# Rose-STL-Lab/spherical-dyffusion

Hardware: AMD Instinct MI355X
Metric: forecast-steps/sec (180x360, 63ch), 25-member ensemble DYffusion sampling, whole job (higher is better)
Workload: dtype f32 tensors; every GEMM-class kernel (1x1 convs, fused MLP, Legendre analysis/synthesis, dhconv) as 3-pass split-f16 MFMA with f32 accumulation; FFT / norms / pointwise in f32 (statistics f64); 1 GPU; 25-member ensemble x horizon-6 DYffusion sampling pass (6 forecaster + 10 interpolator SFNO forwards, dropout stream on, AR feedback), 180x360, 63 state + 2 forcing channels, embed 256, 8 blocks; horizon=6, relayed_members=0, parallelism=members of one initial condition sharded over GPUs, no data-path collective

## Files before the change

### include/sdy_amd.h

```cpp
#ifndef SDY_AMD_H
#define SDY_AMD_H

#include <stddef.h>
#include <stdint.h>

#ifdef __cplusplus
extern "C" {
#endif
#pragma GCC visibility push(default)

#define SDY_OK 0
#define SDY_ERR_ARG (-1)
#define SDY_ERR_UNSUPPORTED (-2)
#define SDY_ERR_ALIGN (-3)
#define SDY_ERR_WORKSPACE (-4)
#define SDY_ERR_NAME (-5)
#define SDY_ERR_SHAPE (-6)
#define SDY_ERR_STATE (-7)

#define SDY_GRID_EQUIANGULAR 0
#define SDY_GRID_LEGENDRE_GAUSS 1

int sdy_version(void);
const char* sdy_error_string(int code);
#define SDY_ABI_STRUCTS 25
int sdy_abi_check(const size_t* sizes, int n);
int sdy_abi_sizes(size_t* sizes, int n);

typedef struct sdy_sht_plan sdy_sht_plan;

int sdy_sht_tables_host(int nlat, int nlon, int lmax, int mmax, int grid, double* pct, double* w, double* theta);

int sdy_sht_plan_create(int nlat, int nlon, int lmax, int mmax, int grid, sdy_sht_plan** out);
int sdy_sht_plan_create_ex(int nlat, int nlon, int lmax, int mmax, int grid, int gemm_mode, sdy_sht_plan** out);
void sdy_sht_plan_destroy(sdy_sht_plan* plan);
int sdy_sht_plan_dims(const sdy_sht_plan* plan, int dims[6]);
int sdy_sht_plan_kernels(const sdy_sht_plan* plan, int out[2]);
size_t sdy_sht_workspace_floats(const sdy_sht_plan* plan, int B, int C);

int sdy_sht_forward(const sdy_sht_plan* plan, const float* x, float* out_c64, int B, int C, float* ws,
                    size_t ws_floats, void* stream);
int sdy_sht_inverse(const sdy_sht_plan* plan, const float* in_c64, float* y, int B, int C, float* ws,
                    size_t ws_floats, void* stream);

int sdy_rfft_lon(const sdy_sht_plan* plan, const float* x, const float* a, const float* d, float* xn_out,
                 float* Xf, int B, int C, void* stream);
int sdy_legendre_fwd(const sdy_sht_plan* plan, const float* Xf, float* Cs, int B, int C, void* stream);
int sdy_legendre_inv(const sdy_sht_plan* plan, const float* Cs, float* Yf, int B, int C, void* stream);
int sdy_irfft_lon(const sdy_sht_plan* plan, const float* Yf, const float* bias, float* y, int B, int C,
                  void* stream);
int sdy_irfft_lon_act(const sdy_sht_plan* plan, const float* Yf, const float* bias, float* zt, long zt_bstride, double* part,
                      int B, int C, void* stream);
int sdy_instnorm_from_partials(const double* part, int K, int B, int C, int HW, const float* gamma, const float* beta,
                               float eps, float* a, float* d, void* stream);
int sdy_gelu_stats(const float* y, long y_bstride, float* out, long out_bstride, int out_tiled, double* stats, int B, int C,
                   int HW, void* stream);
int sdy_affine_copy_stats(const float* x, long x_bstride, const float* a, const float* d, float* out, long out_bstride,
                          double* stats, int C, int HW, const unsigned char* rows, int n_rows, int src_row0, void* stream);

int sdy_dhconv_pack_weight(const float* w_host, int Ci, int Co, int L, float* w_packed_dev, void* stream);
int sdy_dhconv(const float* Cs_in, const float* w_packed, float* Cs_out, int L, int mtr, int B, int Ci, int Co,
               void* stream);
size_t sdy_dhconv_h3_pack_bytes(int Ci, int Co, int L);
int sdy_dhconv_h3_pack_weight(const float* w_host, int Ci, int Co, int L, void* packed_dev, float* scale);
int sdy_dhconv_h3(const float* Cs_in, const void* packed, float scale, float* Cs_out, int L, int mtr, int B, int Ci,
                  int Co, void* stream);

int sdy_dhconv_frag_supported(int Ci, int Co);
size_t sdy_dhconv_frag_pack_bytes(int L);
int sdy_dhconv_frag_pack(const float* w_host, int L, void* packed_dev, float* scale);
int sdy_dhconv_frag(const float* Cs_in, const void* packed, float scale, float* Cs_out, int L, int mtr, int B,
                    void* stream);

int sdy_instnorm_coeffs(const float* x, int B, int C, int HW, const float* gamma, const float* beta,
                        const float* scale_shift, long ss_stride, float eps, float* a, float* d, void* stream);

typedef struct sdy_conv_args {
  const float* x;  long x_bstride;
  const float* wt; int ldw;
  float* out;      long out_bstride;
  int B, Cin, Cout, HW;
  const float* pa; const float* pd;
  const float* bias;
  const float* add; long add_bstride;
  int add_mode;
  int act;
  float drop_p;
  const float* keep_mask;
  uint64_t seed; uint32_t call; uint32_t stream_id; uint32_t batch_offset;
  int rows_per_call;
  const float* batch_scale;
  int kernel_tag;
  const void* w_h3;
  float w_h3_scale;
  const void* w_frag;
  float w_frag_scale;
  double* stats;
  int out_tiled;
  const unsigned char* x_rows;
} sdy_conv_args;
int sdy_conv1x1(const sdy_conv_args* args, void* stream);

int sdy_conv256_h3_supported(int Cin, int Cout);
size_t sdy_conv256_h3_pack_bytes(void);
size_t sdy_conv256_h3_pack_bytes_cin(int Cin);
int sdy_conv256_h3_pack(const float* w_host, void* packed_dev, float* scale);
int sdy_conv256_h3_pack_cin(const float* w_host, int Cin, void* packed_dev, float* scale);
size_t sdy_h3_pack_bytes(int Cout, int Cin);
int sdy_h3_pack_weight(const float* w_host, int Cout, int Cin, void* packed_dev, float* scale);

typedef struct sdy_mlp_args {
  const float* x;  long x_bstride;
  const float* pa; const float* pd;
  const void* w; float w1_scale; float w2_scale;
  const float* b1; const float* b2;
  float* out;      long out_bstride;
  const float* add; long add_bstride;
  const float* add_a; const float* add_d;
  int B, E, hidden, HW;
  float drop_p;
  uint64_t seed; uint32_t call; uint32_t stream_fc1; uint32_t stream_fc2; uint32_t batch_offset;
  int rows_per_call;
  const float* batch_scale;
  double* stats;
  int x_tiled;
  const float* keep_hidden;
  const float* keep_out;
  const unsigned char* out_rows;
  int add_by_launch_row;
} sdy_mlp_args;
int sdy_instnorm_from_stats(double* stats, int B, int C, int HW, const float* gamma, const float* beta,
                            const float* scale_shift, long ss_bstride, float eps, float* a_out, float* d_out, void* stream);
int sdy_mlp_h3_supported(int E, int hidden);
size_t sdy_mlp_h3_pack_bytes(int E, int hidden);
int sdy_mlp_h3_pack(const float* w1_host, const float* w2_host, int E, int hidden, void* packed_dev, float* scale1,
                    float* scale2);
int sdy_mlp_h3(const sdy_mlp_args* args, void* stream);

typedef struct sdy_pair_args {
  const float* x;  long x_bstride;
  const void* w; float w1_scale; float w2_scale;
  const float* b1;
  float* out;      long out_bstride;
  const float* add; long add_bstride;
  int B, Cin, hidden, Cout, HW;
  double* stats;
} sdy_pair_args;
int sdy_pair_h3_supported(int Cin, int hidden, int Cout);
size_t sdy_pair_h3_pack_bytes(int Cin, int hidden, int Cout);
int sdy_pair_h3_pack(const float* w1_host, const float* w2_host, int Cin, int hidden, int Cout, void* packed_dev,
                     float* scale1, float* scale2);
int sdy_pair_h3(const sdy_pair_args* args, void* stream);

typedef struct sdy_sfno_config {
  int nlat, nlon;
  int in_chans;
  int out_chans;
  int embed_dim;
  int num_layers;
  int mlp_hidden;
  int lmax, mmax;
  int data_grid;
  int with_time_emb;
  int time_dim;
  float dropout_mlp;
  float drop_path_rate;
  int big_skip, pos_embed;
  int gemm_mode;
} sdy_sfno_config;

typedef struct sdy_sfno sdy_sfno;
int sdy_sfno_create(const sdy_sfno_config* cfg, sdy_sfno** out);
void sdy_sfno_destroy(sdy_sfno* net);
int sdy_sfno_set_param(sdy_sfno* net, const char* name, const float* host, size_t numel);
int sdy_sfno_ready(const sdy_sfno* net);
const char* sdy_sfno_missing(const sdy_sfno* net);
size_t sdy_sfno_workspace_floats(const sdy_sfno* net, int B);
int sdy_sfno_max_batch(const sdy_sfno* net);

typedef struct sdy_sfno_fwd_args {
  const float* in[3]; int in_chans[3];
  const float* time;
  float* out;
  int B;
  int enable_dropout;
  uint64_t seed; uint32_t call; uint32_t batch_offset;
  int rows_per_call;
  const float* const* keep_masks;
  const float* drop_path_keep;
  float* ws; size_t ws_floats;
  int reuse_encoder;
  int shared_inputs;
  const float* gen_src;
  int gen_chans;
  int gen_pos;
  const float* gen_coef;
  const float* gen_noise;
} sdy_sfno_fwd_args;
int sdy_sfno_forward(sdy_sfno* net, const sdy_sfno_fwd_args* args, void* stream);

int sdy_sfno_time_embed(sdy_sfno* net, const float* time, int B, float* t_repr, float* ss, void* stream);

int sdy_cold_update(const float* x_s, const float* x_ip_next, const float* x_ip_s, float* out, size_t n,
                    void* stream);
int sdy_concat_channels(const float* const* src, const int* chans, int nsrc, float* out, int B, int HW,
                        void* stream);

#define SDY_MAX_VARS 96
typedef struct sdy_var_table {
  int nvars;
  const float* data[SDY_MAX_VARS];
  float mean[SDY_MAX_VARS];
  float std[SDY_MAX_VARS];
} sdy_var_table;
int sdy_norm_pack(const sdy_var_table* vars, int t, int T1, int B, int HW, float* out, void* stream);

typedef struct sdy_step_finish_args {
  int B, HW, T1, t;
  const float* gen; int n_out;
  const float* prev_in; float* next_in; int n_in;
  int n_entries;
  int out_idx[SDY_MAX_VARS];
  int in_idx[SDY_MAX_VARS];
  float* gen_norm_tl[SDY_MAX_VARS];
  float* gen_tl[SDY_MAX_VARS];
  float mean[SDY_MAX_VARS], std[SDY_MAX_VARS];
  int presc_entry;
  const float* presc_target;
  const float* presc_mask;
  int mask_value, interpolate;
  const float* ar_init;
} sdy_step_finish_args;
int sdy_step_finish(const sdy_step_finish_args* args, void* stream);
int sdy_init_timeline(const sdy_var_table* vars, int T1, int B, int HW, float* const* tl_norm, float* const* tl_denorm,
                      void* stream);
int sdy_lp_rel_terms(const float* gen, const sdy_var_table* targets, int t, int T1, int B, int HW, double* terms,
                     void* stream);

int sdy_ensemble_metrics(const float* pred, const float* truth, const float* weights, int M, long member_stride,
                         int n_planes, int HW, double* out, void* stream);

int sdy_ensemble_series(const float* pred, int M, long member_stride, long sample_stride, const float* truth,
                        long truth_sample_stride, const float* weights, int n_sample, int T, int HW, double* out,
                        void* stream);

int sdy_ensemble_series_grad(const float* pred, int M, long member_stride, long sample_stride, const float* truth,
                             long truth_sample_stride, const float* weights, int n_sample, int T, int nlat, int nlon,
                             double* out, void* stream);

#define SDY_DERIVED_MAX_LEVELS 16
typedef struct {
  const float* q[SDY_DERIVED_MAX_LEVELS];
  const float* ps;
  const float* lhf;
  const float* prate;
  const float* adv;
  long s0, s1;
  int n0, n1, T, HW, K;
  float ak[SDY_DERIVED_MAX_LEVELS + 1], bk[SDY_DERIVED_MAX_LEVELS + 1];
// ... 338 lines not shown
```

### spherical-dyffusion_amd/_lib.py

```python
from __future__ import annotations

import ctypes as C
import os

_HERE = os.path.dirname(os.path.abspath(__file__))
LIB_PATH = os.environ.get("SDY_AMD_LIB") or os.path.join(_HERE, "libsdy_amd.so")

SDY_GRID = {"equiangular": 0, "legendre-gauss": 1}


class SdyError(RuntimeError):
    pass


class SdyConvArgs(C.Structure):
    _fields_ = [
        ("x", C.c_void_p), ("x_bstride", C.c_long),
        ("wt", C.c_void_p), ("ldw", C.c_int),
        ("out", C.c_void_p), ("out_bstride", C.c_long),
        ("B", C.c_int), ("Cin", C.c_int), ("Cout", C.c_int), ("HW", C.c_int),
        ("pa", C.c_void_p), ("pd", C.c_void_p),
        ("bias", C.c_void_p),
        ("add", C.c_void_p), ("add_bstride", C.c_long),
        ("add_mode", C.c_int),
        ("act", C.c_int),
        ("drop_p", C.c_float),
        ("keep_mask", C.c_void_p),
        ("seed", C.c_uint64), ("call", C.c_uint32), ("stream_id", C.c_uint32), ("batch_offset", C.c_uint32),
        ("rows_per_call", C.c_int),
        ("batch_scale", C.c_void_p),
        ("kernel_tag", C.c_int),
        ("w_h3", C.c_void_p),
        ("w_h3_scale", C.c_float),
        ("w_frag", C.c_void_p),
        ("w_frag_scale", C.c_float),
        ("stats", C.c_void_p),
        ("out_tiled", C.c_int),
        ("x_rows", C.c_void_p),
    ]


class SdyMlpArgs(C.Structure):
    _fields_ = [
        ("x", C.c_void_p), ("x_bstride", C.c_long),
        ("pa", C.c_void_p), ("pd", C.c_void_p),
        ("w", C.c_void_p), ("w1_scale", C.c_float), ("w2_scale", C.c_float),
        ("b1", C.c_void_p), ("b2", C.c_void_p),
        ("out", C.c_void_p), ("out_bstride", C.c_long),
        ("add", C.c_void_p), ("add_bstride", C.c_long),
        ("add_a", C.c_void_p), ("add_d", C.c_void_p),
        ("B", C.c_int), ("E", C.c_int), ("hidden", C.c_int), ("HW", C.c_int),
        ("drop_p", C.c_float),
        ("seed", C.c_uint64), ("call", C.c_uint32), ("stream_fc1", C.c_uint32), ("stream_fc2", C.c_uint32),
        ("batch_offset", C.c_uint32),
        ("rows_per_call", C.c_int),
        ("batch_scale", C.c_void_p),
        ("stats", C.c_void_p),
        ("x_tiled", C.c_int),
        ("keep_hidden", C.c_void_p), ("keep_out", C.c_void_p),
        ("out_rows", C.c_void_p),
        ("add_by_launch_row", C.c_int),
    ]


class SdyPairArgs(C.Structure):
    _fields_ = [
        ("x", C.c_void_p), ("x_bstride", C.c_long),
        ("w", C.c_void_p), ("w1_scale", C.c_float), ("w2_scale", C.c_float),
        ("b1", C.c_void_p),
        ("out", C.c_void_p), ("out_bstride", C.c_long),
        ("add", C.c_void_p), ("add_bstride", C.c_long),
        ("B", C.c_int), ("Cin", C.c_int), ("hidden", C.c_int), ("Cout", C.c_int), ("HW", C.c_int),
        ("stats", C.c_void_p),
    ]


SDY_MAX_VARS = 96


class SdyVarTable(C.Structure):
    _fields_ = [("nvars", C.c_int), ("data", C.c_void_p * SDY_MAX_VARS), ("mean", C.c_float * SDY_MAX_VARS),
                ("std", C.c_float * SDY_MAX_VARS)]


class SdyStepFinishArgs(C.Structure):
    _fields_ = [
        ("B", C.c_int), ("HW", C.c_int), ("T1", C.c_int), ("t", C.c_int),
        ("gen", C.c_void_p), ("n_out", C.c_int),
        ("prev_in", C.c_void_p), ("next_in", C.c_void_p), ("n_in", C.c_int),
        ("n_entries", C.c_int),
        ("out_idx", C.c_int * SDY_MAX_VARS), ("in_idx", C.c_int * SDY_MAX_VARS),
        ("gen_norm_tl", C.c_void_p * SDY_MAX_VARS), ("gen_tl", C.c_void_p * SDY_MAX_VARS),
        ("mean", C.c_float * SDY_MAX_VARS), ("std", C.c_float * SDY_MAX_VARS),
        ("presc_entry", C.c_int),
        ("presc_target", C.c_void_p), ("presc_mask", C.c_void_p),
        ("mask_value", C.c_int), ("interpolate", C.c_int),
        ("ar_init", C.c_void_p),
    ]


class SdySfnoConfig(C.Structure):
    _fields_ = [
        ("nlat", C.c_int), ("nlon", C.c_int),
        ("in_chans", C.c_int), ("out_chans", C.c_int),
        ("embed_dim", C.c_int), ("num_layers", C.c_int), ("mlp_hidden", C.c_int),
        ("lmax", C.c_int), ("mmax", C.c_int),
        ("data_grid", C.c_int),
        ("with_time_emb", C.c_int), ("time_dim", C.c_int),
        ("dropout_mlp", C.c_float), ("drop_path_rate", C.c_float),
        ("big_skip", C.c_int), ("pos_embed", C.c_int),
        ("gemm_mode", C.c_int),
    ]


class SdySfnoFwdArgs(C.Structure):
    _fields_ = [
        ("in_", C.c_void_p * 3), ("in_chans", C.c_int * 3),
        ("time", C.c_void_p),
        ("out", C.c_void_p),
        ("B", C.c_int),
# ... 238 lines not shown
        ("pool_times", C.c_int),
        ("n_events", C.c_int),
        ("n_maps", C.c_int),
        ("below", C.c_ubyte * SDY_MAX_VARS), ("is_map", C.c_ubyte * SDY_MAX_VARS),
        ("map_first", C.c_int * SDY_MAX_VARS),
        ("scalars", C.c_void_p), ("maps", C.c_void_p),
        ("acc", C.c_void_p),
    ]


SDY_FSS_MAX_RADII = 4


class SdyFssArgs(C.Structure):
    _anonymous_ = ("win",)
    _fields_ = [
        ("win", SdyWindow), ("H", C.c_int), ("W", C.c_int),
        ("t0", C.c_int),
        ("t_start", C.c_int), ("n_slots", C.c_int),
        ("pool_times", C.c_int),
        ("n_events", C.c_int),
        ("n_maps", C.c_int),
        ("below", C.c_ubyte * SDY_MAX_VARS), ("is_map", C.c_ubyte * SDY_MAX_VARS),
        ("map_first", C.c_int * SDY_MAX_VARS),
        ("scalars", C.c_void_p), ("maps", C.c_void_p),
        ("n_radii", C.c_int), ("radii", C.c_int * SDY_FSS_MAX_RADII),
        ("acc", C.c_void_p),
        ("ws", C.c_void_p), ("ws_bytes", C.c_size_t),
    ]


SDY_GRAM_MAX_MEMBERS = 64


class SdyMemberGramArgs(C.Structure):
    _anonymous_ = ("win",)
    _fields_ = [
        ("win", SdyWindow), ("HW", C.c_int),
        ("weights", C.c_void_p),
        ("climatology", C.c_void_p * SDY_MAX_VARS),
        ("out", C.c_void_p),
        ("ws", C.c_void_p), ("ws_bytes", C.c_size_t),
    ]


SDY_RANK_HIST_MAX_MEMBERS = 64


class SdyRankHistArgs(C.Structure):
    _anonymous_ = ("win",)
    _fields_ = [
        ("win", SdyWindow), ("H", C.c_int), ("W", C.c_int),
        ("t0", C.c_int),
        ("t_start", C.c_int), ("n_slots", C.c_int),
        ("pool_times", C.c_int),
        ("counts", C.c_void_p), ("ties", C.c_void_p),
    ]


ABI_STRUCTS = (SdyConvArgs, SdyMlpArgs, SdyPairArgs, SdySfnoConfig, SdySfnoFwdArgs, SdyVarTable, SdyStepFinishArgs,
               SdyDerivedArgs, SdyCorrectorArgs, SdyDryAirArgs, SdyHistArgs, SdyCoarsenArgs, SdyVideoArgs, SdyZonalArgs,
               SdyMemberSumArgs, SdyMemberStatsArgs, SdySpectrumArgs, SdyVariabilityArgs, SdyVariabilityMapsArgs,
               SdyVariabilityStatsArgs, SdyRegionSeriesArgs, SdyEventArgs, SdyFssArgs, SdyMemberGramArgs,
               SdyRankHistArgs)

SIGNATURES = {
    "sdy_version": (C.c_int, []),
    "sdy_error_string": (C.c_char_p, [C.c_int]),
    "sdy_abi_check": (C.c_int, [C.POINTER(C.c_size_t), C.c_int]),
    "sdy_abi_sizes": (C.c_int, [C.POINTER(C.c_size_t), C.c_int]),
    "sdy_sht_tables_host": (C.c_int, [C.c_int, C.c_int, C.c_int, C.c_int, C.c_int, C.c_void_p, C.c_void_p, C.c_void_p]),
    "sdy_sht_plan_create": (C.c_int, [C.c_int, C.c_int, C.c_int, C.c_int, C.c_int, C.POINTER(C.c_void_p)]),
    "sdy_sht_plan_create_ex": (C.c_int, [C.c_int, C.c_int, C.c_int, C.c_int, C.c_int, C.c_int, C.POINTER(C.c_void_p)]),
    "sdy_sht_plan_destroy": (None, [C.c_void_p]),
    "sdy_sht_plan_dims": (C.c_int, [C.c_void_p, C.POINTER(C.c_int * 6)]),
    "sdy_sht_plan_kernels": (C.c_int, [C.c_void_p, C.POINTER(C.c_int * 2)]),
    "sdy_sht_workspace_floats": (C.c_size_t, [C.c_void_p, C.c_int, C.c_int]),
    "sdy_sht_forward": (C.c_int, [C.c_void_p, C.c_void_p, C.c_void_p, C.c_int, C.c_int, C.c_void_p, C.c_size_t, C.c_void_p]),
    "sdy_sht_inverse": (C.c_int, [C.c_void_p, C.c_void_p, C.c_void_p, C.c_int, C.c_int, C.c_void_p, C.c_size_t, C.c_void_p]),
    "sdy_rfft_lon": (C.c_int, [C.c_void_p, C.c_void_p, C.c_void_p, C.c_void_p, C.c_void_p, C.c_void_p, C.c_int, C.c_int, C.c_void_p]),
    "sdy_legendre_fwd": (C.c_int, [C.c_void_p, C.c_void_p, C.c_void_p, C.c_int, C.c_int, C.c_void_p]),
    "sdy_legendre_inv": (C.c_int, [C.c_void_p, C.c_void_p, C.c_void_p, C.c_int, C.c_int, C.c_void_p]),
    "sdy_irfft_lon": (C.c_int, [C.c_void_p, C.c_void_p, C.c_void_p, C.c_void_p, C.c_int, C.c_int, C.c_void_p]),
    "sdy_irfft_lon_act": (C.c_int, [C.c_void_p, C.c_void_p, C.c_void_p, C.c_void_p, C.c_long, C.c_void_p, C.c_int, C.c_int,
                                    C.c_void_p]),
    "sdy_instnorm_from_partials": (C.c_int, [C.c_void_p, C.c_int, C.c_int, C.c_int, C.c_int, C.c_void_p, C.c_void_p, C.c_float,
                                             C.c_void_p, C.c_void_p, C.c_void_p]),
    "sdy_gelu_stats": (C.c_int, [C.c_void_p, C.c_long, C.c_void_p, C.c_long, C.c_int, C.c_void_p, C.c_int, C.c_int, C.c_int,
                                 C.c_void_p]),
    "sdy_affine_copy_stats": (C.c_int, [C.c_void_p, C.c_long, C.c_void_p, C.c_void_p, C.c_void_p, C.c_long, C.c_void_p, C.c_int,
                                        C.c_int, C.c_void_p, C.c_int, C.c_int, C.c_void_p]),
    "sdy_dhconv_pack_weight": (C.c_int, [C.c_void_p, C.c_int, C.c_int, C.c_int, C.c_void_p, C.c_void_p]),
    "sdy_dhconv": (C.c_int, [C.c_void_p, C.c_void_p, C.c_void_p, C.c_int, C.c_int, C.c_int, C.c_int, C.c_int, C.c_void_p]),
    "sdy_dhconv_h3_pack_bytes": (C.c_size_t, [C.c_int, C.c_int, C.c_int]),
    "sdy_dhconv_h3_pack_weight": (C.c_int, [C.c_void_p, C.c_int, C.c_int, C.c_int, C.c_void_p, C.POINTER(C.c_float)]),
    "sdy_dhconv_h3": (C.c_int, [C.c_void_p, C.c_void_p, C.c_float, C.c_void_p, C.c_int, C.c_int, C.c_int, C.c_int, C.c_int,
                                C.c_void_p]),
    "sdy_dhconv_frag_supported": (C.c_int, [C.c_int, C.c_int]),
    "sdy_dhconv_frag_pack_bytes": (C.c_size_t, [C.c_int]),
    "sdy_dhconv_frag_pack": (C.c_int, [C.c_void_p, C.c_int, C.c_void_p, C.POINTER(C.c_float)]),
    "sdy_dhconv_frag": (C.c_int, [C.c_void_p, C.c_void_p, C.c_float, C.c_void_p, C.c_int, C.c_int, C.c_int, C.c_void_p]),
    "sdy_instnorm_coeffs": (C.c_int, [C.c_void_p, C.c_int, C.c_int, C.c_int, C.c_void_p, C.c_void_p, C.c_void_p, C.c_long,
                                      C.c_float, C.c_void_p, C.c_void_p, C.c_void_p]),
    "sdy_conv1x1": (C.c_int, [C.POINTER(SdyConvArgs), C.c_void_p]),
    "sdy_ensemble_metrics": (C.c_int, [C.c_void_p, C.c_void_p, C.c_void_p, C.c_int, C.c_long, C.c_int, C.c_int, C.c_void_p,
                                       C.c_void_p]),
    "sdy_instnorm_from_stats": (C.c_int, [C.c_void_p, C.c_int, C.c_int, C.c_int, C.c_void_p, C.c_void_p, C.c_void_p,
                                          C.c_long, C.c_float, C.c_void_p, C.c_void_p, C.c_void_p]),
    "sdy_mlp_h3_supported": (C.c_int, [C.c_int, C.c_int]),
    "sdy_mlp_h3_pack_bytes": (C.c_size_t, [C.c_int, C.c_int]),
    "sdy_mlp_h3_pack": (C.c_int, [C.c_void_p, C.c_void_p, C.c_int, C.c_int, C.c_void_p, C.POINTER(C.c_float),
                                  C.POINTER(C.c_float)]),
    "sdy_mlp_h3": (C.c_int, [C.POINTER(SdyMlpArgs), C.c_void_p]),
    "sdy_pair_h3_supported": (C.c_int, [C.c_int, C.c_int, C.c_int]),
    "sdy_pair_h3_pack_bytes": (C.c_size_t, [C.c_int, C.c_int, C.c_int]),
    "sdy_pair_h3_pack": (C.c_int, [C.c_void_p, C.c_void_p, C.c_int, C.c_int, C.c_int, C.c_void_p, C.POINTER(C.c_float),
                                   C.POINTER(C.c_float)]),
    "sdy_pair_h3": (C.c_int, [C.POINTER(SdyPairArgs), C.c_void_p]),
    "sdy_conv256_h3_supported": (C.c_int, [C.c_int, C.c_int]),
    "sdy_conv256_h3_pack_bytes": (C.c_size_t, []),
    "sdy_conv256_h3_pack_bytes_cin": (C.c_size_t, [C.c_int]),
    "sdy_conv256_h3_pack": (C.c_int, [C.c_void_p, C.c_void_p, C.POINTER(C.c_float)]),
    "sdy_conv256_h3_pack_cin": (C.c_int, [C.c_void_p, C.c_int, C.c_void_p, C.POINTER(C.c_float)]),
    "sdy_h3_pack_bytes": (C.c_size_t, [C.c_int, C.c_int]),
    "sdy_h3_pack_weight": (C.c_int, [C.c_void_p, C.c_int, C.c_int, C.c_void_p, C.POINTER(C.c_float)]),
    "sdy_sfno_create": (C.c_int, [C.POINTER(SdySfnoConfig), C.POINTER(C.c_void_p)]),
    "sdy_sfno_destroy": (None, [C.c_void_p]),
    "sdy_sfno_set_param": (C.c_int, [C.c_void_p, C.c_char_p, C.c_void_p, C.c_size_t]),
    "sdy_sfno_ready": (C.c_int, [C.c_void_p]),
    "sdy_sfno_missing": (C.c_char_p, [C.c_void_p]),
    "sdy_sfno_workspace_floats": (C.c_size_t, [C.c_void_p, C.c_int]),
    "sdy_sfno_max_batch": (C.c_int, [C.c_void_p]),
    "sdy_sfno_forward": (C.c_int, [C.c_void_p, C.POINTER(SdySfnoFwdArgs), C.c_void_p]),
    "sdy_sfno_time_embed": (C.c_int, [C.c_void_p, C.c_void_p, C.c_int, C.c_void_p, C.c_void_p, C.c_void_p]),
    "sdy_norm_pack": (C.c_int, [C.POINTER(SdyVarTable), C.c_int, C.c_int, C.c_int, C.c_int, C.c_void_p, C.c_void_p]),
    "sdy_step_finish": (C.c_int, [C.POINTER(SdyStepFinishArgs), C.c_void_p]),
    "sdy_init_timeline": (C.c_int, [C.POINTER(SdyVarTable), C.c_int, C.c_int, C.c_int, C.POINTER(C.c_void_p),
                                    C.POINTER(C.c_void_p), C.c_void_p]),
    "sdy_lp_rel_terms": (C.c_int, [C.c_void_p, C.POINTER(SdyVarTable), C.c_int, C.c_int, C.c_int, C.c_int, C.c_void_p,
                                   C.c_void_p]),
    "sdy_cold_update": (C.c_int, [C.c_void_p, C.c_void_p, C.c_void_p, C.c_void_p, C.c_size_t, C.c_void_p]),
    "sdy_concat_channels": (C.c_int, [C.POINTER(C.c_void_p), C.POINTER(C.c_int), C.c_int, C.c_void_p, C.c_int, C.c_int,
                                      C.c_void_p]),
    "sdy_time_mean_accumulate": (C.c_int, [C.c_void_p, C.c_int, C.c_long, C.c_int, C.c_long, C.c_int, C.c_int, C.c_int,
                                          C.c_float, C.c_void_p, C.c_void_p]),
    "sdy_status_flags": (C.c_int, [C.POINTER(C.c_uint), C.c_int, C.c_void_p]),
    "sdy_status_flags_async": (C.c_int, [C.c_void_p, C.c_int, C.c_void_p]),
    "sdy_range_headroom_enable": (C.c_int, [C.c_int]),
    "sdy_range_headroom": (C.c_int, [C.POINTER(C.c_float), C.c_int, C.c_void_p]),
    "sdy_dropout_stream_rounds": (C.c_int, []),
    "sdy_dropout_stream_words": (C.c_int, [C.c_uint32, C.c_uint32, C.c_uint32, C.c_uint32, C.c_uint32, C.c_uint32,
                                           C.POINTER(C.c_uint32)]),
    "sdy_cond_noise_fill": (C.c_int, [C.c_uint64, C.c_uint32, C.c_uint32, C.c_int, C.c_int, C.c_int, C.c_int, C.c_void_p,
                                      C.c_void_p]),
    "sdy_ensemble_series": (C.c_int, [C.c_void_p, C.c_int, C.c_long, C.c_long, C.c_void_p, C.c_long, C.c_void_p, C.c_int,
                                     C.c_int, C.c_int, C.c_void_p, C.c_void_p]),
    "sdy_ensemble_series_grad": (C.c_int, [C.c_void_p, C.c_int, C.c_long, C.c_long, C.c_void_p, C.c_long, C.c_void_p,
                                          C.c_int, C.c_int, C.c_int, C.c_int, C.c_void_p, C.c_void_p]),
    "sdy_derived_water": (C.c_int, [C.POINTER(SdyDerivedArgs), C.c_void_p]),
    "sdy_corrector": (C.c_int, [C.POINTER(SdyCorrectorArgs), C.c_void_p]),
    "sdy_corrector_host": (C.c_int, [C.POINTER(SdyCorrectorArgs)]),
    "sdy_corrector_workspace_bytes": (C.c_size_t, [C.c_int, C.c_int]),
    "sdy_dry_air_series": (C.c_int, [C.POINTER(SdyDryAirArgs), C.c_void_p]),
    "sdy_dry_air_series_host": (C.c_int, [C.POINTER(SdyDryAirArgs)]),
    "sdy_dry_air_workspace_bytes": (C.c_size_t, [C.c_int, C.c_int, C.c_int]),
    "sdy_hist_add": (C.c_int, [C.POINTER(SdyHistArgs), C.c_void_p]),
# ... 115 lines not shown
```

### spherical-dyffusion_amd/csrc/capi.hip

```cpp
#include <cmath>
#include <cstdio>
#include <cstdlib>
#include <cstring>
#include <mutex>
#include <string>
#include <vector>

#include "common.h"
#include "fft.h"
#include "pointwise.h"

static inline int round_up(int v, int m) { return (v + m - 1) / m * m; }
static inline size_t round_up_sz(size_t v, size_t m) { return (v + m - 1) / m * m; }

template <class F>
static float h3_pack_host(std::vector<_Float16>& buf, int nb, int rows, int K, int rows_pad, int Kpad, F value) {
  float mx = 0.f;
  for (int b = 0; b < nb; ++b)
    for (int r = 0; r < rows; ++r)
      for (int k = 0; k < K; ++k) mx = std::fmax(mx, std::fabs(value(b, r, k)));
  const float s = sdy_h3_scale(mx);
  const size_t plane = (size_t)nb * rows_pad * Kpad;
  buf.assign(2 * plane, (_Float16)0.0f);
  for (int b = 0; b < nb; ++b)
    for (int r = 0; r < rows; ++r) {
      const size_t base = ((size_t)b * rows_pad + r) * Kpad;
      for (int k = 0; k < K; ++k) sdy_h3_split(value(b, r, k) * s, buf[base + k], buf[plane + base + k]);
    }
  return s;
}


extern "C" int sdy_version(void) { return 102; }

extern "C" int sdy_abi_sizes(size_t* sizes, int n) {
  const size_t mine[SDY_ABI_STRUCTS] = {
      sizeof(sdy_conv_args),      sizeof(sdy_mlp_args),      sizeof(sdy_pair_args),        sizeof(sdy_sfno_config),
      sizeof(sdy_sfno_fwd_args),  sizeof(sdy_var_table),     sizeof(sdy_step_finish_args), sizeof(sdy_derived_args),
      sizeof(sdy_corrector_args), sizeof(sdy_dry_air_args),  sizeof(sdy_hist_args),        sizeof(sdy_coarsen_args),
      sizeof(sdy_video_args),     sizeof(sdy_zonal_args),    sizeof(sdy_member_sum_args),  sizeof(sdy_member_stats_args),
      sizeof(sdy_spectrum_args),  sizeof(sdy_variability_args), sizeof(sdy_variability_maps_args),
      sizeof(sdy_variability_stats_args), sizeof(sdy_region_series_args), sizeof(sdy_event_args),
      sizeof(sdy_fss_args),       sizeof(sdy_member_gram_args), sizeof(sdy_rank_hist_args)};
  if (!sizes || n != SDY_ABI_STRUCTS) return SDY_ERR_ARG;
  for (int i = 0; i < n; ++i) sizes[i] = mine[i];
  return SDY_OK;
}

extern "C" int sdy_abi_check(const size_t* sizes, int n) {
  size_t mine[SDY_ABI_STRUCTS];
  if (!sizes || sdy_abi_sizes(mine, n) != SDY_OK) return SDY_ERR_ARG;
  for (int i = 0; i < n; ++i)
    if (sizes[i] != mine[i]) return SDY_ERR_ARG;
  return SDY_OK;
}

extern "C" const char* sdy_error_string(int code) {
  switch (code) {
    case SDY_OK: return "ok";
    case SDY_ERR_ARG: return "bad argument (null pointer or non-positive extent)";
    case SDY_ERR_UNSUPPORTED: return "unsupported size/configuration";
    case SDY_ERR_ALIGN: return "extent along a contiguous dimension is not a multiple of 4, or a pointer read as float4 is not 16-byte aligned";
    case SDY_ERR_WORKSPACE: return "workspace too small";
    case SDY_ERR_NAME: return "unknown parameter name";
    case SDY_ERR_SHAPE: return "parameter has the wrong number of elements";
    case SDY_ERR_STATE: return "object not fully initialised";
    default: return code > 0 ? hipGetErrorString((hipError_t)code) : "unknown error";
  }
}

struct sdy_sht_plan {
  int nlat, nlon, lmax, mmax, mtr, grid;
  int Lpad4, Kpad4;
  float* d_wqT = nullptr;
  float* d_pct = nullptr;
  float* d_tw = nullptr;
  float* d_pw = nullptr;
  SdyFftDesc fft;
  int gemm_mode = 0;
  void* d_wq_h3 = nullptr;
  void* d_pct_h3 = nullptr;
  float s_wq = 1.f, s_pct = 1.f;
  int h3_rows_fwd = 0, h3_k_fwd = 0, h3_rows_inv = 0, h3_k_inv = 0;
  void* d_wq_frag = nullptr;
  void* d_pct_frag = nullptr;
  float s_wq_frag = 1.f, s_pct_frag = 1.f;
  void* d_wq_par = nullptr;
  void* d_pct_par = nullptr;
  float s_wq_par = 1.f, s_pct_par = 1.f;
  int* d_kdead = nullptr;
  int* d_mcut = nullptr;
  enum Leg { LEG_PAR, LEG_H3, LEG_GEMM_H3, LEG_GEMM_F32 } leg = LEG_GEMM_F32;
  bool fused360 = false;
};

namespace {
struct SdySwitches {
  bool gemm_f32, no_fft360, no_leg_par, no_leg_frag, no_dh_frag, no_fused_mlp, no_drop_skip, no_skip_fold;
};
const SdySwitches& sw() {
  static const SdySwitches v = [] {
    auto on = [](const char* n) { return std::getenv(n) != nullptr; };
    const char* g = std::getenv("SDY_GEMM_MODE");
    return SdySwitches{g && std::string(g) == "f32", on("SDY_NO_FFT360"), on("SDY_NO_LEG_PAR"), on("SDY_NO_LEG_FRAG"),
                       on("SDY_NO_DH_FRAG"), on("SDY_NO_FUSED_MLP"), on("SDY_NO_DROP_SKIP"), on("SDY_NO_SKIP_FOLD")};
  }();
  return v;
}
}
static int env_gemm_mode() { return sw().gemm_f32 ? 0 : 1; }

template <class D, class T>
static hipError_t upload(D** dst, const std::vector<T>& v) {
  hipError_t e = hipMalloc((void**)dst, v.size() * sizeof(T));
  return e == hipSuccess ? hipMemcpy(*dst, v.data(), v.size() * sizeof(T), hipMemcpyHostToDevice) : e;
}
struct LegTables { const float *wqT, *pf; int nlat, lmax, Lpad4, Kpad4; };
static float leg_wq_at(void* c, int m, int l, int k) {
  const LegTables* x = static_cast<const LegTables*>(c);
  return x->wqT[((size_t)m * x->nlat + k) * x->Lpad4 + l];
}
static float leg_pct_at(void* c, int m, int k, int l) {
  const LegTables* x = static_cast<const LegTables*>(c);
  return x->pf[((size_t)m * x->lmax + l) * x->Kpad4 + k];
}

extern "C" int sdy_sht_plan_create(int nlat, int nlon, int lmax, int mmax, int grid, sdy_sht_plan** out) {
  return sdy_sht_plan_create_ex(nlat, nlon, lmax, mmax, grid, env_gemm_mode(), out);
}

extern "C" int sdy_sht_plan_create_ex(int nlat, int nlon, int lmax, int mmax, int grid, int gemm_mode,
                                      sdy_sht_plan** out) {
  if (gemm_mode != 0 && gemm_mode != 1) return SDY_ERR_ARG;
  if (!out || nlat < 2 || nlon < 4 || lmax < 1 || mmax < 1) return SDY_ERR_ARG;
  if (nlon % 4) return SDY_ERR_ALIGN;
  if (mmax > nlon / 2 + 1) return SDY_ERR_ARG;
  if (grid != SDY_GRID_EQUIANGULAR && grid != SDY_GRID_LEGENDRE_GAUSS) return SDY_ERR_ARG;
  sdy_sht_plan* p = new sdy_sht_plan();
  p->nlat = nlat; p->nlon = nlon; p->lmax = lmax; p->mmax = mmax; p->grid = grid;
  p->mtr = mmax < lmax ? mmax : lmax;
  p->Lpad4 = round_up(lmax, 4);
  p->Kpad4 = round_up(nlat, 4);
  const int n = nlon / 2;
  p->fft.n = n;
  p->fft.S = (n + 1) | 1;
  p->fft.guard_f16 = gemm_mode == 1 ? 1 : 0;
  int r = sdy_factor_radices(n, p->fft.radices, &p->fft.nstages);
  if (r != SDY_OK) { delete p; return r; }
  if ((size_t)(4 * 16 * p->fft.S + 4 * n + 2) * sizeof(float) > 64 * 1024) { delete p; return SDY_ERR_UNSUPPORTED; }

  std::vector<double> pct((size_t)mmax * lmax * nlat), w(nlat);
  r = sdy_sht_tables_host(nlat, nlon, lmax, mmax, grid, pct.data(), w.data(), nullptr);
  if (r != SDY_OK) { delete p; return r; }
  const int mtr = p->mtr;
  std::vector<float> wqT((size_t)mtr * nlat * p->Lpad4, 0.0f), pf((size_t)mtr * lmax * p->Kpad4, 0.0f);
  for (int m = 0; m < mtr; ++m)
    for (int l = 0; l < lmax; ++l)
      for (int k = 0; k < nlat; ++k) {
        const double v = pct[((size_t)m * lmax + l) * nlat + k];
        wqT[((size_t)m * nlat + k) * p->Lpad4 + l] = (float)(v * w[k]);
        pf[((size_t)m * lmax + l) * p->Kpad4 + k] = (float)v;
      }
  std::vector<float> tw(2 * (size_t)n), pw(2 * (size_t)(n + 1));
  for (int j = 0; j < n; ++j) {
    const double a = -2.0 * M_PI * j / n;
    tw[2 * j] = (float)std::cos(a);
    tw[2 * j + 1] = (float)std::sin(a);
  }
  for (int m = 0; m <= n; ++m) {
    const double a = -2.0 * M_PI * m / nlon;
    pw[2 * m] = (float)std::cos(a);
    pw[2 * m + 1] = (float)std::sin(a);
  }
  hipError_t e = upload(&p->d_wqT, wqT);
  if (e == hipSuccess) e = upload(&p->d_pct, pf);
  if (e == hipSuccess) e = upload(&p->d_tw, tw);
  if (e == hipSuccess) e = upload(&p->d_pw, pw);
  if (e != hipSuccess) { sdy_sht_plan_destroy(p); return (int)e; }
  p->gemm_mode = gemm_mode;
  if (gemm_mode == 1) {
    std::vector<_Float16> buf;
    p->h3_rows_fwd = lmax > 128 ? round_up(lmax, 256) : 128; p->h3_k_fwd = round_up(nlat, 64);
    p->s_wq = h3_pack_host(buf, mtr, lmax, nlat, p->h3_rows_fwd, p->h3_k_fwd, [&](int m, int l, int k) {
      return wqT[((size_t)m * nlat + k) * p->Lpad4 + l];
    });
    if ((e = upload(&p->d_wq_h3, buf)) != hipSuccess) { sdy_sht_plan_destroy(p); return (int)e; }
    p->h3_rows_inv = nlat > 128 ? round_up(nlat, 256) : 128; p->h3_k_inv = round_up(lmax, 64);
    p->s_pct = h3_pack_host(buf, mtr, nlat, lmax, p->h3_rows_inv, p->h3_k_inv, [&](int m, int k, int l) {
// ... 120 lines not shown
  g.B = Xf; g.ldb = N; g.sB = (long)p->nlat * N;
  g.C = Cs; g.ldc = p->mtr * N; g.sC = N;
  g.M = p->Lpad4; g.M_store = p->lmax; g.N = N; g.K = p->nlat; g.nbatch = p->mtr;
  g.tri_mode = SDY_TRI_LEG_FWD; g.tile = SDY_TILE_64x128;
  if (p->leg == sdy_sht_plan::LEG_PAR)
    return sdy_leg_par_launch(p->d_wq_par, p->s_wq_par, p->mtr, Xf, tiled ? 64 : N, (long)p->nlat * N, Cs,
                              cs_tiled ? 64L : (long)p->mtr * N, cs_tiled ? (long)(N / 64) * p->lmax * 64 : (long)N,
                              p->lmax, p->nlat, N, 1, polar ? p->d_kdead : nullptr, (hipStream_t)stream,
                              tiled ? 64L * p->nlat : 0L, cs_tiled ? 64L * p->lmax : 0L);
  if (tiled || cs_tiled) return SDY_ERR_UNSUPPORTED;
  if (p->leg == sdy_sht_plan::LEG_H3)
    return sdy_leg_h3_launch(p->d_wq_frag, p->s_wq_frag, p->mtr, Xf, N, (long)p->nlat * N, Cs, (long)p->mtr * N, N, p->lmax,
                             p->nlat, N, SDY_TRI_LEG_FWD, (hipStream_t)stream);
  if (p->leg == sdy_sht_plan::LEG_GEMM_H3)
    return sdy_gemm_h3_launch(g, p->d_wq_h3, p->h3_rows_fwd, p->h3_k_fwd, (long)p->h3_rows_fwd * p->h3_k_fwd,
                              (long)p->mtr * p->h3_rows_fwd * p->h3_k_fwd, p->s_wq, 0, (hipStream_t)stream);
  return sdy_gemm_launch(g, (hipStream_t)stream);
}
extern "C" int sdy_legendre_fwd(const sdy_sht_plan* p, const float* Xf, float* Cs, int B, int C, void* stream) {
  if (!p || !Xf || !Cs || B <= 0 || C <= 0) return SDY_ERR_ARG;
  if (C & 1) return SDY_ERR_ALIGN;
  SDY_TRY(sdy_spec_zero_upper_launch(Cs, p->lmax, p->mtr, 2 * B * C, (hipStream_t)stream));
  return legendre_fwd_impl(p, Xf, Cs, B, C, false, stream, false, false);
}

struct sdy_vsht_plan {
  const sdy_sht_plan* base = nullptr;
  float* d_dT = nullptr;
  float* d_mT = nullptr;
};

extern "C" void sdy_vsht_plan_destroy(sdy_vsht_plan* v) {
  if (!v) return;
  if (v->d_dT) (void)hipFree(v->d_dT);
  if (v->d_mT) (void)hipFree(v->d_mT);
  delete v;
}

extern "C" int sdy_vsht_plan_create(const sdy_sht_plan* p, sdy_vsht_plan** out) {
  if (!p || !out) return SDY_ERR_ARG;
  const int nlat = p->nlat, lmax = p->lmax, mtr = p->mtr;
  std::vector<double> dtab((size_t)mtr * lmax * nlat), mtab((size_t)mtr * lmax * nlat), w(nlat);
  SDY_TRY(sdy_vsht_tables_host(nlat, p->nlon, lmax, mtr, p->grid, dtab.data(), mtab.data()));
  SDY_TRY(sdy_sht_tables_host(nlat, p->nlon, lmax, mtr, p->grid, nullptr, w.data(), nullptr));
  std::vector<float> dT((size_t)mtr * nlat * p->Lpad4, 0.0f), mT((size_t)mtr * nlat * p->Lpad4, 0.0f);
  for (int m = 0; m < mtr; ++m)
    for (int l = 0; l < lmax; ++l)
      for (int k = 0; k < nlat; ++k) {
        const size_t from = ((size_t)m * lmax + l) * nlat + k, to = ((size_t)m * nlat + k) * p->Lpad4 + l;
        dT[to] = (float)(dtab[from] * w[k]);
        mT[to] = (float)(mtab[from] * w[k]);
      }
  sdy_vsht_plan* v = new sdy_vsht_plan();
  v->base = p;
  hipError_t e = upload(&v->d_dT, dT);
  if (e == hipSuccess) e = upload(&v->d_mT, mT);
  if (e != hipSuccess) { sdy_vsht_plan_destroy(v); return (int)e; }
  *out = v;
  return SDY_OK;
}

extern "C" int sdy_vector_legendre_fwd(const sdy_vsht_plan* v, const float* Xf, float* Cs_d, float* Cs_m, int B, int C,
                                       void* stream) {
  if (!v || !v->base || !Xf || !Cs_d || !Cs_m || B <= 0 || C <= 0) return SDY_ERR_ARG;
  if (C & 1) return SDY_ERR_ALIGN;
  const sdy_sht_plan* p = v->base;
  const int N = 2 * B * C;
  const float* tables[2] = {v->d_dT, v->d_mT};
  float* outs[2] = {Cs_d, Cs_m};
  for (int i = 0; i < 2; ++i) {
    SDY_TRY(sdy_spec_zero_upper_launch(outs[i], p->lmax, p->mtr, N, (hipStream_t)stream));
    GemmParams g{};
    g.A = tables[i]; g.lda = p->Lpad4; g.sA = (long)p->nlat * p->Lpad4;
    g.B = Xf; g.ldb = N; g.sB = (long)p->nlat * N;
    g.C = outs[i]; g.ldc = p->mtr * N; g.sC = N;
    g.M = p->Lpad4; g.M_store = p->lmax; g.N = N; g.K = p->nlat; g.nbatch = p->mtr;
    g.tri_mode = SDY_TRI_LEG_FWD; g.tile = SDY_TILE_64x128;
    SDY_TRY(sdy_gemm_launch(g, (hipStream_t)stream));
  }
  return SDY_OK;
}

static int legendre_inv_impl(const sdy_sht_plan* p, const float* Cs, float* Yf, int B, int C, bool polar, void* stream,
                             bool tiled, bool cs_tiled) {
  if (!p || !Cs || !Yf || B <= 0 || C <= 0) return SDY_ERR_ARG;
  if (C & 1) return SDY_ERR_ALIGN;
  const int N = 2 * B * C;
  GemmParams g{};
  g.A = p->d_pct; g.lda = p->Kpad4; g.sA = (long)p->lmax * p->Kpad4;
  g.B = Cs; g.ldb = p->mtr * N; g.sB = N;
  g.C = Yf; g.ldc = N; g.sC = (long)p->nlat * N;
  g.M = p->Kpad4; g.M_store = p->nlat; g.N = N; g.K = p->lmax; g.nbatch = p->mtr;
  g.tri_mode = SDY_TRI_LEG_INV; g.tile = SDY_TILE_64x128;
  if (p->leg == sdy_sht_plan::LEG_PAR)
    return sdy_leg_par_launch(p->d_pct_par, p->s_pct_par, p->mtr, Cs, cs_tiled ? 64L : (long)p->mtr * N,
                              cs_tiled ? (long)(N / 64) * p->lmax * 64 : (long)N, Yf, tiled ? 64 : N,
                              (long)p->nlat * N, p->nlat, p->lmax, N, 0, polar ? p->d_kdead : nullptr, (hipStream_t)stream,
                              cs_tiled ? 64L * p->lmax : 0L, tiled ? 64L * p->nlat : 0L);
  if (tiled || cs_tiled) return SDY_ERR_UNSUPPORTED;
  if (p->leg == sdy_sht_plan::LEG_H3)
    return sdy_leg_h3_launch(p->d_pct_frag, p->s_pct_frag, p->mtr, Cs, (long)p->mtr * N, N, Yf, N, (long)p->nlat * N, p->nlat,
                             p->lmax, N, SDY_TRI_LEG_INV, (hipStream_t)stream);
  if (p->leg == sdy_sht_plan::LEG_GEMM_H3)
    return sdy_gemm_h3_launch(g, p->d_pct_h3, p->h3_rows_inv, p->h3_k_inv, (long)p->h3_rows_inv * p->h3_k_inv,
                              (long)p->mtr * p->h3_rows_inv * p->h3_k_inv, p->s_pct, 0, (hipStream_t)stream);
  return sdy_gemm_launch(g, (hipStream_t)stream);
}
extern "C" int sdy_legendre_inv(const sdy_sht_plan* p, const float* Cs, float* Yf, int B, int C, void* stream) {
  return legendre_inv_impl(p, Cs, Yf, B, C, false, stream, false, false);
}

extern "C" int sdy_sht_forward(const sdy_sht_plan* p, const float* x, float* out_c64, int B, int C, float* ws,
                               size_t ws_floats, void* stream) {
  if (!p || !x || !out_c64 || !ws) return SDY_ERR_ARG;
  if (ws_floats < sdy_sht_workspace_floats(p, B, C)) return SDY_ERR_WORKSPACE;
  float* Xf = ws;
  float* Cs = ws + round_up_sz(xf_floats(p, B, C), 64);
  SDY_TRY(sdy_rfft_lon(p, x, nullptr, nullptr, nullptr, Xf, B, C, stream));
  SDY_TRY(legendre_fwd_impl(p, Xf, Cs, B, C, false, stream, false, false));
  return sdy_spec_to_torch_launch(Cs, out_c64, B, C, p->lmax, p->mtr, p->mmax, (hipStream_t)stream);
}

extern "C" int sdy_sht_inverse(const sdy_sht_plan* p, const float* in_c64, float* y, int B, int C, float* ws,
                               size_t ws_floats, void* stream) {
  if (!p || !in_c64 || !y || !ws) return SDY_ERR_ARG;
  if (ws_floats < sdy_sht_workspace_floats(p, B, C)) return SDY_ERR_WORKSPACE;
  float* Yf = ws;
  float* Cs = ws + round_up_sz(xf_floats(p, B, C), 64);
  SDY_TRY(sdy_torch_to_spec_launch(in_c64, Cs, B, C, p->lmax, p->mtr, p->mmax, (hipStream_t)stream));
  SDY_TRY(sdy_legendre_inv(p, Cs, Yf, B, C, stream));
  return sdy_irfft_lon(p, Yf, nullptr, y, B, C, stream);
}

extern "C" int sdy_dhconv_pack_weight(const float* w_host, int Ci, int Co, int L, float* w_packed_dev, void* stream) {
  if (!w_host || !w_packed_dev || Ci <= 0 || Co <= 0 || L <= 0) return SDY_ERR_ARG;
  std::vector<float> packed((size_t)L * 2 * Ci * Co);
  for (int i = 0; i < Ci; ++i)
    for (int o = 0; o < Co; ++o)
      for (int l = 0; l < L; ++l) {
        const float* s = w_host + (((size_t)i * Co + o) * L + l) * 2;
        packed[(((size_t)l * 2 + 0) * Ci + i) * Co + o] = s[0];
        packed[(((size_t)l * 2 + 1) * Ci + i) * Co + o] = s[1];
      }
  (void)stream;
  SDY_HIP_TRY(hipMemcpy(w_packed_dev, packed.data(), packed.size() * sizeof(float), hipMemcpyHostToDevice));
  return SDY_OK;
}

extern "C" int sdy_dhconv(const float* Cs_in, const float* w_packed, float* Cs_out, int L, int mtr, int B, int Ci,
                          int Co, void* stream) {
  if (!Cs_in || !w_packed || !Cs_out || L <= 0 || mtr <= 0 || B <= 0 || Ci <= 0 || Co <= 0) return SDY_ERR_ARG;
  if ((Ci & 3) || (Co & 3)) return SDY_ERR_ALIGN;
  GemmParams g{};
  g.A = Cs_in; g.a_kcontig = 1; g.lda = 2 * Ci; g.sA = (long)mtr * B * 2 * Ci;
  g.B = w_packed; g.b_cplx = 1; g.cplx_Ei = Ci; g.cplx_Eo = Co; g.ldb = 2 * Co; g.sB = (long)2 * Ci * Co;
  g.C = Cs_out; g.ldc = 2 * Co; g.sC = (long)mtr * B * 2 * Co;
  g.M = mtr * B; g.M_store = mtr * B; g.N = 2 * Co; g.K = 2 * Ci; g.nbatch = L;
  g.tri_mode = SDY_TRI_DHCONV; g.tri_B = B; g.tile = SDY_TILE_64x128;
  return sdy_gemm_launch(g, (hipStream_t)stream);
}

static inline int dh_npad(int Co) { return round_up(2 * Co, 128); }
static inline int dh_kpad(int Ci) { return round_up(2 * Ci, 64); }

extern "C" size_t sdy_dhconv_h3_pack_bytes(int Ci, int Co, int L) {
  if (Ci <= 0 || Co <= 0 || L <= 0) return 0;
  return (size_t)2 * L * dh_npad(Co) * dh_kpad(Ci) * sizeof(_Float16);
}

static int dhconv_h3_pack(const float* w, int Ci, int Co, int L, void* packed_dev, float* scale, int ilv) {
  if (!w || !packed_dev || !scale || Ci <= 0 || Co <= 0 || L <= 0) return SDY_ERR_ARG;
  if (ilv && ((Ci & 15) || (Co & 15))) return SDY_ERR_UNSUPPORTED;
  std::vector<_Float16> buf;
  *scale = h3_pack_host(buf, L, 2 * Co, 2 * Ci, dh_npad(Co), dh_kpad(Ci), [&](int l, int op, int ip) {
    const int ro = ilv ? (op >> 4) & 1 : op >= Co, o = ilv ? (op >> 5) * 16 + (op & 15) : op - ro * Co;
    const int ri = ilv ? (ip >> 4) & 1 : ip >= Ci, i = ilv ? (ip >> 5) * 16 + (ip & 15) : ip - ri * Ci;
    const float* e = w + (((size_t)i * Co + o) * L + l) * 2;
    if (ri == ro) return e[0];
    return ri ? -e[1] : e[1];
  });
  SDY_HIP_TRY(hipMemcpy(packed_dev, buf.data(), buf.size() * sizeof(_Float16), hipMemcpyHostToDevice));
  return SDY_OK;
}
extern "C" int sdy_dhconv_h3_pack_weight(const float* w, int Ci, int Co, int L, void* packed_dev, float* scale) {
  return dhconv_h3_pack(w, Ci, Co, L, packed_dev, scale, 0);
}

extern "C" int sdy_dhconv_h3(const float* Cs_in, const void* packed, float scale, float* Cs_out, int L, int mtr, int B,
                             int Ci, int Co, void* stream) {
  if (!Cs_in || !packed || !Cs_out || L <= 0 || mtr <= 0 || B <= 0 || Ci <= 0 || Co <= 0) return SDY_ERR_ARG;
  if ((Ci & 3) || (Co & 3)) return SDY_ERR_ALIGN;
  GemmParams g{};
  g.A = Cs_in; g.lda = 2 * Ci; g.sA = (long)mtr * B * 2 * Ci;
  g.C = Cs_out; g.ldc = 2 * Co; g.sC = (long)mtr * B * 2 * Co;
  g.M = mtr * B; g.M_store = mtr * B; g.N = 2 * Co; g.K = 2 * Ci; g.nbatch = L;
  g.tri_mode = SDY_TRI_DHCONV; g.tri_B = B;
  const int Np = dh_npad(Co), Kp = dh_kpad(Ci);
  return sdy_gemm_h3_launch(g, packed, Np, Kp, (long)Np * Kp, (long)L * Np * Kp, scale, 1, (hipStream_t)stream);
}

extern "C" int sdy_instnorm_coeffs(const float* x, int B, int C, int HW, const float* gamma, const float* beta,
                                   const float* scale_shift, long ss_stride, float eps, float* a, float* d,
                                   void* stream) {
  return sdy_instnorm_coeffs_launch(x, B, C, HW, gamma, beta, scale_shift, ss_stride, eps, a, d, (hipStream_t)stream);
}

static inline bool tiled_stride_ok(long bs, int C, int HW) { return bs >= (long)((HW + 63) / 64) * C * 64; }

extern "C" int sdy_instnorm_from_partials(const double* part, int K, int B, int C, int HW, const float* gamma,
                                          const float* beta, float eps, float* a, float* d, void* stream) {
  if (!part || !gamma || !beta || !a || !d || K <= 0 || B <= 0 || C <= 0 || HW <= 0) return SDY_ERR_ARG;
  if ((HW & 3) || !fft_aligned16(part)) return SDY_ERR_ALIGN;
  return sdy_instnorm_from_partials_launch(part, K, B, C, HW, gamma, beta, eps, a, d, (hipStream_t)stream);
}

extern "C" int sdy_gelu_stats(const float* y, long y_bstride, float* out, long out_bstride, int out_tiled, double* stats,
                              int B, int C, int HW, void* stream) {
  if (!y || !out || B <= 0 || C <= 0 || HW <= 0 || y_bstride < 0 || out_bstride < 0) return SDY_ERR_ARG;
  if ((HW & 3) || (y_bstride & 3) || (out_bstride & 3) || !fft_aligned16(y) || !fft_aligned16(out) || !fft_aligned16(stats))
    return SDY_ERR_ALIGN;
  if (out_tiled && (!tiled_stride_ok(out_bstride, C, HW) || out == y)) return SDY_ERR_ARG;
  return sdy_gelu_stats_launch(y, y_bstride, out, out_bstride, out_tiled ? 1 : 0, stats, B, C, HW, (hipStream_t)stream);
}

extern "C" int sdy_affine_copy_stats(const float* x, long x_bstride, const float* a, const float* d, float* out,
                                     long out_bstride, double* stats, int C, int HW, const unsigned char* rows, int n_rows,
                                     int src_row0, void* stream) {
  if (!x || !out || !rows || (a == nullptr) != (d == nullptr) || C <= 0 || HW <= 0 || n_rows <= 0 || n_rows > SDY_MAP_MAX ||
      x_bstride < 0 || out_bstride < 0)
    return SDY_ERR_ARG;
  if ((HW & 3) || (x_bstride & 3) || (out_bstride & 3) || !fft_aligned16(x) || !fft_aligned16(out) || !fft_aligned16(stats))
    return SDY_ERR_ALIGN;
  return sdy_affine_copy_stats_launch(x, x_bstride, a, d, out, out_bstride, stats, C, HW, rows, n_rows, (hipStream_t)stream,
                                      src_row0 >= 0 ? src_row0 : -1);
}

extern "C" int sdy_irfft_lon_act(const sdy_sht_plan* p, const float* Yf, const float* bias, float* zt, long zt_bstride,
                                 double* part, int B, int C, void* stream) {
  if (!p || !Yf || !zt || !part || B <= 0 || C <= 0 || zt_bstride < 0) return SDY_ERR_ARG;
  if (C % 4 != 0 || (zt_bstride & 3) || !fft_aligned16(Yf) || !fft_aligned16(zt) || !fft_aligned16(part)) return SDY_ERR_ALIGN;
  if (!(p->fft.fft360 && p->fft.n == 180) || C % 16 != 0) return SDY_ERR_UNSUPPORTED;
  if (!tiled_stride_ok(zt_bstride, C, p->nlat * p->nlon)) return SDY_ERR_ARG;
  return sdy_fft360_launch_inv(p->fft, Yf, bias, nullptr, B, C, p->nlat, p->mtr, 0, nullptr, (hipStream_t)stream, zt, zt_bstride,
                               part);
}

static inline int h3_mpad(int Cout) { return Cout > 128 ? round_up(Cout, 256) : 128; }
static inline int h3_kpad(int Cin) { return round_up(Cin, 64); }

extern "C" size_t sdy_h3_pack_bytes(int Cout, int Cin) {
  if (Cout <= 0 || Cin <= 0) return 0;
  return (size_t)2 * h3_mpad(Cout) * h3_kpad(Cin) * sizeof(_Float16);
}

extern "C" int sdy_h3_pack_weight(const float* w, int Cout, int Cin, void* packed_dev, float* scale) {
  if (!w || !packed_dev || !scale || Cout <= 0 || Cin <= 0) return SDY_ERR_ARG;
  std::vector<_Float16> buf;
  *scale = h3_pack_host(buf, 1, Cout, Cin, h3_mpad(Cout), h3_kpad(Cin),
                        [&](int, int o, int i) { return w[(size_t)o * Cin + i]; });
  SDY_HIP_TRY(hipMemcpy(packed_dev, buf.data(), buf.size() * sizeof(_Float16), hipMemcpyHostToDevice));
  return SDY_OK;
}

extern "C" int sdy_conv1x1(const sdy_conv_args* a, void* stream) {
  if (!a || !a->x || (!a->wt && !a->w_h3 && !a->w_frag) || !a->out) return SDY_ERR_ARG;
  if (a->B <= 0 || a->Cin <= 0 || a->Cout <= 0 || a->HW <= 0) return SDY_ERR_ARG;
  if (!a->w_h3 && a->ldw < a->Cout) return SDY_ERR_ARG;
  if ((a->pa == nullptr) != (a->pd == nullptr)) return SDY_ERR_ARG;
  if (a->add_mode != 0 && !a->add) return SDY_ERR_ARG;
  if ((!a->w_h3 && (a->ldw & 3)) || (a->HW & 3) || (a->x_bstride & 3) || (a->out_bstride & 3)) return SDY_ERR_ALIGN;
  if (a->drop_p < 0.0f || a->drop_p >= 1.0f) return SDY_ERR_ARG;
  if (a->w_frag && sdy_conv256_h3_supported(a->Cin, a->Cout) && a->drop_p == 0.0f && !a->keep_mask && !a->batch_scale)
    return sdy_conv256_h3_launch(a, (hipStream_t)stream);
  if (a->stats || a->out_tiled || a->x_rows) return SDY_ERR_UNSUPPORTED;
  GemmParams g{};
  g.A = a->wt; g.lda = a->ldw; g.sA = 0;
  g.B = a->x; g.ldb = a->HW; g.sB = a->x_bstride;
  g.C = a->out; g.ldc = a->HW; g.sC = a->out_bstride;
  g.M = round_up(a->Cout, 4); g.M_store = a->Cout; g.N = a->HW; g.K = a->Cin; g.nbatch = a->B;
  g.tile = a->Cout > 64 ? SDY_TILE_128x128 : SDY_TILE_64x128;
  g.tag = (a->kernel_tag >= 1 && a->kernel_tag <= 3) ? a->kernel_tag : 0;
  g.pa = a->pa; g.pd = a->pd; g.p_bstride = a->Cin;
  g.bias = a->bias;
  g.add = a->add_mode ? a->add : nullptr; g.sAdd = a->add_bstride; g.ldadd = a->HW; g.add_mode = a->add_mode;
  g.act = a->act;
  if (a->drop_p > 0.0f) {
    g.drop_thr = sdy_drop_threshold16(a->drop_p);
    if (g.drop_thr == 0u) g.drop_thr = 1u;
    g.drop_scale = 1.0f / (1.0f - a->drop_p);
    g.keep_mask = a->keep_mask;
  }
  g.seed_lo = (uint32_t)(a->seed & 0xFFFFFFFFu); g.seed_hi = (uint32_t)(a->seed >> 32);
  g.stream_id = a->stream_id; g.call = a->call; g.batch_offset = a->batch_offset;
  if (a->rows_per_call < 0 || (a->rows_per_call > 0 && a->B % a->rows_per_call)) return SDY_ERR_ARG;
  g.rows_per_call = a->rows_per_call > 0 ? a->rows_per_call : a->B;
  g.batch_scale = a->batch_scale;
  if (a->w_h3) {
    const int Mp = h3_mpad(a->Cout), Kp = h3_kpad(a->Cin);
    return sdy_gemm_h3_launch(g, a->w_h3, Mp, Kp, 0, (long)Mp * Kp, a->w_h3_scale, 0, (hipStream_t)stream);
  }
  return sdy_gemm_launch(g, (hipStream_t)stream);
}

extern "C" int sdy_cold_update(const float* x_s, const float* x_ip_next, const float* x_ip_s, float* out, size_t n,
                               void* stream) {
  return sdy_cold_update_launch(x_s, x_ip_next, x_ip_s, out, n, (hipStream_t)stream);
}

extern "C" int sdy_concat_channels(const float* const* src, const int* chans, int nsrc, float* out, int B, int HW,
                                   void* stream) {
  if (!src || !chans || nsrc < 1 || nsrc > 4) return SDY_ERR_ARG;
  long total = 0;
  for (int i = 0; i < nsrc; ++i) total += chans[i];
  return sdy_concat_launch(src, chans, nsrc, out, total * HW, B, HW, (hipStream_t)stream);
}

extern "C" int sdy_cond_noise_fill(uint64_t seed, uint32_t call, uint32_t batch_offset, int rows_per_call, int B, int C, int HW,
                                   float* out, void* stream) {
  return sdy_cond_noise_launch(seed, call, batch_offset, rows_per_call, B, C, HW, out, (hipStream_t)stream);
}

namespace {

struct DevBuf {
  float* p = nullptr;
  size_t n = 0;
  bool set = false;
  void* h3 = nullptr;
  float h3_scale = 1.0f;
  void* frag = nullptr;
  float frag_scale = 1.0f;
};

struct BlockW {
  DevBuf n0w, n0b, n1w, n1b;
  DevBuf tw, tb;
  DevBuf fw;
  DevBuf fb;
  DevBuf skw, skb;
  DevBuf w1, b1, w2, b2;
  std::vector<float> w1_host, w2_host;
  void* mlp = nullptr;
  float mlp_s1 = 1.0f, mlp_s2 = 1.0f;
  std::vector<float> fw_host, skw_host, fb_host, skb_host;
  DevBuf fbs;
};

}

static int spec_ilv(const sdy_sfno_config& c) { return (c.gemm_mode == 1 && c.embed_dim % 16 == 0) ? 1 : 0; }

static bool skip_foldable(const sdy_sfno_config& c, int i) {
  const bool first = i == 0, last = i == c.num_layers - 1;
  return c.gemm_mode == 1 && c.data_grid != SDY_GRID_LEGENDRE_GAUSS && first != last;
}

enum DhKind { DH_FOLDED, DH_FRAG, DH_GEMM_H3, DH_GEMM_F32 };
static DhKind dhconv_kind(const sdy_sfno_config& c, int i) {
  if (c.gemm_mode != 1) return DH_GEMM_F32;
  if (!sdy_dhconv_frag_supported(c.embed_dim, c.embed_dim) || sw().no_dh_frag) return DH_GEMM_H3;
  return skip_foldable(c, i) && !sw().no_skip_fold ? DH_FOLDED : DH_FRAG;
}

namespace {
struct XfSide {
  const sdy_sht_plan* plan;
  bool polar;
  bool tiled;
  int ilv;
  const int* mcut;
};

struct BlockPath {
  XfSide in, out;
  bool scale_residual;
  bool fused_mlp;
  bool lazy_norm;
  bool cs_tiled;
  DhKind dh;
  enum Skip { SKIP_CONV, SKIP_GELU, SKIP_IN_FFT } skip;
  bool stats1;
  bool z_tiled;
  bool drop_skip;
};
}

struct sdy_sfno {
  sdy_sfno_config cfg;
  int HW, catC, decC, ldo;
  sdy_sht_plan* plan_data = nullptr;
  sdy_sht_plan* plan_lg = nullptr;
  DevBuf pos, e0w, e0b, e2w, d0w, d0b, d2w;
  struct Pair { std::vector<float> w1_host, w2_host; void* w = nullptr; float s1 = 1.0f, s2 = 1.0f; } enc, dec;
  DevBuf t1w, t1b, t3w, t3b, freq, wbt, bb;
  std::vector<BlockW> blk;
  std::vector<BlockPath> path;
  SdyTimeMlp tm;
  std::string missing;
  const float* enc_ws = nullptr;
  int enc_B = 0;
  bool enc_has_stats = false;
};

static int dev_alloc(DevBuf& b, size_t n) {
  if (b.p && b.n == n) return SDY_OK;
  if (b.p) (void)hipFree(b.p);
  b.p = nullptr;
  SDY_HIP_TRY(hipMalloc((void**)&b.p, n * sizeof(float)));
  b.n = n;
  return SDY_OK;
}
static int dev_upload(DevBuf& b, const float* host, size_t n) {
  SDY_TRY(dev_alloc(b, n));
  SDY_HIP_TRY(hipMemcpy(b.p, host, n * sizeof(float), hipMemcpyHostToDevice));
  b.set = true;
  return SDY_OK;
}
static int dev_upload_T(DevBuf& b, const float* host, int out, int in, int ld) {
  std::vector<float> t((size_t)in * ld, 0.0f);
  for (int o = 0; o < out; ++o)
    for (int i = 0; i < in; ++i) t[(size_t)i * ld + o] = host[(size_t)o * in + i];
  return dev_upload(b, t.data(), t.size());
}
static void dev_free(DevBuf& b) {
  if (b.p) (void)hipFree(b.p);
  if (b.h3) (void)hipFree(b.h3);
  if (b.frag) (void)hipFree(b.frag);
  b.p = nullptr;
  b.h3 = nullptr;
  b.frag = nullptr;
  b.set = false;
}
static int dev_upload_conv(DevBuf& b, const float* host, int out, int in, int ld, bool want_h3) {
  SDY_TRY(dev_upload_T(b, host, out, in, ld));
  if (want_h3) {
    if (b.h3) (void)hipFree(b.h3);
    b.h3 = nullptr;
    SDY_HIP_TRY(hipMalloc(&b.h3, sdy_h3_pack_bytes(out, in)));
    SDY_TRY(sdy_h3_pack_weight(host, out, in, b.h3, &b.h3_scale));
    if (sdy_conv256_h3_supported(in, out)) {
      if (b.frag) (void)hipFree(b.frag);
      b.frag = nullptr;
      SDY_HIP_TRY(hipMalloc(&b.frag, sdy_conv256_h3_pack_bytes_cin(in)));
      SDY_TRY(sdy_conv256_h3_pack_cin(host, in, b.frag, &b.frag_scale));
    }
  }
  return SDY_OK;
}

extern "C" int sdy_sfno_create(const sdy_sfno_config* c, sdy_sfno** out) {
  if (!c || !out) return SDY_ERR_ARG;
  if (c->nlat < 2 || c->nlon < 4 || c->in_chans < 1 || c->out_chans < 1 || c->embed_dim < 4 || c->num_layers < 1 ||
      c->num_layers > 32 || c->mlp_hidden < 4)
    return SDY_ERR_ARG;
  if ((c->embed_dim & 3) || (c->mlp_hidden & 3) || ((c->nlat * c->nlon) & 3)) return SDY_ERR_ALIGN;
  if (c->with_time_emb && (c->time_dim < 4 || (c->embed_dim & 1))) return SDY_ERR_ARG;
  if (c->dropout_mlp < 0.f || c->dropout_mlp >= 1.f || c->drop_path_rate < 0.f || c->drop_path_rate >= 1.f)
    return SDY_ERR_ARG;
  sdy_sfno* n = new sdy_sfno();
  n->cfg = *c;
  n->HW = c->nlat * c->nlon;
  n->catC = c->embed_dim + c->in_chans;
  n->decC = c->embed_dim + (c->big_skip ? c->in_chans : 0);
  n->ldo = round_up(c->out_chans, 4);
  n->blk.resize(c->num_layers);
// ... 143 lines not shown
          float* d = sum.data() + ((size_t)ii * E + oo) * c.lmax * 2;
          for (int l = 0; l < c.lmax; ++l) d[2 * l] += ws;
        }
      if (!w.fw.frag) SDY_HIP_TRY(hipMalloc(&w.fw.frag, sdy_dhconv_frag_pack_bytes(c.lmax)));
      return sdy_dh_h3_pack(sum.data(), c.lmax, w.fw.frag, &w.fw.frag_scale, spec_ilv(c));
    };
    const DhKind dh = dhconv_kind(c, i);
    const bool fold = dh == DH_FOLDED;
    if (rest == "filter.filter.weight") {
      EXPECT_NUMEL((size_t)E * E * c.lmax * 2);
      if (fold) {
        w.fw_host.assign(host, host + numel);
        SDY_TRY(pack_folded());
      } else if (dh == DH_FRAG) {
        if (!w.fw.frag) SDY_HIP_TRY(hipMalloc(&w.fw.frag, sdy_dhconv_frag_pack_bytes(c.lmax)));
        SDY_TRY(sdy_dh_h3_pack(host, c.lmax, w.fw.frag, &w.fw.frag_scale, spec_ilv(c)));
      } else if (dh == DH_GEMM_H3) {
        if (w.fw.h3) (void)hipFree(w.fw.h3);
        w.fw.h3 = nullptr;
        SDY_HIP_TRY(hipMalloc(&w.fw.h3, sdy_dhconv_h3_pack_bytes(E, E, c.lmax)));
        SDY_TRY(dhconv_h3_pack(host, E, E, c.lmax, w.fw.h3, &w.fw.h3_scale, spec_ilv(c)));
      } else {
        SDY_TRY(dev_alloc(w.fw, numel));
        SDY_TRY(sdy_dhconv_pack_weight(host, E, E, c.lmax, w.fw.p, nullptr));
      }
      w.fw.set = true;
      return SDY_OK;
    }
    auto fold_bias = [&]() -> int {
      if (!fold || w.fb_host.empty() || w.skb_host.empty()) return SDY_OK;
      std::vector<float> sum(E);
      for (int k = 0; k < E; ++k) sum[k] = w.fb_host[k] + w.skb_host[k];
      return dev_upload(w.fbs, sum.data(), E);
    };
    if (rest == "filter.filter.bias") {
      EXPECT_NUMEL(E);
      w.fb_host.assign(host, host + numel);
      SDY_TRY(fold_bias());
      return dev_upload(w.fb, host, numel);
    }
    if (rest == "inner_skip.weight") {
      EXPECT_NUMEL((size_t)E * E);
      if (fold) {
        w.skw_host.assign(host, host + numel);
        SDY_TRY(pack_folded());
      }
      return dev_upload_conv(w.skw, host, E, E, E, h3);
    }
    if (rest == "inner_skip.bias") {
      EXPECT_NUMEL(E);
      w.skb_host.assign(host, host + numel);
      SDY_TRY(fold_bias());
      return dev_upload(w.skb, host, numel);
    }
    auto pack_mlp = [&]() -> int {
      if (!h3 || !sdy_mlp_h3_supported(E, H) || w.w1_host.empty() || w.w2_host.empty()) return SDY_OK;
      if (!w.mlp) SDY_HIP_TRY(hipMalloc(&w.mlp, sdy_mlp_h3_pack_bytes(E, H)));
      return sdy_mlp_h3_pack(w.w1_host.data(), w.w2_host.data(), E, H, w.mlp, &w.mlp_s1, &w.mlp_s2);
    };
    if (rest == "mlp.fwd.0.weight") {
      EXPECT_NUMEL((size_t)H * E);
      SDY_TRY(dev_upload_conv(w.w1, host, H, E, H, h3));
      if (h3 && sdy_mlp_h3_supported(E, H)) { w.w1_host.assign(host, host + numel); SDY_TRY(pack_mlp()); }
      return SDY_OK;
    }
    if (rest == "mlp.fwd.0.bias") { EXPECT_NUMEL(H); return dev_upload(w.b1, host, numel); }
    if (rest == "mlp.fwd.2.weight" || rest == "mlp.fwd.3.weight") {
      EXPECT_NUMEL((size_t)E * H);
      SDY_TRY(dev_upload_conv(w.w2, host, E, H, E, h3));
      if (h3 && sdy_mlp_h3_supported(E, H)) { w.w2_host.assign(host, host + numel); SDY_TRY(pack_mlp()); }
      return SDY_OK;
    }
    if (rest == "mlp.fwd.2.bias" || rest == "mlp.fwd.3.bias") { EXPECT_NUMEL(E); return dev_upload(w.b2, host, numel); }
  }
  return SDY_ERR_NAME;
}

static BlockPath resolve_path(const sdy_sfno* n, int i) {
  const sdy_sfno_config& c = n->cfg;
  const BlockW& w = n->blk[i];
  const int E = c.embed_dim, ilv = spec_ilv(c);
  auto side = [&](const sdy_sht_plan* p) {
    const bool polar = plan_polar_ok(p, E), tiled = plan_tiled_ok(p, E, ilv);
    return XfSide{p, polar, tiled, tiled ? 2 : ilv, polar ? p->d_mcut : nullptr};
  };
  BlockPath b;
  b.in = side(i == 0 ? n->plan_data : n->plan_lg);
  b.out = side(i == c.num_layers - 1 ? n->plan_data : n->plan_lg);
  b.scale_residual = b.in.plan != b.out.plan;
  b.fused_mlp = w.mlp && !sw().no_fused_mlp;
  b.lazy_norm = b.fused_mlp && !b.scale_residual;
  b.dh = dhconv_kind(c, i);
  const bool dh_frag = b.dh == DH_FOLDED || b.dh == DH_FRAG;
  b.cs_tiled = b.in.tiled && b.out.tiled && dh_frag && b.in.plan->lmax == b.out.plan->lmax && b.in.plan->mtr == b.out.plan->mtr;
  b.stats1 = c.gemm_mode == 1 && w.skw.frag && sdy_conv256_h3_supported(E, E);
  b.z_tiled = b.stats1 && b.fused_mlp;
  b.skip = b.dh != DH_FOLDED ? BlockPath::SKIP_CONV : (b.out.tiled && b.z_tiled) ? BlockPath::SKIP_IN_FFT : BlockPath::SKIP_GELU;
  b.drop_skip = b.fused_mlp && b.z_tiled && b.cs_tiled && !sw().no_drop_skip;
  return b;
}

extern "C" int sdy_sfno_ready(const sdy_sfno* n_c) {
  sdy_sfno* n = const_cast<sdy_sfno*>(n_c);
  if (!n) return SDY_ERR_ARG;
  if (!n->path.empty()) return SDY_OK;
  const sdy_sfno_config& c = n->cfg;
  n->missing.clear();
  auto need = [&](const DevBuf& b, const std::string& nm) {
    if (!b.set && n->missing.empty()) n->missing = nm;
  };
  if (c.pos_embed) need(n->pos, "pos_embed");
  need(n->e0w, "encoder.0.weight"); need(n->e0b, "encoder.0.bias"); need(n->e2w, "encoder.2.weight");
  need(n->d0w, "decoder.0.weight"); need(n->d0b, "decoder.0.bias"); need(n->d2w, "decoder.2.weight");
  if (c.with_time_emb) {
    need(n->t1w, "time_emb_mlp.1.weight"); need(n->t1b, "time_emb_mlp.1.bias");
    need(n->t3w, "time_emb_mlp.3.weight"); need(n->t3b, "time_emb_mlp.3.bias");
  }
  for (int i = 0; i < c.num_layers; ++i) {
    const BlockW& w = n->blk[i];
    const std::string p = "blocks." + std::to_string(i) + ".";
    need(w.n0w, p + "norm0.weight"); need(w.n0b, p + "norm0.bias");
    need(w.n1w, p + "norm1.weight"); need(w.n1b, p + "norm1.bias");
    if (c.with_time_emb) { need(w.tw, p + "time_mlp.1.weight"); need(w.tb, p + "time_mlp.1.bias"); }
    need(w.fw, p + "filter.filter.weight"); need(w.fb, p + "filter.filter.bias");
    need(w.skw, p + "inner_skip.weight"); need(w.skb, p + "inner_skip.bias");
    need(w.w1, p + "mlp.fwd.0.weight"); need(w.b1, p + "mlp.fwd.0.bias");
    need(w.w2, p + "mlp.fwd.{2|3}.weight"); need(w.b2, p + "mlp.fwd.{2|3}.bias");
  }
  if (!n->missing.empty()) return SDY_ERR_STATE;
  if (c.with_time_emb) {
    n->tm.E = c.embed_dim; n->tm.T = c.time_dim;
    n->tm.freq = n->freq.p; n->tm.w1t = n->t1w.p; n->tm.b1 = n->t1b.p; n->tm.w2t = n->t3w.p; n->tm.b2 = n->t3b.p;
    n->tm.wbt = n->wbt.p; n->tm.bb = n->bb.p;
  } else {
    n->tm.E = 0;
  }
  std::vector<BlockPath> path;
  for (int i = 0; i < c.num_layers; ++i) {
    const BlockW& w = n->blk[i];
    const BlockPath b = resolve_path(n, i);
    const void* packed = b.dh == DH_GEMM_F32 ? (const void*)w.fw.p : b.dh == DH_GEMM_H3 ? w.fw.h3 : w.fw.frag;
    if (!packed) return SDY_ERR_STATE;
    if (b.dh == DH_FOLDED && !(b.scale_residual && w.fbs.set)) return SDY_ERR_STATE;
    path.push_back(b);
  }
  n->path = std::move(path);
  return SDY_OK;
}

extern "C" const char* sdy_sfno_missing(const sdy_sfno* n) { return n ? n->missing.c_str() : ""; }

namespace {
struct WsLayout {
  size_t cat, xa, xb, xe, xn, y, zt, hid, xf, cs, cs2, ca, cd, ca1, cd1, st0, st1, ste, ss, dp, trep, sp, total;
};
WsLayout ws_layout(const sdy_sfno* n, int B) {
  const sdy_sfno_config& c = n->cfg;
  const size_t HW = n->HW, E = c.embed_dim;
  WsLayout w;
  size_t off = 0;
  auto take = [&](size_t floats) { size_t o = off; off += round_up_sz(floats, 64); return o; };
  w.cat = take((size_t)B * n->catC * HW);
  const size_t img = (size_t)B * E * HW;
  w.xa = take(img); w.xb = take(img);
  w.xe = take(img);
  w.xn = take(img); w.y = take(img);
  w.zt = take((size_t)B * ((HW + 63) / 64) * E * 64);
  w.hid = take((size_t)B * c.mlp_hidden * HW);
  w.xf = take(xf_floats(n->plan_data, B, (int)E));
  w.cs = take(cs_floats(n->plan_data, B, (int)E)); w.cs2 = take(cs_floats(n->plan_data, B, (int)E));
  w.ca = take((size_t)B * E); w.cd = take((size_t)B * E); w.ca1 = take((size_t)B * E); w.cd1 = take((size_t)B * E);
  w.st1 = take((size_t)B * E * 4);
  w.st0 = take((size_t)B * E * 4);
  w.ste = take((size_t)B * E * 4);
  w.ss = take((size_t)B * c.num_layers * 2 * E);
  w.dp = take((size_t)B * c.num_layers);
  w.trep = take((size_t)2 * B * (c.with_time_emb ? c.time_dim : 1));
  w.sp = take((size_t)B * E * c.nlat * 4);
  w.total = off;
  return w;
}
}

extern "C" size_t sdy_sfno_workspace_floats(const sdy_sfno* n, int B) {
  if (!n || B <= 0) return 0;
  return ws_layout(n, B).total;
}

extern "C" int sdy_sfno_max_batch(const sdy_sfno* n) {
  if (!n) return 0;
  const sdy_sfno_config& c = n->cfg;
  const int mtr = c.mmax < c.lmax ? c.mmax : c.lmax;
  bool all_tiled = sdy_sfno_ready(n) == SDY_OK;
  for (const BlockPath& p : n->path) all_tiled = all_tiled && p.cs_tiled;
  long b;
  if (all_tiled) {
    b = ((1L << 32) - 1) / ((long)mtr * 8 * c.lmax * 64);
  } else {
    const long per_row = 192L * mtr * 2 * c.embed_dim * 4 + 2L * c.embed_dim * 4;
    b = ((1L << 32) - 1) / per_row;
  }
  if (b > SDY_MAP_MAX) b = SDY_MAP_MAX;
  return b < 1 ? 1 : (int)b;
}

extern "C" int sdy_sfno_time_embed(sdy_sfno* n, const float* time, int B, float* t_repr, float* ss, void* stream) {
  if (!n || !time || B <= 0) return SDY_ERR_ARG;
  SDY_TRY(sdy_sfno_ready(n));
  if (!n->cfg.with_time_emb) return SDY_ERR_UNSUPPORTED;
  if (!ss) return SDY_ERR_ARG;
  float* scratch = nullptr;
  SDY_HIP_TRY(hipMallocAsync(reinterpret_cast<void**>(&scratch), (size_t)2 * B * n->cfg.time_dim * sizeof(float), (hipStream_t)stream));
  const int rc = sdy_time_mlp_launch(n->tm, time, B, t_repr, ss, nullptr, nullptr, 0, 0, 0, 0, 0, (hipStream_t)stream, scratch);
  SDY_HIP_TRY(hipFreeAsync(scratch, (hipStream_t)stream));
  return rc;
}

namespace {
enum SdyStage {
  ST_CONCAT, ST_TIME_MLP, ST_ENC0, ST_ENC2, ST_NORM_COEFFS, ST_FFT_FWD, ST_LEG_FWD, ST_LEG_INV, ST_FFT_INV, ST_DHCONV,
  ST_SKIP_CONV, ST_MLP_FUSED, ST_MLP_FUSED_DROP, ST_FC1, ST_FC2, ST_DEC0, ST_DEC2, ST_ENC_PAIR, ST_DEC_PAIR, ST_DROP_COPY,
  ST_SKIP_GELU, ST_COUNT
};
const char* const kStageNames[ST_COUNT] = {
  "concat", "time_mlp", "encoder.0 conv", "encoder.2 conv", "instnorm coefficients", "rfft (lon)", "legendre analysis",
  "legendre synthesis", "irfft (lon)", "dhconv", "inner-skip conv", "mlp fused", "mlp fused (dropout)", "mlp fc1", "mlp fc2",
  "decoder.0 conv", "decoder.2 conv", "encoder (fused pair)", "decoder (fused pair)", "drop-path copy",
  "inner skip folded (gelu)"};
struct SdyProfiler {
  bool on = false;
  struct Rec { int stage; int rows; hipEvent_t e0, e1; bool closed; };
  std::vector<Rec> recs;
  std::vector<hipEvent_t> pool;
  std::mutex mu;
  int get_event(hipEvent_t* e) {
    if (!pool.empty()) { *e = pool.back(); pool.pop_back(); return SDY_OK; }
    SDY_HIP_TRY(hipEventCreate(e));
    return SDY_OK;
  }
  int begin(int stage, int rows, hipStream_t s, int* idx) {
    std::lock_guard<std::mutex> g(mu);
    Rec r{stage, rows, nullptr, nullptr, false};
    SDY_TRY(get_event(&r.e0));
    int rc = get_event(&r.e1);
    if (rc == SDY_OK) {
      hipError_t e = hipEventRecord(r.e0, s);
      if (e != hipSuccess) rc = (int)e;
    }
    if (rc != SDY_OK) {
      pool.push_back(r.e0);
      if (r.e1) pool.push_back(r.e1);
// ... 158 lines not shown
      SDY_STAGE_N(ST_ENC_PAIR, Be, sdy_pair_h3(&pa, stream));
    } else {
      sdy_conv_args cv = conv_args(n->e0w, B);
      cv.x = cat_in; cv.x_bstride = cat_bs; cv.ldw = E; cv.out = xa; cv.out_bstride = xbs;
      cv.Cin = c.in_chans; cv.Cout = E; cv.bias = n->e0b.p; cv.act = 1;
      SDY_STAGE(ST_ENC0, sdy_conv1x1(&cv, stream));
      cv = conv_args(n->e2w, B);
      cv.x = xa; cv.x_bstride = xbs; cv.ldw = E; cv.out = xe; cv.out_bstride = xbs; cv.Cin = E; cv.Cout = E;
      if (c.pos_embed) { cv.add = n->pos.p; cv.add_bstride = 0; cv.add_mode = 2; }
      if (cv.w_frag && sdy_conv256_h3_supported(E, E)) {
        SDY_HIP_TRY(hipMemsetAsync(ste, 0, (size_t)B * E * 2 * sizeof(double), stream));
        cv.stats = ste; have_ste = true;
      }
      SDY_STAGE(ST_ENC2, sdy_conv1x1(&cv, stream));
    }
    n->enc_ws = enc_once ? nullptr : ws; n->enc_B = B; n->enc_has_stats = have_ste;
    if (have_ste) {
      for (int b0 = 0; b0 < B; b0 += Be)
        SDY_HIP_TRY(hipMemcpyAsync(st0 + (size_t)b0 * E * 2, ste, (size_t)Be * E * 2 * sizeof(double), hipMemcpyDeviceToDevice,
                                   stream));
      cur_stats = st0;
    }
    return SDY_OK;
  }

  int block(int i) {
    const bool last = i == c.num_layers - 1;
    Blk k{i, n->path[i], n->blk[i], last ? cat : nxt, last ? cat_bs : xbs};
    k.z = k.P.z_tiled ? zt : y;
    k.z_bs = k.P.z_tiled ? zt_bs : xbs;
    k.st_out = (k.P.fused_mlp && !last) ? st0 : nullptr;
    SDY_TRY(norm0(k));
    drop_rows(k);
    SDY_TRY(spectral(k));
    if (k.Bp > 0) {
      SDY_TRY(inner_skip(k));
      SDY_TRY(mlp(k));
    }
    if (k.nD > 0) SDY_TRY(drop_copy(k));
    cur_stats = k.st_out;
    cur = k.dst;
    nxt = (k.dst == xa) ? xb : xa;
    return SDY_OK;
  }

  int norm0(const Blk& k) {
    const float* ssk = c.with_time_emb ? ss + (size_t)k.i * 2 * E : nullptr;
    const long ss_bs = (long)c.num_layers * 2 * E;
    if (cur_stats)
      SDY_STAGE(ST_NORM_COEFFS, sdy_instnorm_from_stats(cur_stats, B, E, HW, k.w.n0w.p, k.w.n0b.p, ssk, ss_bs, 1e-6f, ca, cd, stream));
    else
      SDY_STAGE(ST_NORM_COEFFS, sdy_instnorm_coeffs_launch(cur, B, E, HW, k.w.n0w.p, k.w.n0b.p, ssk, ss_bs, 1e-6f, ca, cd, stream));
    return SDY_OK;
  }

  void drop_rows(Blk& k) const {
    k.Bp = B;
    k.nD = 0;
    if (drop && !a->drop_path_keep && B <= SDY_MAP_MAX && n->tm.dp_rate[k.i] > 0.f && k.P.drop_skip) {
      unsigned char drp[SDY_MAP_MAX];
      k.Bp = 0;
      for (int b = 0; b < B; ++b) {
        const int bq = b / rpc;
        const philox4 wd = philox4x32((uint32_t)(b - bq * rpc) + a->batch_offset, 0xFFFFFFFFu, 0x1000u + (uint32_t)k.i,
                                      a->call + (uint32_t)bq, (uint32_t)(a->seed & 0xFFFFFFFFu), (uint32_t)(a->seed >> 32));
        if (wd.x >= n->tm.dp_thr[k.i]) k.perm[k.Bp++] = (unsigned char)b;
        else drp[k.nD++] = (unsigned char)b;
      }
      for (int j = 0; j < k.nD; ++j) k.perm[k.Bp + j] = drp[j];
    }
    k.rows = k.nD > 0 ? k.perm : nullptr;
    k.Bf = k.P.scale_residual ? B : k.Bp;
  }

  int spectral(const Blk& k) {
    const BlockPath& P = k.P;
    const sdy_sht_plan *pin = P.in.plan, *pout = P.out.plan;
    if (k.Bf > 0) {
      float* xn_out = (P.scale_residual || P.lazy_norm) ? nullptr : xn;
      SDY_STAGE_N(ST_FFT_FWD, k.Bf, sdy_fft_launch_fwd(pin->fft, cur, ca, cd, xn_out, Xf, k.Bf, E, pin->nlat, pin->mtr, P.in.ilv,
                                                       P.in.mcut, stream, k.rows, (k.i == 0 && enc_once) ? Be : 0));
      SDY_STAGE_N(ST_LEG_FWD, k.Bf, legendre_fwd_impl(pin, Xf, Cs, k.Bf, E, P.in.polar, stream, P.in.tiled, P.cs_tiled));
      if (P.scale_residual) {
        SDY_STAGE(ST_LEG_INV, legendre_inv_impl(pout, Cs, Xf, B, E, P.out.polar, stream, P.out.tiled, P.cs_tiled));
        SDY_STAGE(ST_FFT_INV, sdy_fft_launch_inv(pout->fft, Xf, nullptr, xn, B, E, pout->nlat, pout->mtr, P.out.ilv, P.out.mcut,
                                                 stream));
      }
    }
    if (k.Bp == 0) return SDY_OK;
    if (P.dh == DH_FOLDED || P.dh == DH_FRAG)
      SDY_STAGE_N(ST_DHCONV, k.Bp, sdy_dh_h3_launch(Cs, k.w.fw.frag, k.w.fw.frag_scale, Cs2, c.lmax, pin->mtr, k.Bp, ilv, stream,
                                                    P.cs_tiled ? 1 : 0, k.Bf));
    else if (P.dh == DH_GEMM_H3)
      SDY_STAGE(ST_DHCONV, sdy_dhconv_h3(Cs, k.w.fw.h3, k.w.fw.h3_scale, Cs2, c.lmax, pin->mtr, B, E, E, stream));
    else
      SDY_STAGE(ST_DHCONV, sdy_dhconv(Cs, k.w.fw.p, Cs2, c.lmax, pin->mtr, B, E, E, stream));
    SDY_STAGE_N(ST_LEG_INV, k.Bp, legendre_inv_impl(pout, Cs2, Xf, k.Bp, E, P.out.polar, stream, P.out.tiled, P.cs_tiled));
    const float* bias = P.dh == DH_FOLDED ? k.w.fbs.p : k.w.fb.p;
    if (P.skip == BlockPath::SKIP_IN_FFT)
      SDY_STAGE_N(ST_FFT_INV, k.Bp, sdy_fft360_launch_inv(pout->fft, Xf, bias, nullptr, k.Bp, E, pout->nlat, pout->mtr, P.out.ilv,
                                                          P.out.mcut, stream, zt, zt_bs, sp));
    else
      SDY_STAGE_N(ST_FFT_INV, k.Bp, sdy_fft_launch_inv(pout->fft, Xf, bias, y, k.Bp, E, pout->nlat, pout->mtr, P.out.ilv,
                                                       P.out.mcut, stream));
    return SDY_OK;
  }

  int inner_skip(const Blk& k) {
    const BlockPath& P = k.P;
    const BlockW& bw = k.w;
    if (P.skip == BlockPath::SKIP_IN_FFT) {
      SDY_STAGE_N(ST_NORM_COEFFS, k.Bp, sdy_instnorm_from_partials_launch(sp, P.out.plan->nlat, k.Bp, E, HW, bw.n1w.p, bw.n1b.p,
                                                                          1e-6f, ca1, cd1, stream));
      return SDY_OK;
    }
    if (P.skip == BlockPath::SKIP_GELU) {
      SDY_STAGE_N(ST_SKIP_GELU, k.Bp, sdy_gelu_stats_launch(y, xbs, k.z, k.z_bs, P.z_tiled ? 1 : 0, st1, k.Bp, E, HW, stream));
    } else {
      sdy_conv_args cv = conv_args(bw.skw, k.Bp);
      cv.x_rows = P.lazy_norm ? k.rows : nullptr;
      cv.x = P.lazy_norm ? cur : xn; cv.x_bstride = xbs;
      if (P.lazy_norm) { cv.pa = ca; cv.pd = cd; }
      cv.ldw = E; cv.out = k.z; cv.out_bstride = k.z_bs; cv.out_tiled = P.z_tiled ? 1 : 0;
      cv.Cin = E; cv.Cout = E; cv.bias = bw.skb.p; cv.add = y; cv.add_bstride = xbs; cv.add_mode = 1; cv.act = 1; cv.kernel_tag = 3;
      if (P.stats1) cv.stats = st1;
      SDY_STAGE_N(ST_SKIP_CONV, k.Bp, sdy_conv1x1(&cv, stream));
    }
    if (P.skip == BlockPath::SKIP_GELU || P.stats1)
      SDY_STAGE_N(ST_NORM_COEFFS, k.Bp, sdy_instnorm_from_stats(st1, k.Bp, E, HW, bw.n1w.p, bw.n1b.p, nullptr, 0, 1e-6f, ca1, cd1,
                                                                stream));
    else
      SDY_STAGE(ST_NORM_COEFFS, sdy_instnorm_coeffs_launch(y, B, E, HW, bw.n1w.p, bw.n1b.p, nullptr, 0, 1e-6f, ca1, cd1, stream));
    return SDY_OK;
  }

  int mlp(const Blk& k) {
    const BlockW& bw = k.w;
    const int i = k.i, Hd = c.mlp_hidden;
    const float* dps = (drop && n->tm.dp_rate[i] > 0.f) ? dp + (size_t)i * B : nullptr;
    const float* keep1 = (pm > 0.f && a->keep_masks) ? a->keep_masks[2 * i] : nullptr;
    const float* keep2 = (pm > 0.f && a->keep_masks) ? a->keep_masks[2 * i + 1] : nullptr;
    if (k.P.fused_mlp) {
      sdy_mlp_args ma;
      std::memset(&ma, 0, sizeof(ma));
      ma.x = k.z; ma.x_bstride = k.z_bs; ma.x_tiled = k.P.z_tiled ? 1 : 0; ma.pa = ca1; ma.pd = cd1;
      ma.w = bw.mlp; ma.w1_scale = bw.mlp_s1; ma.w2_scale = bw.mlp_s2; ma.b1 = bw.b1.p; ma.b2 = bw.b2.p;
      ma.out = k.dst; ma.out_bstride = k.dst_bs;
      if (k.P.lazy_norm) { ma.add = cur; ma.add_bstride = xbs; ma.add_a = ca; ma.add_d = cd; }
      else { ma.add = xn; ma.add_bstride = xbs; ma.add_by_launch_row = k.rows ? 1 : 0; }
      ma.B = k.Bp; ma.out_rows = k.rows; ma.E = E; ma.hidden = Hd; ma.HW = HW;
      ma.drop_p = pm; ma.seed = a->seed; ma.call = a->call; ma.stream_fc1 = 2u * i; ma.stream_fc2 = 2u * i + 1u;
      ma.batch_offset = a->batch_offset; ma.rows_per_call = rpc;
      ma.batch_scale = dps; ma.keep_hidden = keep1; ma.keep_out = keep2; ma.stats = k.st_out;
      SDY_STAGE_N(pm > 0.f ? ST_MLP_FUSED_DROP : ST_MLP_FUSED, k.Bp, sdy_mlp_h3(&ma, stream));
      return SDY_OK;
    }
    sdy_conv_args cv = conv_args(bw.w1, B);
    cv.x = y; cv.x_bstride = xbs; cv.ldw = Hd; cv.out = hid; cv.out_bstride = (long)Hd * HW;
    cv.Cin = E; cv.Cout = Hd; cv.pa = ca1; cv.pd = cd1; cv.bias = bw.b1.p; cv.act = 1; cv.kernel_tag = 1;
    cv.drop_p = pm; cv.stream_id = 2u * i; cv.keep_mask = keep1;
    SDY_STAGE(ST_FC1, sdy_conv1x1(&cv, stream));
    cv = conv_args(bw.w2, B);
    cv.x = hid; cv.x_bstride = (long)Hd * HW; cv.ldw = E; cv.out = k.dst; cv.out_bstride = k.dst_bs;
    cv.Cin = Hd; cv.Cout = E; cv.bias = bw.b2.p; cv.kernel_tag = 2;
    cv.drop_p = pm; cv.stream_id = 2u * i + 1u; cv.keep_mask = keep2; cv.batch_scale = dps;
    cv.add = xn; cv.add_bstride = xbs; cv.add_mode = 2;
    SDY_STAGE(ST_FC2, sdy_conv1x1(&cv, stream));
    return SDY_OK;
  }

  int drop_copy(const Blk& k) {
    if (k.P.lazy_norm)
      SDY_STAGE_N(ST_DROP_COPY, k.nD, sdy_affine_copy_stats_launch(cur, xbs, ca, cd, k.dst, k.dst_bs, k.st_out, E, HW,
                                                                   k.perm + k.Bp, k.nD, stream));
    else
      SDY_STAGE_N(ST_DROP_COPY, k.nD, sdy_affine_copy_stats_launch(xn, xbs, nullptr, nullptr, k.dst, k.dst_bs, k.st_out, E, HW,
                                                                   k.perm + k.Bp, k.nD, stream, k.Bp));
    return SDY_OK;
  }

  int decoder() {
    if (n->dec.w) {
      sdy_pair_args pa{};
      pa.x = cat; pa.x_bstride = cat_bs; pa.w = n->dec.w; pa.w1_scale = n->dec.s1; pa.w2_scale = n->dec.s2;
      pa.b1 = n->d0b.p; pa.out = a->out; pa.out_bstride = (long)c.out_chans * HW;
      pa.B = B; pa.Cin = n->decC; pa.hidden = E; pa.Cout = c.out_chans; pa.HW = HW;
      SDY_STAGE(ST_DEC_PAIR, sdy_pair_h3(&pa, stream));
      return SDY_OK;
    }
    sdy_conv_args cv = conv_args(n->d0w, B);
    cv.x = cat; cv.x_bstride = cat_bs; cv.ldw = E;
    cv.out = xa; cv.out_bstride = xbs; cv.Cin = n->decC; cv.Cout = E; cv.bias = n->d0b.p; cv.act = 1;
    SDY_STAGE(ST_DEC0, sdy_conv1x1(&cv, stream));
    cv = conv_args(n->d2w, B);
    cv.x = xa; cv.x_bstride = xbs; cv.ldw = n->ldo; cv.out = a->out; cv.out_bstride = (long)c.out_chans * HW;
    cv.Cin = E; cv.Cout = c.out_chans;
    SDY_STAGE(ST_DEC2, sdy_conv1x1(&cv, stream));
    return SDY_OK;
  }
};
}

extern "C" int sdy_sfno_forward(sdy_sfno* n, const sdy_sfno_fwd_args* a, void* stream) {
  if (!n || !a || !a->out || !a->ws || a->B <= 0) return SDY_ERR_ARG;
  SDY_TRY(sdy_sfno_ready(n));
  SfnoCall f(n, a, (hipStream_t)stream);
  SDY_TRY(f.check());
// ... 7 lines not shown
```

### spherical-dyffusion_amd/csrc/common.h

```cpp
#pragma once
#include <hip/hip_runtime.h>
#include <stdint.h>
#include <atomic>
#include <cmath>
#include <type_traits>

#include "../../include/sdy_amd.h"

#define SDY_HIP_TRY(expr)                       \
  do {                                          \
    hipError_t _e = (expr);                     \
    if (_e != hipSuccess) return (int)_e;       \
  } while (0)

#define SDY_TRY(expr)             \
  do {                            \
    int _r = (expr);              \
    if (_r != SDY_OK) return _r;  \
  } while (0)

static inline int sdy_launch_status() {
  hipError_t e = hipGetLastError();
  return e == hipSuccess ? SDY_OK : (int)e;
}
// ... 229 lines not shown
    uint32_t hi0 = (uint32_t)(p0 >> 32), lo0 = (uint32_t)p0;
    uint32_t hi1 = (uint32_t)(p1 >> 32), lo1 = (uint32_t)p1;
    uint32_t n0 = hi1 ^ c1 ^ k0, n2 = hi0 ^ c3 ^ k1;
    c0 = n0; c1 = lo1; c2 = n2; c3 = lo0;
    k0 += W0; k1 += W1;
  }
  return philox4{c0, c1, c2, c3};
}
static inline uint32_t sdy_drop_threshold16(float p) {
  double t = (double)p * 65536.0;
  if (t >= 65535.0) return 0xFFFFu;
  if (t <= 0.0) return 0u;
  return (uint32_t)t;
}
__host__ __device__ __forceinline__ bool sdy_keep16(uint32_t word, int half, uint32_t thr16) {
  return half ? (word >= (thr16 << 16)) : ((uint16_t)word >= (uint16_t)thr16);
}
static inline uint32_t sdy_drop_threshold(float p) {
  double t = (double)p * 4294967296.0;
  if (t >= 4294967295.0) return 0xFFFFFFFFu;
  if (t <= 0.0) return 0u;
  return (uint32_t)t;
}

#define SDY_NOISE_STREAM 0x2000u
__device__ __forceinline__ float sdy_u01_open0(uint32_t w) { return (float)((w >> 8) + 1u) * 5.9604644775390625e-08f; }
__device__ __forceinline__ f32x4 sdy_cond_noise4(uint32_t q, uint32_t traj, uint32_t C, uint32_t c, uint32_t call,
                                                 uint32_t seed_lo, uint32_t seed_hi) {
  const philox4 w = philox4x32(q, traj * C + c, SDY_NOISE_STREAM, call, seed_lo, seed_hi);
  const float r0 = sqrtf(-2.0f * logf(sdy_u01_open0(w.x)));
  const float r1 = sqrtf(-2.0f * logf(sdy_u01_open0(w.z)));
  float s0, c0, s1, c1;
  sincospif(2.0f * sdy_u01_open0(w.y), &s0, &c0);
  sincospif(2.0f * sdy_u01_open0(w.w), &s1, &c1);
  f32x4 e;
  e.x = r0 * c0; e.y = r0 * s0; e.z = r1 * c1; e.w = r1 * s1;
  return e;
}

enum { SDY_TRI_NONE = 0, SDY_TRI_LEG_FWD = 1, SDY_TRI_LEG_INV = 2, SDY_TRI_DHCONV = 3 };
enum { SDY_TILE_128x128 = 0, SDY_TILE_64x128 = 1 };

struct GemmParams {
  const float* A; const float* B; float* C;
  int M, N, K;
  int M_store;
  int lda, ldb, ldc;
  long sA, sB, sC;
  int nbatch;
  int a_kcontig;
  int b_cplx;
  int cplx_Ei, cplx_Eo;
  int tri_mode, tri_B;
  int tile;
  int tag;
  const float* pa; const float* pd; long p_bstride;
  const float* bias;
  const float* add; long sAdd; int ldadd; int add_mode;
  int act;
  uint32_t drop_thr; float drop_scale; const float* keep_mask;
  uint32_t seed_lo, seed_hi, stream_id, call, batch_offset;
  int rows_per_call;
  const float* batch_scale;
};
int sdy_gemm_launch(const GemmParams& p, hipStream_t stream);
int sdy_gemm_h3_launch(const GemmParams& p, const void* packed, int rows_pad, int Kpad, long bstride, long plane_halfs,
                       float w_scale, int rows_mode, hipStream_t stream);

int sdy_conv256_h3_launch(const sdy_conv_args* a, hipStream_t stream);
extern "C" int sdy_conv256_h3_pack_cin(const float* w_host, int Cin, void* dev, float* scale);
extern "C" size_t sdy_conv256_h3_pack_bytes_cin(int Cin);
int sdy_dh_h3_pack(const float* w_host, int L, void* packed_dev, float* scale, int ilv);
int sdy_dh_h3_launch(const float* Cs_in, const void* packed, float scale, float* Cs_out, int L, int mtr, int B, int ilv,
                      hipStream_t stream, int tiled = 0, int B_in = 0);

typedef float (*sdy_leg_value_fn)(void* ctx, int z, int row, int k);
int sdy_leg_h3_supported(int rows, int K);
size_t sdy_leg_h3_table_bytes(int nz);
int sdy_leg_h3_pack(int nz, int rows, int K, sdy_leg_value_fn value, void* ctx, void* dev, float* scale);
int sdy_leg_par_supported(int nlat, int lmax);
size_t sdy_leg_par_table_bytes(int nz);
int sdy_leg_par_pack(int nz, int nlat, int lmax, int fwd, sdy_leg_value_fn value, void* ctx, void* dev, float* scale);
int sdy_leg_par_launch(const void* table, float scale, int nz, const float* X, long ldx, long sX, float* C, long ldc,
                       long sC, int rows_out, int K, int N, int fwd, const int* kdead, hipStream_t stream, long tsx = 0, long tsc = 0);
int sdy_leg_h3_launch(const void* table, float scale, int nz, const float* X, long ldx, long sX, float* C, long ldc, long sC,
                      int M_store, int K, int N, int tri, hipStream_t stream);

int sdy_factor_radices(int n, int* radices, int* nstages);
```

### spherical-dyffusion_amd/csrc/conv_h3.hip

```cpp
#include <cmath>
#include <cstdlib>
#include <type_traits>
#include <vector>

#include "common.h"

namespace {

constexpr int CE = 256;
constexpr int CTN = 64;
constexpr int CKMAX = 384;
constexpr int CRING = 4;
constexpr float CSX = SDY_ACT_SX;
constexpr int CSTAT_BYTES = CE * 2 * 8;
#ifndef SDY_CONV_STAMP_T0
#define SDY_CONV_STAMP_T0 2
#endif

template <int KBLK, int NW>
struct ConvCfg {
  static_assert(NW == 4 || NW == 8, "4 or 8 waves");
  static constexpr int NT = 64 * NW;
  static constexpr int MT = 8 / NW;
  static constexpr int RS = 4 * NW;
  static constexpr int OC = (8 * KBLK + RS - 1) / RS;
  static constexpr int RPT = 64 / NW;
  static constexpr int PPI = (8 * OC + RPT - 1) / RPT;
  static constexpr int KROW = KBLK <= 4 ? 256 : 384;
  static constexpr int KSW = KROW / 16;
  static constexpr int GPK = 4 * MT;
  static constexpr int GPW = MT * KSW;
  static constexpr int WGS = NW == 4 ? 2 : 1;
  static constexpr int TILE_BYTES = 2 * CTN * KROW * 2;
  static constexpr int LDS_BYTES = TILE_BYTES + CSTAT_BYTES + CE * 4 + SDY_GELU_TAB_BYTES;
};
#ifndef SDY_CONV_GELU_TAB
#define SDY_CONV_GELU_TAB 1
#endif

struct ConvParams {
  const float* x; long x_bs;
  const float* pa; const float* pd;
  const sdy_f16x8* w;
  const float* bias;
  const float* add; long add_bs; int add_mode;
  int act;
  float* out; long out_bs;
  int out_tiled;
  double* stats;
  int HW, B;
  int Cin;
  float out_scale;
  unsigned* flags;
  unsigned* head;
  const float* gelu_tab;
  SdyImgMap xmap;
  unsigned long long* stamps;
};

__device__ __forceinline__ int cv_swz(int px) { return (px & 15) ^ (((px >> 4) & 1) * 3); }
template <int KROW>
__device__ __forceinline__ int cv_off(int px, int c) { return px * KROW + (((c & ~15) | ((c ^ cv_swz(px)) & 15)) << 3); }

template <int KBLK, int NW>
__global__ __launch_bounds__(64 * NW, NW == 4 ? 2 : 1) void conv_h3_kernel(const ConvParams p) {
  using G = ConvCfg<KBLK, NW>;
  constexpr int CMT = G::MT, CRS = G::RS, COC = G::OC, CRPT = G::RPT, KROW = G::KROW, CGPK = G::GPK, CGPW = G::GPW;
  __shared__ __attribute__((aligned(16))) unsigned char smem[G::LDS_BYTES];
  _Float16* Xs_hi = reinterpret_cast<_Float16*>(smem);
  _Float16* Xs_lo = Xs_hi + CTN * KROW;
  float* Os = reinterpret_cast<float*>(smem);

  const int tid = threadIdx.x, lane = tid & 63, wave = tid >> 6;
  int h = lane >> 5, l31 = lane & 31;
  int q0 = tid & 15, o0 = tid >> 4;
  const int tpi = (p.HW + CTN - 1) / CTN;
  const int ntiles = tpi * p.B;
  const int t_per = (ntiles + (int)gridDim.x - 1) / (int)gridDim.x;
  const int t_begin = (int)blockIdx.x * t_per;
  const int t_end = (t_begin + t_per < ntiles) ? t_begin + t_per : ntiles;

  sdy_f16x8 r_hi[CRING], r_lo[CRING];
  constexpr int CGROUP_BYTES = SDY_GROUP * (int)sizeof(sdy_f16x8);
  const char* const wbase = reinterpret_cast<const char*>(p.w) + (size_t)__builtin_amdgcn_readfirstlane(wave) * CGPW * CGROUP_BYTES;
  unsigned woff = (unsigned)lane * 16u;
#pragma unroll
  for (int s = 0; s < CRING; ++s) {
    r_hi[s] = sdy_ring_ld(wbase, woff, 0);
    r_lo[s] = sdy_ring_ld(wbase, woff, CGROUP_BYTES / 2);
    woff += CGROUP_BYTES;
  }
  constexpr int NWIN = KBLK * CMT;
  if (NWIN == 1) woff -= CRING * CGROUP_BYTES;

  double* Ss = reinterpret_cast<double*>(smem + G::TILE_BYTES);
  float* Bs = reinterpret_cast<float*>(smem + G::TILE_BYTES + CSTAT_BYTES);
  if (tid < CE) {
    Bs[tid] = p.bias ? p.bias[tid] / p.out_scale : 0.0f;
    Ss[2 * tid] = 0.0; Ss[2 * tid + 1] = 0.0;
  }
  float* Gt = reinterpret_cast<float*>(smem + G::TILE_BYTES + CSTAT_BYTES + CE * 4);
  const unsigned gt_base = (unsigned)(uintptr_t)Gt;
  const bool tab_gelu = SDY_CONV_GELU_TAB && p.act == 1;
  if (tab_gelu) gelu_tab_to_lds(Gt, p.gelu_tab, tid, G::NT, 1.0f / SDY_GELU_SX);
  const float os_scale = tab_gelu ? p.out_scale * SDY_GELU_WS : p.out_scale;

  f32x4 xr[COC][8], addv[CRPT];
  auto img = [&](const float* base, long bs, int t) { return base + (long)(t / tpi) * bs; };
  auto ximg = [&](int t) { return p.x + (long)sdy_img(p.xmap, t / tpi) * p.x_bs; };
  auto lane_col = [&](int t) {
    const int nn = (t % tpi) * CTN + 4 * q0;
    return nn < p.HW ? nn : 0;
  };
  const float* addsrc = p.add ? p.add : p.out;
  const long addsrc_bs = p.add ? p.add_bs : p.out_bs;
  if (t_begin < t_end) {
    const float* xz = ximg(t_begin);
    const unsigned xo = (unsigned)(8 * o0 * p.HW + lane_col(t_begin)) * 4u;
#pragma unroll
    for (int oc = 0; oc < COC; ++oc)
#pragma unroll
      for (int e = 0; e < 8; ++e) {
        const int ch = 8 * (o0 + CRS * oc) + e;
        xr[oc][e] = f32x4{0.f, 0.f, 0.f, 0.f};
        if (ch < p.Cin) xr[oc][e] = sdy_ld16s(xz + (long)(8 * CRS * oc + e) * p.HW, xo);
      }
  }

// ... 21 lines not shown
        if (p.pa) {
          const f32x4 a0 = *reinterpret_cast<const f32x4*>(p.pa + (long)zx * CE + c0);
          const f32x4 a1 = *reinterpret_cast<const f32x4*>(p.pa + (long)zx * CE + c0 + 4);
          const f32x4 d0 = *reinterpret_cast<const f32x4*>(p.pd + (long)zx * CE + c0);
          const f32x4 d1 = *reinterpret_cast<const f32x4*>(p.pd + (long)zx * CE + c0 + 4);
#pragma unroll
          for (int e = 0; e < 4; ++e) {
            av[e] = a0[e] * CSX; av[e + 4] = a1[e] * CSX;
            dv[e] = d0[e] * CSX; dv[e + 4] = d1[e] * CSX;
          }
        } else {
#pragma unroll
          for (int e = 0; e < 8; ++e) { av[e] = CSX; dv[e] = 0.f; }
        }
#pragma unroll
        for (int pp = 0; pp < 4; ++pp) {
          sdy_f16x8 vh, vl;
          float v[8];
#pragma unroll
          for (int e = 0; e < 8; ++e) v[e] = (ok && c0 + e < p.Cin) ? fmaf(xr[oc][e][pp], av[e], dv[e]) : 0.0f;
          sdy_split8(v, vh, vl, amax);
          const int off = cv_off<KROW>(4 * q0 + pp, o0 + CRS * oc);
          *reinterpret_cast<sdy_f16x8*>(Xs_hi + off) = vh;
          *reinterpret_cast<sdy_f16x8*>(Xs_lo + off) = vl;
        }
      }
      sdy_flag_range(p.flags, amax, p.head);
    }
    __syncthreads();
    stamp(1);
    const int col = n0 + 4 * q0;
    const bool c_ok = full || col < p.HW;
    const unsigned ro = (unsigned)(o0 * p.HW + (c_ok ? col : 0)) * 4u;
    const unsigned ro_out = p.out_tiled ? (unsigned)(o0 * CTN + 4 * q0) * 4u : ro;
    const int out_rs = p.out_tiled ? CTN : p.HW;
    const int tnext = (tile + 1 < t_end) ? tile + 1 : tile;
    const float* xz_next = ximg(tnext);
    const unsigned xo_next = (unsigned)(8 * o0 * p.HW + lane_col(tnext)) * 4u;
    stamp(2);
    f32x16 acc[CMT][2];
#pragma unroll
    for (int mi = 0; mi < CMT; ++mi)
#pragma unroll
      for (int r4 = 0; r4 < 4; ++r4) {
        const f32x4 b4 = *reinterpret_cast<const f32x4*>(Bs + 32 * (CMT * wave + mi) + 8 * r4 + 4 * h);
#pragma unroll
        for (int j = 0; j < 2; ++j)
#pragma unroll
          for (int r = 0; r < 4; ++r) acc[mi][j][4 * r4 + r] = b4[r];
      }
#pragma unroll
    for (int kb = 0; kb < KBLK; ++kb) {
#pragma unroll
      for (int i = 0; i < 4; ++i) {
        const int ks = 4 * kb + i;
        sdy_f16x8 bh[2], bl[2];
#pragma unroll
        for (int j = 0; j < 2; ++j) {
          const int off = cv_off<KROW>(32 * j + l31, 2 * ks + h);
          bh[j] = *reinterpret_cast<const sdy_f16x8*>(Xs_hi + off);
          bl[j] = *reinterpret_cast<const sdy_f16x8*>(Xs_lo + off);
        }
#pragma unroll
        for (int mi = 0; mi < CMT; ++mi) {
          const int g = kb * CGPK + CMT * i + mi;
          const int s = g % CRING;
#pragma unroll
          for (int j = 0; j < 2; ++j) SDY_CROSS_TERM(acc[mi][j] = __builtin_amdgcn_mfma_f32_32x32x16_f16(r_lo[s], bh[j], acc[mi][j], 0, 0, 0));
#pragma unroll
          for (int j = 0; j < 2; ++j) SDY_CROSS_TERM(acc[mi][j] = __builtin_amdgcn_mfma_f32_32x32x16_f16(r_hi[s], bl[j], acc[mi][j], 0, 0, 0));
#pragma unroll
          for (int j = 0; j < 2; ++j) acc[mi][j] = __builtin_amdgcn_mfma_f32_32x32x16_f16(r_hi[s], bh[j], acc[mi][j], 0, 0, 0);
          r_hi[s] = sdy_ring_ld(wbase, woff, 0);
          r_lo[s] = sdy_ring_ld(wbase, woff, CGROUP_BYTES / 2);
          woff += CGROUP_BYTES;
          if ((g + CRING + 1) % (NWIN * CRING) == 0) woff -= NWIN * CRING * CGROUP_BYTES;
          __builtin_amdgcn_sched_barrier(0);
        }
      }
    }

    stamp(3);
    {
      const float* az = img(addsrc, addsrc_bs, tile);
#pragma unroll
      for (int i = 0; i < CRPT; ++i) addv[i] = p.add ? sdy_ld16s(az + (long)(CRS * i) * p.HW, ro) : f32x4{0.f, 0.f, 0.f, 0.f};
    }
    __syncthreads();
    stamp(4);
#pragma unroll
    for (int mi = 0; mi < CMT; ++mi)
#pragma unroll
      for (int j = 0; j < 2; ++j)
#pragma unroll
        for (int r = 0; r < 16; ++r) {
          const int row = 32 * (CMT * wave + mi) + (r & 3) + 8 * (r >> 2) + 4 * h;
          Os[row * CTN + 32 * j + l31] = acc[mi][j][r] * os_scale;
        }
    __syncthreads();
    stamp(5);
    {
      float* oz = p.out + (long)z * p.out_bs + (p.out_tiled ? (long)(tile - z * tpi) * (CE * CTN) : 0L);
#pragma unroll
      for (int i = 0; i < CRPT; ++i) {
        f32x4 v = *reinterpret_cast<const f32x4*>(Os + (o0 + CRS * i) * CTN + 4 * q0);
        if (tab_gelu) {
          if (p.add_mode == 1) v = addv[i] * SDY_GELU_WS + v;
          v = f32x4{gelu_tab16(v.x, gt_base), gelu_tab16(v.y, gt_base), gelu_tab16(v.z, gt_base), gelu_tab16(v.w, gt_base)};
        } else {
        if (p.add_mode == 1) v += addv[i];
        if (p.act == 1) {
          const sdy_gf2 g0 = gelu_erf2(sdy_gf2{v.x, v.y}), g1 = gelu_erf2(sdy_gf2{v.z, v.w});
          v = f32x4{g0.x, g0.y, g1.x, g1.y};
        }
        }
        if (p.add_mode == 2) v += addv[i];
        if (c_ok) sdy_st16s(oz + (long)(CRS * i) * out_rs, ro_out, v);
#pragma unroll
        for (int k = 0; k < G::PPI; ++k) {
          const int piece = G::PPI * i + k, oc = piece >> 3, e = piece & 7;
          if (oc < COC) {
            const int ch = 8 * (o0 + CRS * oc) + e;
            if (ch < p.Cin) xr[oc][e] = sdy_ld16s(xz_next + (long)(8 * CRS * oc + e) * p.HW, xo_next);
          }
        }
        if (p.stats) {
          const float s1 = row16_sum(c_ok ? (v.x + v.y) + (v.z + v.w) : 0.0f);
          const float s2 = row16_sum(c_ok ? (v.x * v.x + v.y * v.y) + (v.z * v.z + v.w * v.w) : 0.0f);
          if (q0 == 0) {
            double* st = Ss + 2 * (o0 + CRS * i);
            __hip_atomic_fetch_add(st, (double)s1, __ATOMIC_RELAXED, __HIP_MEMORY_SCOPE_WORKGROUP);
            __hip_atomic_fetch_add(st + 1, (double)s2, __ATOMIC_RELAXED, __HIP_MEMORY_SCOPE_WORKGROUP);
          }
        }
      }
    }
    stamp(6);
    {
      const int nt = tile + 1;
      if (p.stats && (nt >= t_end || nt / tpi != z)) {
        __syncthreads();
        if (tid < CE) {
          double* st = p.stats + ((long)z * CE + tid) * 2;
          __hip_atomic_fetch_add(st, Ss[2 * tid], __ATOMIC_RELAXED, __HIP_MEMORY_SCOPE_AGENT);
          __hip_atomic_fetch_add(st + 1, Ss[2 * tid + 1], __ATOMIC_RELAXED, __HIP_MEMORY_SCOPE_AGENT);
          Ss[2 * tid] = 0.0; Ss[2 * tid + 1] = 0.0;
        }
      }
    }
    stamp(7);
    __syncthreads();
  }
}

}

#if SDY_STAMPS_ON
static unsigned long long* g_cstamps = nullptr;
SDY_DEBUG_EXPORT int sdy_conv256_h3_debug_stamps(unsigned long long* host64) {
  if (!g_cstamps || !host64) return SDY_ERR_STATE;
  SDY_HIP_TRY(hipDeviceSynchronize());
  SDY_HIP_TRY(hipMemcpy(host64, g_cstamps, 64 * sizeof(unsigned long long), hipMemcpyDeviceToHost));
  return SDY_OK;
}
#endif

extern "C" int sdy_conv256_h3_supported(int Cin, int Cout) { return (Cin >= 1 && Cin <= CKMAX && Cout == CE) ? 1 : 0; }

static void conv_layout(int Cin, int* nw, int* ksw, int* mt) {
  const int kblk = (Cin + 63) / 64;
  *nw = kblk <= 4 ? 4 : 8;
  *ksw = kblk <= 4 ? 16 : 24;
  *mt = 8 / *nw;
}

extern "C" size_t sdy_conv256_h3_pack_bytes_cin(int Cin) {
  int nw, ksw, mt;
  conv_layout(Cin < 1 ? 1 : Cin, &nw, &ksw, &mt);
  return (size_t)nw * mt * ksw * SDY_GROUP * sizeof(sdy_f16x8);
}
extern "C" size_t sdy_conv256_h3_pack_bytes(void) { return sdy_conv256_h3_pack_bytes_cin(CE); }

extern "C" int sdy_conv256_h3_pack_cin(const float* w_host, int Cin, void* dev, float* scale) {
  if (!w_host || !dev || !scale || Cin < 1 || Cin > CKMAX) return SDY_ERR_ARG;
  const float s = sdy_h3_scale(sdy_h3_absmax(w_host, (size_t)CE * Cin));
  int nw, ksw, mt;
  conv_layout(Cin, &nw, &ksw, &mt);
  const size_t gh = (size_t)SDY_GROUP * 8;
  std::vector<_Float16> buf((size_t)nw * mt * ksw * gh);
  _Float16* d = buf.data();
  for (int w = 0; w < nw; ++w)
    for (int ks = 0; ks < ksw; ++ks)
      for (int mi = 0; mi < mt; ++mi, d += gh)
        sdy_h3_put_group(d, s, [&](int r, int k) {
          const int kk = 16 * ks + k;
          return kk < Cin ? w_host[(size_t)(32 * (mt * w + mi) + r) * Cin + kk] : 0.0f;
        });
  SDY_HIP_TRY(hipMemcpy(dev, buf.data(), buf.size() * sizeof(_Float16), hipMemcpyHostToDevice));
  *scale = s;
  return SDY_OK;
}
extern "C" int sdy_conv256_h3_pack(const float* w_host, void* dev, float* scale) {
  return sdy_conv256_h3_pack_cin(w_host, CE, dev, scale);
}

template <int KBLK, int NW>
static void conv_launch(const ConvParams& p, long ntiles, int n_cu, hipStream_t stream) {
  using G = ConvCfg<KBLK, NW>;
  const long want = (long)n_cu * G::WGS;
  dim3 grid((unsigned)(ntiles < want ? ntiles : want));
  hipLaunchKernelGGL((conv_h3_kernel<KBLK, NW>), grid, dim3(G::NT), 0, stream, p);
}

int sdy_conv256_h3_launch(const sdy_conv_args* a, hipStream_t stream) {
  if (!a || !a->x || !a->w_frag || !a->out || a->B <= 0 || a->HW <= 0) return SDY_ERR_ARG;
  if (!sdy_conv256_h3_supported(a->Cin, a->Cout)) return SDY_ERR_UNSUPPORTED;
  if (a->drop_p > 0.f || a->keep_mask || a->batch_scale) return SDY_ERR_UNSUPPORTED;
  if (a->pa && a->Cin != CE) return SDY_ERR_UNSUPPORTED;
  if ((a->HW & 3) || (a->x_bstride & 3) || (a->out_bstride & 3) || (a->add_mode && (a->add_bstride & 3))) return SDY_ERR_ALIGN;
  if ((long)a->HW * CKMAX * 4 >= (1L << 32)) return SDY_ERR_UNSUPPORTED;
  ConvParams p;
  p.x = a->x; p.x_bs = a->x_bstride; p.pa = a->pa; p.pd = a->pd;
  p.w = reinterpret_cast<const sdy_f16x8*>(a->w_frag);
  p.bias = a->bias;
  p.add = a->add_mode ? a->add : nullptr; p.add_bs = a->add_bstride; p.add_mode = a->add_mode;
  p.act = a->act;
  p.out = a->out; p.out_bs = a->out_bstride; p.out_tiled = a->out_tiled;
  if (a->out_tiled && a->add_mode && a->add == a->out) return SDY_ERR_ARG;
  p.stats = a->stats;
  SDY_TRY(sdy_flags_ptr(&p.flags));
  SDY_TRY(sdy_headroom_ptr(SDY_RANGE_CONV, &p.head));
  SDY_TRY(sdy_gelu_table_ptr(&p.gelu_tab));
  p.HW = a->HW; p.B = a->B; p.Cin = a->Cin;
  SDY_TRY(sdy_img_map_fill(p.xmap, a->x_rows, a->B));
  p.out_scale = 1.0f / (a->w_frag_scale * CSX);
  p.stamps = nullptr;
#if SDY_STAMPS_ON
  if (std::getenv("SDY_CONV_STAMPS")) {
    if (!g_cstamps) SDY_HIP_TRY(hipMalloc(&g_cstamps, 64 * sizeof(unsigned long long)));
    p.stamps = g_cstamps;
  }
#endif
  int n_cu = 0;
  SDY_TRY(sdy_cu_count(&n_cu));
  const long ntiles = (long)((a->HW + CTN - 1) / CTN) * a->B;
  switch ((a->Cin + 63) / 64) {
    case 1: conv_launch<1, 4>(p, ntiles, n_cu, stream); break;
    case 2: conv_launch<2, 4>(p, ntiles, n_cu, stream); break;
    case 3: conv_launch<3, 4>(p, ntiles, n_cu, stream); break;
    case 4: conv_launch<4, 4>(p, ntiles, n_cu, stream); break;
    case 5: conv_launch<5, 8>(p, ntiles, n_cu, stream); break;
    default: conv_launch<6, 8>(p, ntiles, n_cu, stream); break;
  }
  return sdy_launch_status();
}
```

### spherical-dyffusion_amd/csrc/fft.h

```cpp
#pragma once
#include <hip/hip_runtime.h>

struct SdyFftDesc {
  int n;
  int S;
  int nstages;
  int radices[10];
  const float* tw;
  const float* pw;
  int guard_f16;
  int fft360;
};


int sdy_fft_launch_fwd(const SdyFftDesc& f, const float* x, const float* a, const float* d, float* xn_out, float* Xf,
                       int B, int C, int K, int mtr, int ilv, const int* mcut, hipStream_t stream,
                       const unsigned char* x_rows = nullptr, int x_mod = 0);
int sdy_fft_launch_inv(const SdyFftDesc& f, const float* Yf, const float* bias, float* y, int B, int C, int K, int mtr,
                       int ilv, const int* mcut, hipStream_t stream);

int sdy_fft360_launch_fwd(const SdyFftDesc& f, const float* x, const float* a, const float* d, float* xn_out, float* Xf,
                          int B, int C, int K, int mtr, int ilv, const int* mcut, hipStream_t stream,
                          const unsigned char* x_rows = nullptr, int x_mod = 0);
int sdy_fft360_launch_inv(const SdyFftDesc& f, const float* Yf, const float* bias, float* y, int B, int C, int K,
                          int mtr, int ilv, const int* mcut, hipStream_t stream, float* zt = nullptr, long zt_bs = 0,
                          double* part = nullptr);
```

### spherical-dyffusion_amd/csrc/fft.hip

```cpp
#include "common.h"
#include "fft.h"

namespace {

constexpr int CB = 16;
constexpr int NT = 256;

struct cpx {
  float r, i;
};
__device__ __forceinline__ cpx cmul(cpx a, cpx b) { return cpx{a.r * b.r - a.i * b.i, a.r * b.i + a.i * b.r}; }
__device__ __forceinline__ cpx cadd(cpx a, cpx b) { return cpx{a.r + b.r, a.i + b.i}; }
__device__ __forceinline__ cpx csub(cpx a, cpx b) { return cpx{a.r - b.r, a.i - b.i}; }
__device__ __forceinline__ cpx cmul_si(cpx a, float s) { return cpx{-s * a.i, s * a.r}; }

template <int R>
__device__ __forceinline__ void dft(cpx* v, float s);
template <>
__device__ __forceinline__ void dft<2>(cpx* v, float) {
  cpx a = v[0], b = v[1];
  v[0] = cadd(a, b);
  v[1] = csub(a, b);
}
template <>
// ... 299 lines not shown

  if constexpr (NH != 0) gload(k_begin);
  for (int k = k_begin; k < k_end; ++k) {
    if constexpr (NH != 0) {
#pragma unroll
      for (int it = 0; it < MIT; ++it) {
        const int m = mg + it * (NT / 4);
        if (m <= n) stage_m(m, rr[it], ri[it]);
      }
    } else {
      for (int m = mg; m <= n; m += NT / 4) {
        f32x4 vr = {0.f, 0.f, 0.f, 0.f}, vi = {0.f, 0.f, 0.f, 0.f};
        if (cq < C && m < mtr) {
          const long o = (((long)m * K + k) * B + b) * (2L * C) + (ilv ? c0 + cq : cq);
          vr = *reinterpret_cast<const f32x4*>(Yf + o);
          vi = *reinterpret_cast<const f32x4*>(Yf + o + (ilv ? CB : C));
        }
        stage_m(m, vr, vi);
      }
    }
    __syncthreads();
    if constexpr (NH != 0) {
      if (k + 1 < k_end) gload(k + 1);
    }

    const int np = n / 2 + 1;
    for (int id = threadIdx.x; id < CB * np; id += NT) {
      const int r = id / np, m = id - r * np;
      float* re = L.a_re + r * S;
      float* im = L.a_im + r * S;
      cpx A = cpx{re[m], im[m]};
      cpx Bc = cpx{re[n - m], -im[n - m]};
      if (m == 0) {
        A.i = 0.f;
        Bc.i = 0.f;
      }
      const cpx Sm = cadd(A, Bc);
      const cpx D = cmul(cpx{L.pw_re[m], -L.pw_im[m]}, csub(A, Bc));
      re[m] = Sm.r - D.i;
      im[m] = Sm.i + D.r;
      if (m > 0) {
        re[n - m] = Sm.r + D.i;
        im[n - m] = -(Sm.i - D.r);
      }
    }
    __syncthreads();

    float *zr, *zi;
    if constexpr (NH != 0)
      fft_rows_ct<NH>(L, S, +1.0f, &zr, &zi);
    else
      fft_rows(f, L, S, +1.0f, &zr, &zi);

    const int q4 = N / 4;
    for (int idx = threadIdx.x; idx < CB * q4; idx += NT) {
      const int r = idx / q4, q = idx - r * q4;
      const int c = c0 + r;
      if (c < C) {
        const float bv = bias ? bias[c] : 0.0f;
        f32x4 v;
        v.x = zr[r * S + 2 * q] + bv;
        v.y = zi[r * S + 2 * q] + bv;
        v.z = zr[r * S + 2 * q + 1] + bv;
        v.w = zi[r * S + 2 * q + 1] + bv;
        *reinterpret_cast<f32x4*>(y + (((long)b * C + c) * K + k) * N + 4 * q) = v;
      }
    }
    __syncthreads();
  }
}

size_t fft_smem_bytes(const SdyFftDesc& f) { return ((size_t)4 * CB * f.S + 2 * f.n + 2 * (f.n + 1)) * sizeof(float); }

}

int sdy_fft_launch_fwd(const SdyFftDesc& f, const float* x, const float* a, const float* d, float* xn_out, float* Xf,
                       int B, int C, int K, int mtr, int ilv, const int* mcut, hipStream_t stream,
                       const unsigned char* x_rows, int x_mod) {
  if (ilv && C % CB != 0) return SDY_ERR_UNSUPPORTED;
  if (f.n == 180 && f.fft360) {
    const int rc = sdy_fft360_launch_fwd(f, x, a, d, xn_out, Xf, B, C, K, mtr, ilv, mcut, stream, x_rows, x_mod);
    if (rc != SDY_ERR_UNSUPPORTED) return rc;
  }
  if (mcut || ilv == 2 || x_rows || x_mod) return SDY_ERR_UNSUPPORTED;
  const size_t smem = fft_smem_bytes(f);
  if (smem > 64 * 1024) return SDY_ERR_UNSUPPORTED;
  constexpr int KPW = 4;
  dim3 grid((C + CB - 1) / CB, (K + KPW - 1) / KPW, B);
  unsigned* flags = nullptr;
  if (f.guard_f16) SDY_TRY(sdy_flags_ptr(&flags));
  if (f.n == 180) {
    hipLaunchKernelGGL((rfft_fwd_kernel<180, KPW>), grid, dim3(NT), smem, stream, f, x, a, d, xn_out, Xf, B, C, K, mtr, ilv, flags);
  } else if (f.n == 32) {
    hipLaunchKernelGGL((rfft_fwd_kernel<32, KPW>), grid, dim3(NT), smem, stream, f, x, a, d, xn_out, Xf, B, C, K, mtr, ilv, flags);
  } else {
    grid.y = K;
    hipLaunchKernelGGL((rfft_fwd_kernel<0, 1>), grid, dim3(NT), smem, stream, f, x, a, d, xn_out, Xf, B, C, K, mtr, ilv, flags);
  }
  return sdy_launch_status();
}

int sdy_fft_launch_inv(const SdyFftDesc& f, const float* Yf, const float* bias, float* y, int B, int C, int K, int mtr,
                       int ilv, const int* mcut, hipStream_t stream) {
  if (ilv && C % CB != 0) return SDY_ERR_UNSUPPORTED;
  if (f.n == 180 && f.fft360) {
    const int rc = sdy_fft360_launch_inv(f, Yf, bias, y, B, C, K, mtr, ilv, mcut, stream);
    if (rc != SDY_ERR_UNSUPPORTED) return rc;
  }
  if (mcut || ilv == 2) return SDY_ERR_UNSUPPORTED;
  const size_t smem = fft_smem_bytes(f);
  if (smem > 64 * 1024) return SDY_ERR_UNSUPPORTED;
  constexpr int KPW = 4;
  dim3 grid((C + CB - 1) / CB, (K + KPW - 1) / KPW, B);
  if (f.n == 180) {
    hipLaunchKernelGGL((irfft_kernel<180, KPW>), grid, dim3(NT), smem, stream, f, Yf, bias, y, B, C, K, mtr, ilv);
  } else if (f.n == 32) {
    hipLaunchKernelGGL((irfft_kernel<32, KPW>), grid, dim3(NT), smem, stream, f, Yf, bias, y, B, C, K, mtr, ilv);
  } else {
    grid.y = K;
    hipLaunchKernelGGL((irfft_kernel<0, 1>), grid, dim3(NT), smem, stream, f, Yf, bias, y, B, C, K, mtr, ilv);
  }
  return sdy_launch_status();
}
```

### spherical-dyffusion_amd/csrc/fft360.hip

```cpp
#include "common.h"
#include "fft.h"

namespace {

typedef float c2 __attribute__((ext_vector_type(2)));

constexpr int NH = 180;
constexpr int NLON = 360;
constexpr int ROWS = 16;
constexpr int NT = 256;
constexpr int P = 200;
constexpr int Q4 = NLON / 4;
constexpr int MIT = 3;
#ifndef SDY_FFT_MINB_F
#define SDY_FFT_MINB_F 4
#endif
#ifndef SDY_FFT_MINB_I
#define SDY_FFT_MINB_I 4
#endif
#ifndef SDY_FFT_KPW
#define SDY_FFT_KPW 1
#endif
constexpr int MINB_F = SDY_FFT_MINB_F, MINB_I = SDY_FFT_MINB_I;

// ... 179 lines not shown
  const bool tail = L.lane < TAIL;

  const int c4 = threadIdx.x & 3, mg = threadIdx.x >> 2;
  const float scale = 6.28318530717958647692f / (float)NLON;
  c2 W[MIT];
#pragma unroll
  for (int it = 0; it < MIT; ++it) {
    const c2 w = reinterpret_cast<const c2*>(f.pw)[min(mg + 64 * it, NH)];
    W[it] = c2{w.y, -w.x} * (0.5f * scale);
  }
  const c2* za = Z + c4 * P + mg;
  const c2* zn01 = Z + c4 * P + (NH - 64 - mg);
  const c2* zn2 = Z + c4 * P + max(NH - 128 - mg, 0);
  const long mstride = (long)K * B * 2 * C;
  const int re_off = (ilv ? 2 * c0 : c0) + 4 * c4, im_off = ilv ? 16 : C;
  const long tile_base = (long)((b * (C / ROWS) + id.x) >> 1) * K * 64 + (id.x & 1) * 32 + 4 * c4;

  float amax = 0.0f;
  f32x4 regs[8];
  auto gload = [&](int k) {
#pragma unroll
    for (int r = 0; r < 4; ++r) {
      const float* src = xw + r * rstride + (long)k * NLON;
      regs[2 * r] = *reinterpret_cast<const f32x4*>(src);
      if (tail) regs[2 * r + 1] = *reinterpret_cast<const f32x4*>(src + 256);
    }
  };
  gload(k_begin);
  __syncthreads();

  for (int k = k_begin; k < k_end; ++k) {
#pragma unroll
    for (int r = 0; r < 4; ++r) {
      const c2 ad = AD[4 * L.wave + r];
      const f32x4 v0 = regs[2 * r] * ad.x + ad.y, v1 = regs[2 * r + 1] * ad.x + ad.y;
      if (xnw) {
        float* dst = xnw + r * rstride + (long)k * NLON;
        *reinterpret_cast<f32x4*>(dst) = v0;
        if (tail) *reinterpret_cast<f32x4*>(dst + 256) = v1;
      }
      *reinterpret_cast<f32x4*>(zw + r * P) = v0;
      if (tail) *reinterpret_cast<f32x4*>(zw + r * P + 128) = v1;
    }
    if (k + 1 < k_end) gload(k + 1);
    __builtin_amdgcn_wave_barrier();

    if (L.t < 15) {
      c2 v[12];
      const c2* src = L.row + L.t;
#pragma unroll
      for (int bb = 0; bb < 12; ++bb) v[bb] = src[15 * bb];
      pass_a_tail<-1>(L, v, TW);
    }
    pass_b<-1, true>(L);
    __syncthreads();

    float* Xk = ilv == 2 ? Xf + tile_base + (long)k * 64 : Xf + ((long)k * B + b) * 2 * C + re_off;
    const int mlive = mcut ? min(mtr, mcut[k]) : mtr;
#pragma unroll
    for (int it = 0; it < MIT; ++it) {
      const int m = mg + 64 * it;
      if (m < mlive) {
        f32x4 vr, vi;
#pragma unroll
        for (int j = 0; j < 4; ++j) {
          const c2 A = za[64 * it + 4 * j * P];
          const c2 Bv = it < 2 ? zn01[64 * (1 - it) + 4 * j * P] : zn2[4 * j * P];
          const c2 S = c2{A.x + Bv.x, A.y - Bv.y}, D = c2{A.x - Bv.x, A.y + Bv.y};
          const c2 X = (0.5f * scale) * S + cmul(D, W[it]);
          vr[j] = X.x;
          vi[j] = X.y;
          amax = __builtin_fmaxf(amax, __builtin_fmaxf(__builtin_fabsf(X.x), __builtin_fabsf(X.y)));
        }
        float* o = Xk + (long)m * mstride;
        SDY_STREAM_STORE(o, vr);
        SDY_STREAM_STORE(o + im_off, vi);
      }
    }
    __syncthreads();
  }
  sdy_flag_range(flags, amax * (2.0f * SDY_ACT_SX), head);
}

template <int KPW>
__global__ __launch_bounds__(NT, MINB_I) void irfft360_kernel(const SdyFftDesc f, const float* __restrict__ Yf,
                                                            const float* __restrict__ bias, float* __restrict__ y, int B,
                                                            int C, int K, int mtr, int ilv,
                                                            const int* __restrict__ mcut, float* __restrict__ zt,
                                                            long zt_bs, double* __restrict__ part) {
  __shared__ __attribute__((aligned(16))) c2 Z[ROWS * P];
  __shared__ c2 TW[TWN];
  __shared__ c2 PW[NH];
  __shared__ float BS[ROWS];
  const Lane L = lane_roles(Z);
  const WgId id = wg_id(C / ROWS, (K + KPW - 1) / KPW);
  const int c0 = id.x * ROWS, b = id.z;
  const int k_begin = id.y * KPW, k_end = min(K, k_begin + KPW);

  fill_twiddles(f, TW);
  if (threadIdx.x < NH) {
    const c2 w = reinterpret_cast<const c2*>(f.pw)[threadIdx.x];
    PW[threadIdx.x] = c2{w.x, -w.y};
  }
  if (threadIdx.x < ROWS) {
    const int s = threadIdx.x;
    BS[s] = bias ? bias[c0 + 4 * (s & 3) + (s >> 2)] : 0.0f;
  }

  const int c4 = threadIdx.x & 3, mg = threadIdx.x >> 2;
  const long mstride = (long)K * B * 2 * C;
  const int re_off = (ilv ? 2 * c0 : c0) + 4 * c4, im_off = ilv ? 16 : C;
  const long tile_base = (long)((b * (C / ROWS) + id.x) >> 1) * K * 64 + (id.x & 1) * 32 + 4 * c4;
  f32x4 rr[MIT], ri[MIT];
  auto gload = [&](int k) {
    const float* Yk = ilv == 2 ? Yf + tile_base + (long)k * 64 : Yf + ((long)k * B + b) * 2 * C + re_off;
    const int mlive = mcut ? min(mtr, mcut[k]) : mtr;
#pragma unroll
    for (int it = 0; it < MIT; ++it) {
      const int m = mg + 64 * it;
      f32x4 vr = {0.f, 0.f, 0.f, 0.f}, vi = {0.f, 0.f, 0.f, 0.f};
      if (m < mlive) {
        const float* o = Yk + (long)m * mstride;
        vr = *reinterpret_cast<const f32x4*>(o);
        vi = *reinterpret_cast<const f32x4*>(o + im_off);
      }
      if (m == 0 || m == NH) vi = f32x4{0.f, 0.f, 0.f, 0.f};
      rr[it] = vr;
      ri[it] = vi;
    }
  };

  float* yw = y + (((long)b * C + c0 + L.wave) * K) * NLON + 4 * L.lane;
  const long rstride = 4L * K * NLON;
  const c2* zw = Z + 4 * L.wave * P + 2 * L.lane;
  const bool tail = L.lane < TAIL;
  c2* zs = Z + c4 * P + mg;

  gload(k_begin);
  for (int k = k_begin; k < k_end; ++k) {
#pragma unroll
    for (int it = 0; it < MIT; ++it) {
      if (mg + 64 * it <= NH) {
#pragma unroll
        for (int j = 0; j < 4; ++j) zs[4 * j * P + 64 * it] = c2{rr[it][j], ri[it][j]};
      }
    }
    __syncthreads();
    if (k + 1 < k_end) gload(k + 1);

    if (L.t < 15) {
      c2 v[12];
      const c2* lo = L.row + L.t;
      const c2* hi = L.row + (15 - L.t);
      const c2* pw = PW + L.t;
#pragma unroll
      for (int bb = 0; bb < 12; ++bb) {
        const c2 A = lo[15 * bb], Bv = hi[15 * (11 - bb)], w = pw[15 * bb];
        const c2 S = c2{A.x + Bv.x, A.y - Bv.y}, Dm = c2{A.x - Bv.x, A.y + Bv.y};
        const c2 D = cmul(Dm, w);
        v[bb] = c2{S.x - D.y, S.y + D.x};
      }
      __builtin_amdgcn_wave_barrier();
      pass_a_tail<+1>(L, v, TW);
    }
    pass_b<+1, false>(L);

    if (zt) {
      float* ztb = zt + (long)b * zt_bs;
      const int px0 = k * NLON + 4 * L.lane, px1 = px0 + 256;
#pragma unroll
      for (int r = 0; r < 4; ++r) {
        const float bs = BS[4 * L.wave + r];
        const int ch = c0 + L.wave + 4 * r;
        f32x4 v = *reinterpret_cast<const f32x4*>(zw + r * P) + bs;
        v = f32x4{gelu_erf(v.x), gelu_erf(v.y), gelu_erf(v.z), gelu_erf(v.w)};
        SDY_STREAM_STORE(ztb + (long)(px0 >> 6) * (C * 64) + ch * 64 + (px0 & 63), v);
        float qs = sdy_quad_sum(v), qs2 = sdy_quad_sumsq(v);
        if (tail) {
          f32x4 u = *reinterpret_cast<const f32x4*>(zw + r * P + 128) + bs;
          u = f32x4{gelu_erf(u.x), gelu_erf(u.y), gelu_erf(u.z), gelu_erf(u.w)};
          SDY_STREAM_STORE(ztb + (long)(px1 >> 6) * (C * 64) + ch * 64 + (px1 & 63), u);
          qs += sdy_quad_sum(u);
          qs2 += sdy_quad_sumsq(u);
        }
        double ds = (double)row16_sum(qs), ds2 = (double)row16_sum(qs2);
        ds += __shfl_xor(ds, 16, 64);
        ds2 += __shfl_xor(ds2, 16, 64);
        ds += __shfl_xor(ds, 32, 64);
        ds2 += __shfl_xor(ds2, 32, 64);
        if (L.lane == 0) {
          double* slot = part + (((long)b * K + k) * C + ch) * 2;
          slot[0] = ds;
          slot[1] = ds2;
        }
      }
    } else {
#pragma unroll
    for (int r = 0; r < 4; ++r) {
      const float bs = BS[4 * L.wave + r];
      float* dst = yw + r * rstride + (long)k * NLON;
      SDY_STREAM_STORE(dst, *reinterpret_cast<const f32x4*>(zw + r * P) + bs);
      if (tail) SDY_STREAM_STORE(dst + 256, *reinterpret_cast<const f32x4*>(zw + r * P + 128) + bs);
    }
    }
    __syncthreads();
  }
}

}

int sdy_fft360_launch_fwd(const SdyFftDesc& f, const float* x, const float* a, const float* d, float* xn_out, float* Xf,
                          int B, int C, int K, int mtr, int ilv, const int* mcut, hipStream_t stream,
                          const unsigned char* x_rows, int x_mod) {
  if (f.n != NH || C % ROWS != 0 || mtr > NH + 1 || (long)ROWS * K * NLON >= (1L << 31)) return SDY_ERR_UNSUPPORTED;
  if (ilv == 2 && (C % (2 * ROWS) != 0 || ROWS != 16)) return SDY_ERR_UNSUPPORTED;
  constexpr int KPW = SDY_FFT_KPW;
  SdyImgMap xmap;
  SDY_TRY(sdy_img_map_fill(xmap, x_rows, B));
  dim3 grid((C / ROWS) * ((K + KPW - 1) / KPW) * B);
  unsigned *flags = nullptr, *head = nullptr;
  if (f.guard_f16) {
    SDY_TRY(sdy_flags_ptr(&flags));
    SDY_TRY(sdy_headroom_ptr(SDY_RANGE_LEG_ANALYSIS, &head));
  }
  hipLaunchKernelGGL((rfft360_kernel<KPW>), grid, dim3(NT), 0, stream, f, x, a, d, xn_out, Xf, B, C, K, mtr, ilv, mcut, xmap,
                     flags, head, x_mod);
  return sdy_launch_status();
}

int sdy_fft360_launch_inv(const SdyFftDesc& f, const float* Yf, const float* bias, float* y, int B, int C, int K,
                          int mtr, int ilv, const int* mcut, hipStream_t stream, float* zt, long zt_bs, double* part) {
  if (f.n != NH || C % ROWS != 0 || mtr > NH + 1 || (long)ROWS * K * NLON >= (1L << 31)) return SDY_ERR_UNSUPPORTED;
  if (ilv == 2 && (C % (2 * ROWS) != 0 || ROWS != 16)) return SDY_ERR_UNSUPPORTED;
  if ((zt == nullptr) != (part == nullptr) || (!zt && !y)) return SDY_ERR_ARG;
  constexpr int KPW = SDY_FFT_KPW;
  dim3 grid((C / ROWS) * ((K + KPW - 1) / KPW) * B);
  hipLaunchKernelGGL((irfft360_kernel<KPW>), grid, dim3(NT), 0, stream, f, Yf, bias, y, B, C, K, mtr, ilv, mcut, zt, zt_bs, part);
  return sdy_launch_status();
}
```

### spherical-dyffusion_amd/csrc/leg_par.hip

```cpp
#include <cmath>
#include <cstdlib>
#include <vector>

#include "common.h"

namespace {

constexpr int PM = 192;
constexpr int PKP = 192;
constexpr int PTN = 64;
constexpr int PKS = 6;
constexpr int PRING = 8;
constexpr int PGPW = 2 * PKS;
constexpr float PSX = SDY_ACT_SX;

struct ParParams {
  const sdy_f16x8* table;
  const float* X; long ldx, sX;
  float* C; long ldc, sC;
  long tsx, tsc;
  int rows_out, K, N;
  const int* kdead;
  float out_scale;
  unsigned long long* stamps;
};

__device__ __forceinline__ int pr_off(int px, int c) { return px * PKP + (((c & ~7) | ((c ^ (px >> 1)) & 7)) << 3); }

__device__ __forceinline__ void st4s(float* ubase, unsigned off_b, float v) {
  sdy_gptr_t b = (sdy_gptr_t)ubase;
  asm volatile("" : "+s"(b), "+v"(off_b));
  *reinterpret_cast<float __attribute__((address_space(1)))*>(b + off_b) = v;
}

template <bool FWD, bool STAMPS>
__global__ __launch_bounds__(192, 3) void leg_par_kernel(const ParParams p) {
  __shared__ __attribute__((aligned(16))) unsigned char smem[2 * PTN * PKP * 2];
  _Float16* Xs_hi = reinterpret_cast<_Float16*>(smem);
  _Float16* Xs_lo = Xs_hi + PTN * PKP;

  const int tid = threadIdx.x, lane = tid & 63;
  const int wave = __builtin_amdgcn_readfirstlane(tid >> 6);
  const int h = lane >> 5, l31 = lane & 31;
  const int z = blockIdx.y;
  const int n0 = blockIdx.x * PTN;
  const bool full = n0 + PTN <= p.N;
  const int Kh = (FWD ? p.K : p.rows_out) >> 1;
  const int cE = z & 1, cO = cE ^ 1;

  const int kd = p.kdead ? p.kdead[z] : 0;
  const bool wave_dead = FWD ? (64 * wave + 63 < z)
                             : (32 * wave + 31 < kd);
  const int ks0 = FWD ? kd >> 4 : z >> 5;
  auto stamp = [&](int i) {
    if (STAMPS && lane == 0 && (blockIdx.x == 37 || blockIdx.x == 150) && (z == 20 || z == 90))
      p.stamps[(((blockIdx.x == 150) * 2 + (z == 90)) * 3 + wave) * 8 + i] = __builtin_amdgcn_s_memtime();
  };
  stamp(0);

  sdy_f16x8 r_hi[PRING], r_lo[PRING];
  constexpr int PGROUP_BYTES = SDY_GROUP * (int)sizeof(sdy_f16x8);
  const char* const wbase = reinterpret_cast<const char*>(p.table) +
                            (size_t)__builtin_amdgcn_readfirstlane(z * 3 + wave) * PGPW * PGROUP_BYTES;
  unsigned woff = (unsigned)lane * 16u;
  if (!wave_dead) {
#pragma unroll
    for (int s = 0; s < PRING; ++s) {
      r_hi[s] = sdy_ring_ld(wbase, woff, 0);
      r_lo[s] = sdy_ring_ld(wbase, woff, PGROUP_BYTES / 2);
      woff += PGROUP_BYTES;
    }
  }

  {
    const int q = tid & 15, o = tid >> 4;
    const bool ok = full || (n0 + 4 * q < p.N);
    const float* xz = p.X + (long)z * p.sX + (p.tsx ? (long)blockIdx.x * p.tsx : (long)n0);
    f32x4 xa[8], xb[8];
    bool va[8], vb[8];
    const bool oct_live = FWD ? (8 * o + 7 >= kd && 8 * o < Kh) : (16 * o + 15 >= z && 16 * o < p.K);
    const bool oct_full = FWD ? true : (16 * o + 15 < p.K);
    const unsigned colc = ok ? 4 * q : 0;
#pragma unroll
    for (int e = 0; e < 8; ++e) {
      xa[e] = f32x4{0.f, 0.f, 0.f, 0.f};
      xb[e] = f32x4{0.f, 0.f, 0.f, 0.f};
      const int r = 8 * o + e;
      if (FWD) {
        va[e] = vb[e] = ok && r < Kh && r >= kd;
      } else {
        va[e] = ok && 2 * r + cE < p.K && 2 * r + cE >= z;
        vb[e] = ok && 2 * r + cO < p.K && 2 * r + cO >= z;
      }
    }
    if (oct_live) {
      if (FWD) {
        const unsigned offA = (unsigned)((long)(8 * o) * p.ldx + colc) * 4u;
        const unsigned offB = (unsigned)((long)(p.K - 8 - 8 * o) * p.ldx + colc) * 4u;
#pragma unroll
        for (int e = 0; e < 8; ++e) {
          xa[e] = sdy_ld16s(xz + (long)e * p.ldx, offA);
          xb[e] = sdy_ld16s(xz + (long)(7 - e) * p.ldx, offB);
        }
// ... 49 lines not shown
    for (int j = 0; j < 2; ++j)
#pragma unroll
      for (int r = 0; r < 16; ++r) acc[hf][j][r] = 0.0f;

#pragma unroll
  for (int ks = 0; ks < PKS; ++ks) {
    if (ks >= ks0) {
#pragma unroll
      for (int hf = 0; hf < 2; ++hf) {
        sdy_f16x8 bh[2], bl[2];
#pragma unroll
        for (int j = 0; j < 2; ++j) {
          const int off = pr_off(32 * j + l31, 12 * hf + 2 * ks + h);
          bh[j] = *reinterpret_cast<const sdy_f16x8*>(Xs_hi + off);
          bl[j] = *reinterpret_cast<const sdy_f16x8*>(Xs_lo + off);
        }
        const int s = 2 * (ks & 3) + hf;
#pragma unroll
        for (int j = 0; j < 2; ++j) SDY_CROSS_TERM(acc[hf][j] = __builtin_amdgcn_mfma_f32_32x32x16_f16(r_lo[s], bh[j], acc[hf][j], 0, 0, 0));
#pragma unroll
        for (int j = 0; j < 2; ++j) SDY_CROSS_TERM(acc[hf][j] = __builtin_amdgcn_mfma_f32_32x32x16_f16(r_hi[s], bl[j], acc[hf][j], 0, 0, 0));
#pragma unroll
        for (int j = 0; j < 2; ++j) acc[hf][j] = __builtin_amdgcn_mfma_f32_32x32x16_f16(r_hi[s], bh[j], acc[hf][j], 0, 0, 0);
      }
    }
    if (ks + 4 < PKS) {
#pragma unroll
      for (int hf = 0; hf < 2; ++hf) {
        const int s = 2 * (ks & 3) + hf;
        r_hi[s] = sdy_ring_ld(wbase, woff, 0);
        r_lo[s] = sdy_ring_ld(wbase, woff, PGROUP_BYTES / 2);
        woff += PGROUP_BYTES;
      }
    }
    __builtin_amdgcn_sched_barrier(0);
  }
  stamp(4);

  float* cz = p.C + (long)z * p.sC + (p.tsc ? (long)blockIdx.x * p.tsc : (long)n0);
  constexpr unsigned long long MH0 = 0x00000000FFFFFFFFull, MH1 = 0xFFFFFFFF00000000ull;
  unsigned long long colm[2];
#pragma unroll
  for (int j = 0; j < 2; ++j) colm[j] = __builtin_amdgcn_ballot_w64(n0 + 32 * j + l31 < p.N);
  if (FWD) {
    const unsigned offl = (unsigned)((long)(8 * h) * p.ldc + l31) * 4u;
#pragma unroll
    for (int hf = 0; hf < 2; ++hf)
#pragma unroll
      for (int r4 = 0; r4 < 4; ++r4) {
        const int base = 64 * wave + 16 * r4 + (hf == 0 ? cE : cO);
        if (base + 14 < z || base >= p.rows_out) continue;
        float* rowp = cz + (long)base * p.ldc;
        if (full && base >= z && base + 14 < p.rows_out) {
#pragma unroll
          for (int r2 = 0; r2 < 4; ++r2, rowp += 2 * p.ldc)
#pragma unroll
            for (int j = 0; j < 2; ++j) st4s(rowp + 32 * j, offl, acc[hf][j][4 * r4 + r2] * p.out_scale);
        } else {
#pragma unroll
          for (int r2 = 0; r2 < 4; ++r2, rowp += 2 * p.ldc) {
            const int lu = base + 2 * r2;
            const unsigned long long m = ((lu >= z && lu < p.rows_out) ? MH0 : 0ull) | ((lu + 8 >= z && lu + 8 < p.rows_out) ? MH1 : 0ull);
#pragma unroll
            for (int j = 0; j < 2; ++j)
              if (__builtin_amdgcn_inverse_ballot_w64(m & colm[j])) st4s(rowp + 32 * j, offl, acc[hf][j][4 * r4 + r2] * p.out_scale);
          }
        }
      }
  } else {
    const unsigned off1 = (unsigned)((long)(4 * h) * p.ldc + l31) * 4u;
    const unsigned off2 = (unsigned)((long)(4 * (1 - h)) * p.ldc + l31) * 4u;
#pragma unroll
    for (int r4 = 0; r4 < 4; ++r4) {
      const int base = 32 * wave + 8 * r4;
      if (base + 7 < kd || base >= Kh) continue;
      float* row1 = cz + (long)base * p.ldc;
      float* row2 = cz + (long)(p.rows_out - 5 - base) * p.ldc;
      if (full && base >= kd && base + 7 < Kh) {
#pragma unroll
        for (int r2 = 0; r2 < 4; ++r2, row1 += p.ldc, row2 -= p.ldc)
#pragma unroll
          for (int j = 0; j < 2; ++j) {
            const float e = acc[0][j][4 * r4 + r2], od = acc[1][j][4 * r4 + r2];
            st4s(row1 + 32 * j, off1, (e + od) * p.out_scale);
            st4s(row2 + 32 * j, off2, (e - od) * p.out_scale);
          }
      } else {
#pragma unroll
        for (int r2 = 0; r2 < 4; ++r2, row1 += p.ldc, row2 -= p.ldc) {
          const int ru = base + r2;
          const unsigned long long m = ((ru >= kd && ru < Kh) ? MH0 : 0ull) | ((ru + 4 >= kd && ru + 4 < Kh) ? MH1 : 0ull);
#pragma unroll
          for (int j = 0; j < 2; ++j)
            if (__builtin_amdgcn_inverse_ballot_w64(m & colm[j])) {
              const float e = acc[0][j][4 * r4 + r2], od = acc[1][j][4 * r4 + r2];
              st4s(row1 + 32 * j, off1, (e + od) * p.out_scale);
              st4s(row2 + 32 * j, off2, (e - od) * p.out_scale);
            }
        }
      }
    }
  }
  stamp(5);
}

}

#if SDY_STAMPS_ON
static unsigned long long* g_lstamps = nullptr;
SDY_DEBUG_EXPORT int sdy_leg_par_debug_stamps(unsigned long long* host96) {
  if (!g_lstamps || !host96) return SDY_ERR_STATE;
  SDY_HIP_TRY(hipDeviceSynchronize());
  SDY_HIP_TRY(hipMemcpy(host96, g_lstamps, 96 * sizeof(unsigned long long), hipMemcpyDeviceToHost));
  return SDY_OK;
}
#endif

size_t sdy_leg_par_table_bytes(int nz) { return ((size_t)nz * 3 * PGPW + PRING) * SDY_GROUP * sizeof(sdy_f16x8); }

int sdy_leg_par_supported(int nlat, int lmax) {
  return (nlat <= PM && lmax <= PM && (nlat & 1) == 0 && nlat >= 16 && lmax >= 16) ? 1 : 0;
}

int sdy_leg_par_pack(int nz, int nlat, int lmax, int fwd, sdy_leg_value_fn value, void* ctx, void* dev, float* scale) {
  if (!sdy_leg_par_supported(nlat, lmax) || !value || !dev || !scale) return SDY_ERR_ARG;
  const int Kh = nlat / 2;
  float mx = 0.f;
  for (int z = 0; z < nz; ++z)
    for (int l = 0; l < lmax; ++l)
      for (int k = 0; k < Kh; ++k) mx = std::fmax(mx, std::fabs(fwd ? value(ctx, z, l, k) : value(ctx, z, k, l)));
  const float s = sdy_h3_scale(mx);
  const size_t gh = (size_t)SDY_GROUP * 8;
  std::vector<_Float16> buf(((size_t)nz * 3 * PGPW + PRING) * gh, (_Float16)0.0f);
  for (int z = 0; z < nz; ++z) {
    const int cE = z & 1;
    for (int w = 0; w < 3; ++w) {
      _Float16* d = buf.data() + (size_t)(z * 3 + w) * PGPW * gh;
      for (int ks = 0; ks < PKS; ++ks)
        for (int hf = 0; hf < 2; ++hf, d += gh) {
          const int cls = hf == 0 ? cE : cE ^ 1;
          sdy_h3_put_group(d, s, [&](int r, int k) {
            const int rt = 32 * w + r, kk = 16 * ks + k;
            if (fwd) {
              const int l = 2 * rt + cls;
              return (l < lmax && kk < Kh) ? value(ctx, z, l, kk) : 0.0f;
            }
            const int l = 2 * kk + cls;
            return (rt < Kh && l < lmax) ? value(ctx, z, rt, l) : 0.0f;
          });
        }
    }
  }
  SDY_HIP_TRY(hipMemcpy(dev, buf.data(), buf.size() * sizeof(_Float16), hipMemcpyHostToDevice));
  *scale = s;
  return SDY_OK;
}

int sdy_leg_par_launch(const void* table, float scale, int nz, const float* X, long ldx, long sX, float* C, long ldc,
                       long sC, int rows_out, int K, int N, int fwd, const int* kdead, hipStream_t stream, long tsx, long tsc) {
  if (!table || !X || !C || nz <= 0 || N <= 0) return SDY_ERR_ARG;
  if ((tsx || tsc) && N % PTN) return SDY_ERR_UNSUPPORTED;
  if (rows_out > PM || K > PM || nz > PM) return SDY_ERR_UNSUPPORTED;
  if ((fwd ? K : rows_out) & 1) return SDY_ERR_UNSUPPORTED;
  if ((N & 3) || (ldx & 3) || (sX & 3) || (ldc & 3) || (sC & 3)) return SDY_ERR_ALIGN;
  ParParams p;
  p.table = reinterpret_cast<const sdy_f16x8*>(table);
  p.X = X; p.ldx = ldx; p.sX = sX;
  p.C = C; p.ldc = ldc; p.sC = sC;
  p.tsx = tsx; p.tsc = tsc;
  if ((long)PM * ldx * 4 + (long)N * 4 >= (1L << 32) || (long)8 * ldc * 4 + (long)N * 4 >= (1L << 32)) return SDY_ERR_UNSUPPORTED;
  p.rows_out = rows_out; p.K = K; p.N = N; p.kdead = kdead;
  p.out_scale = 1.0f / (scale * PSX);
  p.stamps = nullptr;
  dim3 grid((N + PTN - 1) / PTN, nz);
#if SDY_STAMPS_ON
  if (std::getenv("SDY_LEG_STAMPS")) {
    if (!g_lstamps) SDY_HIP_TRY(hipMalloc(&g_lstamps, 96 * sizeof(unsigned long long)));
    p.stamps = g_lstamps;
  }
  if (p.stamps) {
    if (fwd) hipLaunchKernelGGL((leg_par_kernel<true, true>), grid, dim3(192), 0, stream, p);
    else hipLaunchKernelGGL((leg_par_kernel<false, true>), grid, dim3(192), 0, stream, p);
    return sdy_launch_status();
  }
#endif
  if (fwd) hipLaunchKernelGGL((leg_par_kernel<true, false>), grid, dim3(192), 0, stream, p);
  else hipLaunchKernelGGL((leg_par_kernel<false, false>), grid, dim3(192), 0, stream, p);
  return sdy_launch_status();
}
```

Measured before the change: 167.0 member-forecast-steps/s.

## Add ring-major Legendre-inverse output layout and tiled skip-conv addend path

Adds a new ilv=3 ring-major Yf layout, which the inverse Legendre kernel writes through a configurable half-stride and the irfft360 kernel reads per (batch,channel-group) ring. The goal is more contiguous, coalesced traffic between the two stages. It also lets the inverse FFT write its output in the 64-pixel tiled layout into the hid buffer, so the skip 1x1 conv can read the addend tiled and match its own tile structure. Both are on by default with env switches to disable them, and the hid workspace is enlarged to hold the tiled output. The risks are extra index arithmetic and possible strided-store inefficiencies in the Legendre kernel epilogue.

```diff
diff --git a/include/sdy_amd.h b/include/sdy_amd.h
--- a/include/sdy_amd.h
+++ b/include/sdy_amd.h
@@ -49,6 +49,9 @@
 int sdy_legendre_inv(const sdy_sht_plan* plan, const float* Cs, float* Yf, int B, int C, void* stream);
 int sdy_irfft_lon(const sdy_sht_plan* plan, const float* Yf, const float* bias, float* y, int B, int C,
                   void* stream);
+int sdy_legendre_inv_fused(const sdy_sht_plan* plan, const float* Cs, float* Yf, int B, int C, int yf_layout, void* stream);
+int sdy_irfft_lon_fused(const sdy_sht_plan* plan, const float* Yf, const float* bias, float* y, long y_bstride, int y_tiled,
+                        int B, int C, int yf_layout, void* stream);
 int sdy_irfft_lon_act(const sdy_sht_plan* plan, const float* Yf, const float* bias, float* zt, long zt_bstride, double* part,
                       int B, int C, void* stream);
 int sdy_instnorm_from_partials(const double* part, int K, int B, int C, int HW, const float* gamma, const float* beta,
@@ -97,6 +100,7 @@
   float w_frag_scale;
   double* stats;
   int out_tiled;
+  int add_tiled;
   const unsigned char* x_rows;
 } sdy_conv_args;
 int sdy_conv1x1(const sdy_conv_args* args, void* stream);
@@ -175,6 +179,7 @@
 int sdy_sfno_set_param(sdy_sfno* net, const char* name, const float* host, size_t numel);
 int sdy_sfno_ready(const sdy_sfno* net);
 const char* sdy_sfno_missing(const sdy_sfno* net);
+int sdy_sfno_block_layouts(const sdy_sfno* net, int block, int out[4]);
 size_t sdy_sfno_workspace_floats(const sdy_sfno* net, int B);
 int sdy_sfno_max_batch(const sdy_sfno* net);
 
diff --git a/spherical-dyffusion_amd/_lib.py b/spherical-dyffusion_amd/_lib.py
--- a/spherical-dyffusion_amd/_lib.py
+++ b/spherical-dyffusion_amd/_lib.py
@@ -36,6 +36,7 @@
         ("w_frag_scale", C.c_float),
         ("stats", C.c_void_p),
         ("out_tiled", C.c_int),
+        ("add_tiled", C.c_int),
         ("x_rows", C.c_void_p),
     ]
 
@@ -440,6 +441,10 @@
     "sdy_legendre_fwd": (C.c_int, [C.c_void_p, C.c_void_p, C.c_void_p, C.c_int, C.c_int, C.c_void_p]),
     "sdy_legendre_inv": (C.c_int, [C.c_void_p, C.c_void_p, C.c_void_p, C.c_int, C.c_int, C.c_void_p]),
     "sdy_irfft_lon": (C.c_int, [C.c_void_p, C.c_void_p, C.c_void_p, C.c_void_p, C.c_int, C.c_int, C.c_void_p]),
+    "sdy_sfno_block_layouts": (C.c_int, [C.c_void_p, C.c_int, C.POINTER(C.c_int * 4)]),
+    "sdy_legendre_inv_fused": (C.c_int, [C.c_void_p, C.c_void_p, C.c_void_p, C.c_int, C.c_int, C.c_int, C.c_void_p]),
+    "sdy_irfft_lon_fused": (C.c_int, [C.c_void_p, C.c_void_p, C.c_void_p, C.c_void_p, C.c_long, C.c_int, C.c_int, C.c_int, C.c_int,
+                                      C.c_void_p]),
     "sdy_irfft_lon_act": (C.c_int, [C.c_void_p, C.c_void_p, C.c_void_p, C.c_void_p, C.c_long, C.c_void_p, C.c_int, C.c_int,
                                     C.c_void_p]),
     "sdy_instnorm_from_partials": (C.c_int, [C.c_void_p, C.c_int, C.c_int, C.c_int, C.c_int, C.c_void_p, C.c_void_p, C.c_float,
diff --git a/spherical-dyffusion_amd/csrc/capi.hip b/spherical-dyffusion_amd/csrc/capi.hip
--- a/spherical-dyffusion_amd/csrc/capi.hip
+++ b/spherical-dyffusion_amd/csrc/capi.hip
@@ -96,14 +96,15 @@
 
 namespace {
 struct SdySwitches {
-  bool gemm_f32, no_fft360, no_leg_par, no_leg_frag, no_dh_frag, no_fused_mlp, no_drop_skip, no_skip_fold;
+  bool gemm_f32, no_fft360, no_leg_par, no_leg_frag, no_dh_frag, no_fused_mlp, no_drop_skip, no_skip_fold, no_ring_major_yf, no_tiled_addend;
 };
 const SdySwitches& sw() {
   static const SdySwitches v = [] {
     auto on = [](const char* n) { return std::getenv(n) != nullptr; };
     const char* g = std::getenv("SDY_GEMM_MODE");
     return SdySwitches{g && std::string(g) == "f32", on("SDY_NO_FFT360"), on("SDY_NO_LEG_PAR"), on("SDY_NO_LEG_FRAG"),
-                       on("SDY_NO_DH_FRAG"), on("SDY_NO_FUSED_MLP"), on("SDY_NO_DROP_SKIP"), on("SDY_NO_SKIP_FOLD")};
+                       on("SDY_NO_DH_FRAG"), on("SDY_NO_FUSED_MLP"), on("SDY_NO_DROP_SKIP"), on("SDY_NO_SKIP_FOLD"),
+                       on("SDY_NO_RING_MAJOR_YF"), on("SDY_NO_TILED_ADDEND")};
   }();
   return v;
 }
@@ -390,8 +391,9 @@
 }
 
 static int legendre_inv_impl(const sdy_sht_plan* p, const float* Cs, float* Yf, int B, int C, bool polar, void* stream,
-                             bool tiled, bool cs_tiled) {
+                             bool tiled, bool cs_tiled, bool ring = false) {
   if (!p || !Cs || !Yf || B <= 0 || C <= 0) return SDY_ERR_ARG;
+  if (ring && (!tiled || p->leg != sdy_sht_plan::LEG_PAR)) return SDY_ERR_UNSUPPORTED;
   if (C & 1) return SDY_ERR_ALIGN;
   const int N = 2 * B * C;
   GemmParams g{};
@@ -402,9 +404,10 @@
   g.tri_mode = SDY_TRI_LEG_INV; g.tile = SDY_TILE_64x128;
   if (p->leg == sdy_sht_plan::LEG_PAR)
     return sdy_leg_par_launch(p->d_pct_par, p->s_pct_par, p->mtr, Cs, cs_tiled ? 64L : (long)p->mtr * N,
-                              cs_tiled ? (long)(N / 64) * p->lmax * 64 : (long)N, Yf, tiled ? 64 : N,
-                              (long)p->nlat * N, p->nlat, p->lmax, N, 0, polar ? p->d_kdead : nullptr, (hipStream_t)stream,
-                              cs_tiled ? 64L * p->lmax : 0L, tiled ? 64L * p->nlat : 0L);
+                              cs_tiled ? (long)(N / 64) * p->lmax * 64 : (long)N, Yf, ring ? (long)N * p->mtr : tiled ? 64 : N,
+                              ring ? 32L : (long)p->nlat * N, p->nlat, p->lmax, N, 0, polar ? p->d_kdead : nullptr,
+                              (hipStream_t)stream, cs_tiled ? 64L * p->lmax : 0L,
+                              ring ? 64L * p->mtr : tiled ? 64L * p->nlat : 0L, ring ? 32L * p->mtr : 32L);
   if (tiled || cs_tiled) return SDY_ERR_UNSUPPORTED;
   if (p->leg == sdy_sht_plan::LEG_H3)
     return sdy_leg_h3_launch(p->d_pct_frag, p->s_pct_frag, p->mtr, Cs, (long)p->mtr * N, N, Yf, N, (long)p->nlat * N, p->nlat,
@@ -416,6 +419,33 @@
 }
 extern "C" int sdy_legendre_inv(const sdy_sht_plan* p, const float* Cs, float* Yf, int B, int C, void* stream) {
   return legendre_inv_impl(p, Cs, Yf, B, C, false, stream, false, false);
+}
+
+static inline bool tiled_stride_ok(long bs, int C, int HW);
+static int yf_layout_ok(const sdy_sht_plan* p, int C, int yf_layout) {
+  if (yf_layout != 2 && yf_layout != 3) return SDY_ERR_ARG;
+  return (p->leg == sdy_sht_plan::LEG_PAR && plan_tiled_ok(p, C, 1)) ? SDY_OK : SDY_ERR_UNSUPPORTED;
+}
+extern "C" int sdy_legendre_inv_fused(const sdy_sht_plan* p, const float* Cs, float* Yf, int B, int C, int yf_layout,
+                                      void* stream) {
+  if (!p || !Cs || !Yf || B <= 0 || C <= 0) return SDY_ERR_ARG;
+  SDY_TRY(yf_layout_ok(p, C, yf_layout));
+  if (!fft_aligned16(Cs) || !fft_aligned16(Yf)) return SDY_ERR_ALIGN;
+  return legendre_inv_impl(p, Cs, Yf, B, C, plan_polar_ok(p, C), stream, true, false, yf_layout == 3);
+}
+extern "C" int sdy_irfft_lon_fused(const sdy_sht_plan* p, const float* Yf, const float* bias, float* y, long y_bstride,
+                                   int y_tiled, int B, int C, int yf_layout, void* stream) {
+  if (!p || !Yf || !y || B <= 0 || C <= 0 || y_bstride < 0) return SDY_ERR_ARG;
+  SDY_TRY(yf_layout_ok(p, C, yf_layout));
+  if ((y_bstride & 3) || !fft_aligned16(Yf) || !fft_aligned16(y)) return SDY_ERR_ALIGN;
+  const int* mcut = plan_polar_ok(p, C) ? p->d_mcut : nullptr;
+  if (y_tiled) {
+    if (!tiled_stride_ok(y_bstride, C, p->nlat * p->nlon)) return SDY_ERR_ARG;
+    return sdy_fft360_launch_inv(p->fft, Yf, bias, y, B, C, p->nlat, p->mtr, yf_layout, mcut, (hipStream_t)stream, nullptr,
+                                 y_bstride, nullptr, 1);
+  }
+  if (y_bstride != (long)C * p->nlat * p->nlon) return SDY_ERR_ARG;
+  return sdy_fft360_launch_inv(p->fft, Yf, bias, y, B, C, p->nlat, p->mtr, yf_layout, mcut, (hipStream_t)stream);
 }
 
 extern "C" int sdy_sht_forward(const sdy_sht_plan* p, const float* x, float* out_c64, int B, int C, float* ws,
@@ -580,7 +610,7 @@
   if (a->drop_p < 0.0f || a->drop_p >= 1.0f) return SDY_ERR_ARG;
   if (a->w_frag && sdy_conv256_h3_supported(a->Cin, a->Cout) && a->drop_p == 0.0f && !a->keep_mask && !a->batch_scale)
     return sdy_conv256_h3_launch(a, (hipStream_t)stream);
-  if (a->stats || a->out_tiled || a->x_rows) return SDY_ERR_UNSUPPORTED;
+  if (a->stats || a->out_tiled || a->add_tiled || a->x_rows) return SDY_ERR_UNSUPPORTED;
   GemmParams g{};
   g.A = a->wt; g.lda = a->ldw; g.sA = 0;
   g.B = a->x; g.ldb = a->HW; g.sB = a->x_bstride;
@@ -676,6 +706,8 @@
   bool polar;
   bool tiled;
   int ilv;
+  bool ring;
+  int ilv_inv;
   const int* mcut;
 };
 
@@ -689,6 +721,7 @@
   enum Skip { SKIP_CONV, SKIP_GELU, SKIP_IN_FFT } skip;
   bool stats1;
   bool z_tiled;
+  bool y_tiled;
   bool drop_skip;
 };
 }
@@ -998,7 +1031,8 @@
   const int E = c.embed_dim, ilv = spec_ilv(c);
   auto side = [&](const sdy_sht_plan* p) {
     const bool polar = plan_polar_ok(p, E), tiled = plan_tiled_ok(p, E, ilv);
-    return XfSide{p, polar, tiled, tiled ? 2 : ilv, polar ? p->d_mcut : nullptr};
+    const bool ring = tiled && !sw().no_ring_major_yf;
+    return XfSide{p, polar, tiled, tiled ? 2 : ilv, ring, ring ? 3 : tiled ? 2 : ilv, polar ? p->d_mcut : nullptr};
   };
   BlockPath b;
   b.in = side(i == 0 ? n->plan_data : n->plan_lg);
@@ -1012,6 +1046,7 @@
   b.stats1 = c.gemm_mode == 1 && w.skw.frag && sdy_conv256_h3_supported(E, E);
   b.z_tiled = b.stats1 && b.fused_mlp;
   b.skip = b.dh != DH_FOLDED ? BlockPath::SKIP_CONV : (b.out.tiled && b.z_tiled) ? BlockPath::SKIP_IN_FFT : BlockPath::SKIP_GELU;
+  b.y_tiled = b.skip == BlockPath::SKIP_CONV && b.out.tiled && b.z_tiled && !sw().no_tiled_addend;
   b.drop_skip = b.fused_mlp && b.z_tiled && b.cs_tiled && !sw().no_drop_skip;
   return b;
 }
@@ -1065,6 +1100,17 @@
 }
 
 extern "C" const char* sdy_sfno_missing(const sdy_sfno* n) { return n ? n->missing.c_str() : ""; }
+
+extern "C" int sdy_sfno_block_layouts(const sdy_sfno* n, int block, int out[4]) {
+  if (!n || !out || block < 0 || block >= n->cfg.num_layers) return SDY_ERR_ARG;
+  SDY_TRY(sdy_sfno_ready(n));
+  const BlockPath& P = n->path[block];
+  out[0] = P.in.ilv;
+  out[1] = P.out.ilv_inv;
+  out[2] = P.y_tiled ? 1 : 0;
+  out[3] = P.z_tiled ? 1 : 0;
+  return SDY_OK;
+}
 
 namespace {
 struct WsLayout {
@@ -1082,7 +1128,7 @@
   w.xe = take(img);
   w.xn = take(img); w.y = take(img);
   w.zt = take((size_t)B * ((HW + 63) / 64) * E * 64);
-  w.hid = take((size_t)B * c.mlp_hidden * HW);
+  w.hid = take((size_t)B * std::max((size_t)c.mlp_hidden * HW, ((HW + 63) / 64) * 64 * E));
   w.xf = take(xf_floats(n->plan_data, B, (int)E));
   w.cs = take(cs_floats(n->plan_data, B, (int)E)); w.cs2 = take(cs_floats(n->plan_data, B, (int)E));
   w.ca = take((size_t)B * E); w.cd = take((size_t)B * E); w.ca1 = take((size_t)B * E); w.cd1 = take((size_t)B * E);
@@ -1407,8 +1453,8 @@
                                                        P.in.mcut, stream, k.rows, (k.i == 0 && enc_once) ? Be : 0));
       SDY_STAGE_N(ST_LEG_FWD, k.Bf, legendre_fwd_impl(pin, Xf, Cs, k.Bf, E, P.in.polar, stream, P.in.tiled, P.cs_tiled));
       if (P.scale_residual) {
-        SDY_STAGE(ST_LEG_INV, legendre_inv_impl(pout, Cs, Xf, B, E, P.out.polar, stream, P.out.tiled, P.cs_tiled));
-        SDY_STAGE(ST_FFT_INV, sdy_fft_launch_inv(pout->fft, Xf, nullptr, xn, B, E, pout->nlat, pout->mtr, P.out.ilv, P.out.mcut,
+        SDY_STAGE(ST_LEG_INV, legendre_inv_impl(pout, Cs, Xf, B, E, P.out.polar, stream, P.out.tiled, P.cs_tiled, P.out.ring));
+        SDY_STAGE(ST_FFT_INV, sdy_fft_launch_inv(pout->fft, Xf, nullptr, xn, B, E, pout->nlat, pout->mtr, P.out.ilv_inv, P.out.mcut,
                                                  stream));
       }
     }
@@ -1420,13 +1466,17 @@
       SDY_STAGE(ST_DHCONV, sdy_dhconv_h3(Cs, k.w.fw.h3, k.w.fw.h3_scale, Cs2, c.lmax, pin->mtr, B, E, E, stream));
     else
       SDY_STAGE(ST_DHCONV, sdy_dhconv(Cs, k.w.fw.p, Cs2, c.lmax, pin->mtr, B, E, E, stream));
-    SDY_STAGE_N(ST_LEG_INV, k.Bp, legendre_inv_impl(pout, Cs2, Xf, k.Bp, E, P.out.polar, stream, P.out.tiled, P.cs_tiled));
+    SDY_STAGE_N(ST_LEG_INV, k.Bp, legendre_inv_impl(pout, Cs2, Xf, k.Bp, E, P.out.polar, stream, P.out.tiled, P.cs_tiled,
+                                                    P.out.ring));
     const float* bias = P.dh == DH_FOLDED ? k.w.fbs.p : k.w.fb.p;
     if (P.skip == BlockPath::SKIP_IN_FFT)
-      SDY_STAGE_N(ST_FFT_INV, k.Bp, sdy_fft360_launch_inv(pout->fft, Xf, bias, nullptr, k.Bp, E, pout->nlat, pout->mtr, P.out.ilv,
+      SDY_STAGE_N(ST_FFT_INV, k.Bp, sdy_fft360_launch_inv(pout->fft, Xf, bias, nullptr, k.Bp, E, pout->nlat, pout->mtr, P.out.ilv_inv,
                                                           P.out.mcut, stream, zt, zt_bs, sp));
+    else if (P.y_tiled)
+      SDY_STAGE_N(ST_FFT_INV, k.Bp, sdy_fft360_launch_inv(pout->fft, Xf, bias, hid, k.Bp, E, pout->nlat, pout->mtr, P.out.ilv_inv,
+                                                          P.out.mcut, stream, nullptr, zt_bs, nullptr, 1));
     else
-      SDY_STAGE_N(ST_FFT_INV, k.Bp, sdy_fft_launch_inv(pout->fft, Xf, bias, y, k.Bp, E, pout->nlat, pout->mtr, P.out.ilv,
+      SDY_STAGE_N(ST_FFT_INV, k.Bp, sdy_fft_launch_inv(pout->fft, Xf, bias, y, k.Bp, E, pout->nlat, pout->mtr, P.out.ilv_inv,
                                                        P.out.mcut, stream));
     return SDY_OK;
   }
@@ -1447,7 +1497,8 @@
       cv.x = P.lazy_norm ? cur : xn; cv.x_bstride = xbs;
       if (P.lazy_norm) { cv.pa = ca; cv.pd = cd; }
       cv.ldw = E; cv.out = k.z; cv.out_bstride = k.z_bs; cv.out_tiled = P.z_tiled ? 1 : 0;
-      cv.Cin = E; cv.Cout = E; cv.bias = bw.skb.p; cv.add = y; cv.add_bstride = xbs; cv.add_mode = 1; cv.act = 1; cv.kernel_tag = 3;
+      cv.Cin = E; cv.Cout = E; cv.bias = bw.skb.p; cv.add = P.y_tiled ? hid : y; cv.add_bstride = P.y_tiled ? zt_bs : xbs; cv.add_tiled = P.y_tiled ? 1 : 0;
+      cv.add_mode = 1; cv.act = 1; cv.kernel_tag = 3;
       if (P.stats1) cv.stats = st1;
       SDY_STAGE_N(ST_SKIP_CONV, k.Bp, sdy_conv1x1(&cv, stream));
     }
diff --git a/spherical-dyffusion_amd/csrc/common.h b/spherical-dyffusion_amd/csrc/common.h
--- a/spherical-dyffusion_amd/csrc/common.h
+++ b/spherical-dyffusion_amd/csrc/common.h
@@ -335,7 +335,8 @@
 size_t sdy_leg_par_table_bytes(int nz);
 int sdy_leg_par_pack(int nz, int nlat, int lmax, int fwd, sdy_leg_value_fn value, void* ctx, void* dev, float* scale);
 int sdy_leg_par_launch(const void* table, float scale, int nz, const float* X, long ldx, long sX, float* C, long ldc,
-                       long sC, int rows_out, int K, int N, int fwd, const int* kdead, hipStream_t stream, long tsx = 0, long tsc = 0);
+                       long sC, int rows_out, int K, int N, int fwd, const int* kdead, hipStream_t stream, long tsx = 0, long tsc = 0,
+                       long hsc = 32);
 int sdy_leg_h3_launch(const void* table, float scale, int nz, const float* X, long ldx, long sX, float* C, long ldc, long sC,
                       int M_store, int K, int N, int tri, hipStream_t stream);
 
diff --git a/spherical-dyffusion_amd/csrc/conv_h3.hip b/spherical-dyffusion_amd/csrc/conv_h3.hip
--- a/spherical-dyffusion_amd/csrc/conv_h3.hip
+++ b/spherical-dyffusion_amd/csrc/conv_h3.hip
@@ -44,6 +44,7 @@
   const sdy_f16x8* w;
   const float* bias;
   const float* add; long add_bs; int add_mode;
+  int add_tiled;
   int act;
   float* out; long out_bs;
   int out_tiled;
@@ -231,9 +232,11 @@
 
     stamp(3);
     {
-      const float* az = img(addsrc, addsrc_bs, tile);
-#pragma unroll
-      for (int i = 0; i < CRPT; ++i) addv[i] = p.add ? sdy_ld16s(az + (long)(CRS * i) * p.HW, ro) : f32x4{0.f, 0.f, 0.f, 0.f};
+      const float* az = img(addsrc, addsrc_bs, tile) + (p.add_tiled ? (long)(tile - z * tpi) * (CE * CTN) : 0L);
+      const unsigned ro_add = p.add_tiled ? (unsigned)(o0 * CTN + 4 * q0) * 4u : ro;
+      const int add_rs = p.add_tiled ? CTN : p.HW;
+#pragma unroll
+      for (int i = 0; i < CRPT; ++i) addv[i] = p.add ? sdy_ld16s(az + (long)(CRS * i) * add_rs, ro_add) : f32x4{0.f, 0.f, 0.f, 0.f};
     }
     __syncthreads();
     stamp(4);
@@ -375,7 +378,9 @@
   p.add = a->add_mode ? a->add : nullptr; p.add_bs = a->add_bstride; p.add_mode = a->add_mode;
   p.act = a->act;
   p.out = a->out; p.out_bs = a->out_bstride; p.out_tiled = a->out_tiled;
-  if (a->out_tiled && a->add_mode && a->add == a->out) return SDY_ERR_ARG;
+  p.add_tiled = (a->add_mode && a->add_tiled) ? 1 : 0;
+  if ((a->out_tiled || p.add_tiled) && a->add_mode && a->add == a->out) return SDY_ERR_ARG;
+  if (p.add_tiled && a->add_bstride < (long)((a->HW + CTN - 1) / CTN) * CE * CTN) return SDY_ERR_ARG;
   p.stats = a->stats;
   SDY_TRY(sdy_flags_ptr(&p.flags));
   SDY_TRY(sdy_headroom_ptr(SDY_RANGE_CONV, &p.head));
diff --git a/spherical-dyffusion_amd/csrc/fft.h b/spherical-dyffusion_amd/csrc/fft.h
--- a/spherical-dyffusion_amd/csrc/fft.h
+++ b/spherical-dyffusion_amd/csrc/fft.h
@@ -24,4 +24,4 @@
                           const unsigned char* x_rows = nullptr, int x_mod = 0);
 int sdy_fft360_launch_inv(const SdyFftDesc& f, const float* Yf, const float* bias, float* y, int B, int C, int K,
                           int mtr, int ilv, const int* mcut, hipStream_t stream, float* zt = nullptr, long zt_bs = 0,
-                          double* part = nullptr);
+                          double* part = nullptr, int y_tiled = 0);
diff --git a/spherical-dyffusion_amd/csrc/fft.hip b/spherical-dyffusion_amd/csrc/fft.hip
--- a/spherical-dyffusion_amd/csrc/fft.hip
+++ b/spherical-dyffusion_amd/csrc/fft.hip
@@ -405,7 +405,7 @@
     const int rc = sdy_fft360_launch_fwd(f, x, a, d, xn_out, Xf, B, C, K, mtr, ilv, mcut, stream, x_rows, x_mod);
     if (rc != SDY_ERR_UNSUPPORTED) return rc;
   }
-  if (mcut || ilv == 2 || x_rows || x_mod) return SDY_ERR_UNSUPPORTED;
+  if (mcut || ilv >= 2 || x_rows || x_mod) return SDY_ERR_UNSUPPORTED;
   const size_t smem = fft_smem_bytes(f);
   if (smem > 64 * 1024) return SDY_ERR_UNSUPPORTED;
   constexpr int KPW = 4;
@@ -430,7 +430,7 @@
     const int rc = sdy_fft360_launch_inv(f, Yf, bias, y, B, C, K, mtr, ilv, mcut, stream);
     if (rc != SDY_ERR_UNSUPPORTED) return rc;
   }
-  if (mcut || ilv == 2) return SDY_ERR_UNSUPPORTED;
+  if (mcut || ilv >= 2) return SDY_ERR_UNSUPPORTED;
   const size_t smem = fft_smem_bytes(f);
   if (smem > 64 * 1024) return SDY_ERR_UNSUPPORTED;
   constexpr int KPW = 4;
diff --git a/spherical-dyffusion_amd/csrc/fft360.hip b/spherical-dyffusion_amd/csrc/fft360.hip
--- a/spherical-dyffusion_amd/csrc/fft360.hip
+++ b/spherical-dyffusion_amd/csrc/fft360.hip
@@ -285,12 +285,12 @@
   sdy_flag_range(flags, amax * (2.0f * SDY_ACT_SX), head);
 }
 
-template <int KPW>
+template <int KPW, bool ACT>
 __global__ __launch_bounds__(NT, MINB_I) void irfft360_kernel(const SdyFftDesc f, const float* __restrict__ Yf,
                                                             const float* __restrict__ bias, float* __restrict__ y, int B,
                                                             int C, int K, int mtr, int ilv,
                                                             const int* __restrict__ mcut, float* __restrict__ zt,
-                                                            long zt_bs, double* __restrict__ part) {
+                                                            long zt_bs, double* __restrict__ part, int y_tiled) {
   __shared__ __attribute__((aligned(16))) c2 Z[ROWS * P];
   __shared__ c2 TW[TWN];
   __shared__ c2 PW[NH];
@@ -311,12 +311,15 @@
   }
 
   const int c4 = threadIdx.x & 3, mg = threadIdx.x >> 2;
-  const long mstride = (long)K * B * 2 * C;
+  const long mstride = ilv == 3 ? 32L : (long)K * B * 2 * C;
   const int re_off = (ilv ? 2 * c0 : c0) + 4 * c4, im_off = ilv ? 16 : C;
   const long tile_base = (long)((b * (C / ROWS) + id.x) >> 1) * K * 64 + (id.x & 1) * 32 + 4 * c4;
+  const long ring_base = (long)(b * (C / ROWS) + id.x) * mtr * 32 + 4 * c4, ring_stride = (long)B * (C / ROWS) * mtr * 32;
   f32x4 rr[MIT], ri[MIT];
   auto gload = [&](int k) {
-    const float* Yk = ilv == 2 ? Yf + tile_base + (long)k * 64 : Yf + ((long)k * B + b) * 2 * C + re_off;
+    const float* Yk = ilv == 3   ? Yf + ring_base + (long)k * ring_stride
+                      : ilv == 2 ? Yf + tile_base + (long)k * 64
+                                 : Yf + ((long)k * B + b) * 2 * C + re_off;
     const int mlive = mcut ? min(mtr, mcut[k]) : mtr;
 #pragma unroll
     for (int it = 0; it < MIT; ++it) {
@@ -368,7 +371,7 @@
     }
     pass_b<+1, false>(L);
 
-    if (zt) {
+    if (ACT) {
       float* ztb = zt + (long)b * zt_bs;
       const int px0 = k * NLON + 4 * L.lane, px1 = px0 + 256;
 #pragma unroll
@@ -398,12 +401,16 @@
         }
       }
     } else {
+    const int px0 = k * NLON + 4 * L.lane, px1 = px0 + 256;
+    float* yt0 = y + (long)b * zt_bs + (long)(px0 >> 6) * (C * 64) + (c0 + L.wave) * 64 + (px0 & 63);
+    float* yt1 = y + (long)b * zt_bs + (long)(px1 >> 6) * (C * 64) + (c0 + L.wave) * 64 + (px1 & 63);
 #pragma unroll
     for (int r = 0; r < 4; ++r) {
       const float bs = BS[4 * L.wave + r];
-      float* dst = yw + r * rstride + (long)k * NLON;
+      float* dst = y_tiled ? yt0 + r * 256 : yw + r * rstride + (long)k * NLON;
+      float* dst1 = y_tiled ? yt1 + r * 256 : dst + 256;
       SDY_STREAM_STORE(dst, *reinterpret_cast<const f32x4*>(zw + r * P) + bs);
-      if (tail) SDY_STREAM_STORE(dst + 256, *reinterpret_cast<const f32x4*>(zw + r * P + 128) + bs);
+      if (tail) SDY_STREAM_STORE(dst1, *reinterpret_cast<const f32x4*>(zw + r * P + 128) + bs);
     }
     }
     __syncthreads();
@@ -417,6 +424,7 @@
                           const unsigned char* x_rows, int x_mod) {
   if (f.n != NH || C % ROWS != 0 || mtr > NH + 1 || (long)ROWS * K * NLON >= (1L << 31)) return SDY_ERR_UNSUPPORTED;
   if (ilv == 2 && (C % (2 * ROWS) != 0 || ROWS != 16)) return SDY_ERR_UNSUPPORTED;
+  if (ilv > 2) return SDY_ERR_UNSUPPORTED;
   constexpr int KPW = SDY_FFT_KPW;
   SdyImgMap xmap;
   SDY_TRY(sdy_img_map_fill(xmap, x_rows, B));
@@ -432,12 +440,19 @@
 }
 
 int sdy_fft360_launch_inv(const SdyFftDesc& f, const float* Yf, const float* bias, float* y, int B, int C, int K,
-                          int mtr, int ilv, const int* mcut, hipStream_t stream, float* zt, long zt_bs, double* part) {
+                          int mtr, int ilv, const int* mcut, hipStream_t stream, float* zt, long zt_bs, double* part, int y_tiled) {
   if (f.n != NH || C % ROWS != 0 || mtr > NH + 1 || (long)ROWS * K * NLON >= (1L << 31)) return SDY_ERR_UNSUPPORTED;
-  if (ilv == 2 && (C % (2 * ROWS) != 0 || ROWS != 16)) return SDY_ERR_UNSUPPORTED;
+  if ((ilv == 2 || ilv == 3) && (C % (2 * ROWS) != 0 || ROWS != 16)) return SDY_ERR_UNSUPPORTED;
+  if (ilv < 0 || ilv > 3) return SDY_ERR_UNSUPPORTED;
   if ((zt == nullptr) != (part == nullptr) || (!zt && !y)) return SDY_ERR_ARG;
+  if (y_tiled && (zt || zt_bs <= 0)) return SDY_ERR_ARG;
   constexpr int KPW = SDY_FFT_KPW;
   dim3 grid((C / ROWS) * ((K + KPW - 1) / KPW) * B);
-  hipLaunchKernelGGL((irfft360_kernel<KPW>), grid, dim3(NT), 0, stream, f, Yf, bias, y, B, C, K, mtr, ilv, mcut, zt, zt_bs, part);
+  if (zt)
+    hipLaunchKernelGGL((irfft360_kernel<KPW, true>), grid, dim3(NT), 0, stream, f, Yf, bias, y, B, C, K, mtr, ilv, mcut, zt, zt_bs,
+                       part, 0);
+  else
+    hipLaunchKernelGGL((irfft360_kernel<KPW, false>), grid, dim3(NT), 0, stream, f, Yf, bias, y, B, C, K, mtr, ilv, mcut, zt, zt_bs,
+                       part, y_tiled);
   return sdy_launch_status();
 }
diff --git a/spherical-dyffusion_amd/csrc/leg_par.hip b/spherical-dyffusion_amd/csrc/leg_par.hip
--- a/spherical-dyffusion_amd/csrc/leg_par.hip
+++ b/spherical-dyffusion_amd/csrc/leg_par.hip
@@ -19,6 +19,7 @@
   const float* X; long ldx, sX;
   float* C; long ldc, sC;
   long tsx, tsc;
+  long hsc;
   int rows_out, K, N;
   const int* kdead;
   float out_scale;
@@ -234,8 +235,8 @@
 #pragma unroll
           for (int j = 0; j < 2; ++j) {
             const float e = acc[0][j][4 * r4 + r2], od = acc[1][j][4 * r4 + r2];
-            st4s(row1 + 32 * j, off1, (e + od) * p.out_scale);
-            st4s(row2 + 32 * j, off2, (e - od) * p.out_scale);
+            st4s(row1 + p.hsc * j, off1, (e + od) * p.out_scale);
+            st4s(row2 + p.hsc * j, off2, (e - od) * p.out_scale);
           }
       } else {
 #pragma unroll
@@ -246,8 +247,8 @@
           for (int j = 0; j < 2; ++j)
             if (__builtin_amdgcn_inverse_ballot_w64(m & colm[j])) {
               const float e = acc[0][j][4 * r4 + r2], od = acc[1][j][4 * r4 + r2];
-              st4s(row1 + 32 * j, off1, (e + od) * p.out_scale);
-              st4s(row2 + 32 * j, off2, (e - od) * p.out_scale);
+              st4s(row1 + p.hsc * j, off1, (e + od) * p.out_scale);
+              st4s(row2 + p.hsc * j, off2, (e - od) * p.out_scale);
             }
         }
       }
@@ -309,9 +310,10 @@
 }
 
 int sdy_leg_par_launch(const void* table, float scale, int nz, const float* X, long ldx, long sX, float* C, long ldc,
-                       long sC, int rows_out, int K, int N, int fwd, const int* kdead, hipStream_t stream, long tsx, long tsc) {
+                       long sC, int rows_out, int K, int N, int fwd, const int* kdead, hipStream_t stream, long tsx, long tsc, long hsc) {
   if (!table || !X || !C || nz <= 0 || N <= 0) return SDY_ERR_ARG;
   if ((tsx || tsc) && N % PTN) return SDY_ERR_UNSUPPORTED;
+  if (hsc != 32 && (fwd || !tsc || hsc < 32 || (hsc & 3))) return SDY_ERR_UNSUPPORTED;
   if (rows_out > PM || K > PM || nz > PM) return SDY_ERR_UNSUPPORTED;
   if ((fwd ? K : rows_out) & 1) return SDY_ERR_UNSUPPORTED;
   if ((N & 3) || (ldx & 3) || (sX & 3) || (ldc & 3) || (sC & 3)) return SDY_ERR_ALIGN;
@@ -319,7 +321,7 @@
   p.table = reinterpret_cast<const sdy_f16x8*>(table);
   p.X = X; p.ldx = ldx; p.sX = sX;
   p.C = C; p.ldc = ldc; p.sC = sC;
-  p.tsx = tsx; p.tsc = tsc;
+  p.tsx = tsx; p.tsc = tsc; p.hsc = hsc;
   if ((long)PM * ldx * 4 + (long)N * 4 >= (1L << 32) || (long)8 * ldc * 4 + (long)N * 4 >= (1L << 32)) return SDY_ERR_UNSUPPORTED;
   p.rows_out = rows_out; p.K = K; p.N = N; p.kdead = kdead;
   p.out_scale = 1.0f / (scale * PSX);
```

Result: no change. 167.9 member-forecast-steps/s (median of 6 runs) (+0.5%).
